# tzt101/MichiGAN

Hardware: AMD Instinct MI355X
Metric: training images/sec at 512x512 (G+D step) (higher is better)
Workload: dtype bf16; 1 GPU; SPADEB G + multiscale PatchGAN D + VGG19 + Gabor orientation losses, full G step + D step (Adam), bs=8/GPU, 512x512, BASELINE.json configs[2]; global_batch=8, batch_per_gpu=8, resolution=512, parallelism=dp1, init=reference default (xavier, 0.02), random VGG weights

## Files before the change

### michigan_amd/_cabi.py

```python
from __future__ import annotations

import contextlib
import ctypes
import os

MG_F32, MG_BF16 = 0, 1
MG_ACT_NONE, MG_ACT_RELU, MG_ACT_LRELU, MG_ACT_TANH = 0, 1, 2, 3
MG_EPI_PLAIN, MG_EPI_SPADE = 0, 1
MG_MAX_TAPS = 64
MG_ABI_VERSION = 10
MG_COMM_ID_BYTES = 128

OPT_CONV_BIGTILES, OPT_CONV_HALO, OPT_WGRAD3X3, OPT_CONV_HALO_BIG, OPT_CONV_SPLITK, OPT_CONV_THIN, OPT_CONV_WIDE, OPT_CONV_DOT = 1, 2, 3, 4, 5, 6, 7, 8
OPT_PROBE_HALO_VARIANT, OPT_PROBE_WGRAD3X3, OPT_PROBE_ADDR_LO, OPT_PROBE_ADDR_HI, OPT_PROBE_NOXPRE = 10, 12, 13, 14, 15
OPT_WGRAD_MIN_STAGES, OPT_NORM_BWD_VEC, OPT_PROBE_HALO_LDSPAD, OPT_CONV_HALO64, OPT_PROBE_HALO64_DBG, OPT_WGRAD3X3_STRIPE = 18, 19, 21, 22, 23, 24

_i32, _f32, _vp, _i64 = ctypes.c_int32, ctypes.c_float, ctypes.c_void_p, ctypes.c_int64


class ConvDesc(ctypes.Structure):
    _fields_ = [
        ("in_", _vp), ("wt", _vp), ("out", _vp), ("bias", _vp), ("resid", _vp), ("x", _vp),
        ("mean", _vp), ("rstd", _vp), ("gamma_out", _vp),
        ("dtype", _i32), ("N", _i32), ("Hin", _i32), ("Win", _i32), ("Cin", _i32),
# ... 102 lines not shown
    "mg_pixel_affine": ([_vp, _vp, _vp, _vp, _i32, _i64, _i32, _vp, _vp], _i32),
    "mg_bg_compose": ([_vp, _vp, _vp, _i64, _i32, _i32, _i32, _i32, _i32, _i32, _vp, _vp, _vp], _i32),
    "mg_masked_mean_fill": ([_vp, _vp, _vp, _vp, _i32, _i32, _i32, _i32, _vp, _vp], _i32),
    "mg_orient_loss_fwd": ([_vp, _vp, _vp, _i32, _i64, _vp, _i64, _i32, _i64, _vp, _vp, _vp], _i32),
    "mg_orient_loss_bwd": ([_vp, _vp, _vp, _i32, _i64, _vp, _i64, _vp, _vp, _vp, _i32, _i64, _vp, _vp], _i32),
    "mg_color_loss_fwd": ([_vp, _vp, _i64, _vp, _i64, _i32, _i32, _i32, _i32, _i32, _i32, _vp, _vp, _vp], _i32),
    "mg_color_loss_bwd": ([_vp, _vp, _i64, _vp, _i64, _vp, _vp, _vp, _i32, _i32, _i32, _i32, _i32, _i32, _vp, _vp], _i32),
    "mg_hair_lab_fwd": ([_vp, _vp, _i64, _vp, _i64, _vp, _i64, _vp, _i64, _vp, _i64, _i32, _i32, _i32, _i32, _i32, _i32, _vp, _vp, _vp, _vp], _i32),
    "mg_hair_lab_bwd": ([_vp, _vp, _i64, _vp, _i64, _vp, _i64, _vp, _vp, _vp, _i32, _i32, _i32, _i32, _i32, _i32, _vp, _vp], _i32),
    "mg_gabor_argmax_fwd": ([_vp, _vp, _vp, _vp, _i32, _i32, _i32, _i32, _i32, _vp], _i32),
    "mg_gabor_argmax_bwd": ([_vp, _vp, _vp, _vp, _i32, _i32, _i32, _i32, _i32, _vp], _i32),
    "mg_self_attention": ([_vp, _vp, _vp, _vp, _i32, _i32, _i32, _i32, _i32, _i64, _i64, _i64, _i64, _vp], _i32),
    "mg_sn_normalize": ([_vp, _i32, _f32, _vp, _vp, _vp, _vp], _i32),
    "mg_sn_scale": ([_vp, _vp, _vp, _i64, _vp], _i32),
    "mg_sn_bwd": ([_vp, _vp, _vp, _vp, _vp, _vp, _i32, _i32, _vp], _i32),
    "mg_adam_step": ([_vp, _vp, _vp, _vp, _i64, _f32, _f32, _f32, _f32, _i32, _f32, _vp], _i32),
    "mg_input_crop_u8": ([_vp, _vp, _vp, _vp, _vp, _vp, _i32, _i32, _i32, _i32, _i32, _i32, _i32, _i32, _vp], _i32),
    "mg_onehot_labels": ([_vp, _vp, _i32, _i64, _i32, _vp], _i32),
    "mg_orient_to_rgb_u8": ([_vp, _vp, _vp, _vp, _i64, _vp], _i32),
    "mg_generate_hole_u8": ([_vp, _vp, _vp, _vp, _vp, _vp, _i32, _i32, _i32, _vp], _i32),
    "mg_noise_octaves": ([_vp, _vp, _i32, _i32, _vp], _i32),
    "mg_resize_bicubic_u8": ([_vp, _vp, _vp, _vp, _vp, _i32, _vp, _vp, _i32, _i32, _i32, _i32, _i32, _i32, _i32, _vp], _i32),
    "mg_bicubic_ksize": ([_i32, _i32], _i32),
    "mg_inputs_set_option": ([_i32, _i32], _i32),
    "mg_bicubic_table": ([_i32, _i32, _vp, _vp], _i32),
    "mg_nearest_table": ([_i32, _i32, _vp], _i32),
    "mg_orient_rgb_table": ([_vp], _i32),
    "mg_noise_field_len": ([_i32], _i64),
    "mg_comm_unique_id": ([_vp], _i32),
    "mg_comm_init": ([_vp, _i32, _i32, ctypes.POINTER(_i64)], _i32),
    "mg_comm_destroy": ([_i64], _i32),
    "mg_comm_world": ([_i64, ctypes.POINTER(_i32), ctypes.POINTER(_i32)], _i32),
    "mg_allreduce_stats": ([_i64, _vp, _i64, _i32, _vp], _i32),
    "mg_allreduce_grads": ([_i64, _vp, _i64, _vp], _i32),
    "mg_probe_mfma_layout": ([_vp, _vp], _i32),
    "mg_probe_tr16": ([_vp, _vp, _vp], _i32),
    "mg_set_option": ([_i32, _i32], _i32),
    "mg_get_option": ([_i32, ctypes.POINTER(_i32)], _i32),
    "mg_sizeof_desc": ([_i32], _i32),
    "mg_abi_version": ([], _i32),
    "mg_last_error": ([], ctypes.c_char_p),
    "mg_feat_moment_workspace": ([_i32, _i64, _i32], _i64),
    "mg_feat_moment_loss_fwd": ([ctypes.POINTER(FeatMomentDesc), _vp], _i32),
    "mg_feat_moment_loss_bwd": ([ctypes.POINTER(FeatMomentDesc), _vp, _vp, _vp, _vp], _i32),
    "mg_orient_smooth": ([_vp, _vp, _vp, _vp, _vp, _vp, _vp, _i32, _i32, _i32, _vp], _i32),
    "mg_stroke_orient": ([_vp, _vp, _vp, _vp, _vp, _vp, _i32, _i32, _i32, _vp], _i32),
    "mg_stroke_compose": ([_vp, _vp, _vp, _vp, _vp, _vp, _vp, _i32, _i32, _i32, _i32, _i32, _i32, _vp, _vp], _i32),
    "mg_inpaint_finish": ([_vp, _vp, _vp, _vp, _vp, _vp, _i32, _i32, _i32, _i32, _i32, _vp, _vp, _vp], _i32),
}
_EDIT_PROTOS = {
    "mge_brush_u8": ([_vp, _vp, _i32, _i32, _i32, _i32, _vp], _i32),
    "mge_morph_u8": ([_vp, _vp, _i32, _i32, _i32, _i32, _i32, _vp, _i32, _i32, _i32, _vp], _i32),
}
EXPORTED_SYMBOLS = tuple(_PROTOS)
_NO_STATUS = {"mg_wgrad_det_workspace", "mg_norm_apply2_supported", "mg_grad_slot_blocks", "mg_pack_job_blocks", "mg_sn_layer_blocks", "mg_stats_workspace", "mg_sizeof_desc", "mg_abi_version", "mg_last_error", "mg_noise_field_len", "mg_bicubic_ksize",
              "mg_feat_moment_workspace"}
_BY_REF = {fn for fn, (argtypes, _) in _PROTOS.items()
           if argtypes and isinstance(getattr(argtypes[0], "_type_", None), type) and issubclass(argtypes[0]._type_, ctypes.Structure)}
DESC_MIRRORS = (ConvDesc, WgradDesc, GradSlot, PackJob, SnLayer, NormApply2Desc, PyramidDesc, FeatMomentDesc)

LIB_PATH = os.environ.get("MG_LIB") or os.path.join(os.path.dirname(os.path.abspath(__file__)), "lib", "libmichigan_hip.so")


class HipBackend:
    name = "hip"

    def __init__(self, path: str = LIB_PATH):
        if not os.path.exists(path) and path == LIB_PATH and os.environ.get("MG_AUTOBUILD", "1") != "0":
            import sys
            print("[michigan_amd] libmichigan_hip.so missing: building it with hipcc (gfx950), ~2 min", file=sys.stderr, flush=True)
            from . import build as _build
            _build.build_locked(verbose=False)
        if not os.path.exists(path):
            raise RuntimeError(
                f"libmichigan_hip.so not found at {path}: build it with "
                "`python -c 'import __graft_entry__ as g; g.build()'` (hipcc, gfx950). "
                "michigan_amd has no CPU / eager-PyTorch fallback.")
        import torch
        self._lib = ctypes.CDLL(path)
        for fn, (argtypes, restype) in list(_PROTOS.items()) + list(_EDIT_PROTOS.items()):
            f = getattr(self._lib, fn)
            f.argtypes, f.restype = argtypes, restype
        if self._lib.mg_abi_version() != MG_ABI_VERSION:
            raise RuntimeError("libmichigan_hip.so ABI version mismatch")
        if any(self._lib.mg_sizeof_desc(which) != ctypes.sizeof(mirror) for which, mirror in enumerate(DESC_MIRRORS)):
            raise RuntimeError("ctypes mirror of the descriptor structs is out of sync with include/michigan_hip.h")

    def __getattr__(self, fn):
        if fn not in _PROTOS and fn not in _EDIT_PROTOS:
            raise AttributeError(fn)
        raw = getattr(self._lib, fn)
        if fn in _NO_STATUS:
            return raw
        by_ref = fn in _BY_REF

        def call(*args):
            if by_ref:
                args = (ctypes.byref(args[0]),) + tuple(args[1:])
            rc = raw(*args)
            if rc != 0:
                msg = self._lib.mg_last_error()
                raise RuntimeError(f"{fn} failed (code {rc}): {msg.decode() if msg else '?'}")
            return rc
        self.__dict__[fn] = call
        return call


_backend = None


def backend():
    global _backend
    if _backend is None:
        _backend = HipBackend()
    return _backend


def set_backend(obj):
    global _backend
    prev, _backend = _backend, obj
    return prev


def get_option(key, be=None):
    v = _i32()
    (be or backend()).mg_get_option(key, ctypes.byref(v))
    return v.value


@contextlib.contextmanager
def options(values, be=None):
    be = be or backend()
    saved = {key: get_option(key, be) for key in values}
    try:
        for key, v in values.items():
            be.mg_set_option(key, v)
        yield
    finally:
        for key, v in saved.items():
            be.mg_set_option(key, v)
```

### michigan_amd/csrc/mg_conv.hip

```cpp

#include "mg_conv_common.h"
#include <map>
#include <mutex>

namespace {

template <typename T, int WM, int WN, int MT, int NT, int EPI, bool PACK>
__global__ __launch_bounds__(NTHR, 3) void conv_taps_kernel(const ConvK d)
{
    constexpr int TM = WM * MT * 32, TN = WN * NT * 32;
    constexpr int EPP = 16 / (int)sizeof(T);
    constexpr int CH  = ROWB / (int)sizeof(T);
    constexpr int A_PT = (TM * 4 + NTHR - 1) / NTHR;
    constexpr int B_PT = (TN * 4) / NTHR;
    constexpr int STAGE = (TM + TN) * ROWB;
    static_assert(WM * WN == 4, "4 waves per workgroup");
    static_assert(EPI == MG_EPI_PLAIN || MT == 2, "SPADE epilogue needs gamma/beta tile pair");

    extern __shared__ __attribute__((aligned(16))) unsigned char smem[];

    const int tid = threadIdx.x, lane = tid & 63, wave = tid >> 6;
    const int wm = wave / WN, wn = wave % WN;
    const int l31 = lane & 31, hi = lane >> 5;

// ... 339 lines not shown
    if constexpr (TM % (16 * WM * WN) == 0) {
        const size_t stage = (size_t)(TM + TN) * ROWB;
        const size_t ldsr = (stage >= 32768 ? 4 : 3) * stage + 2 * TM * sizeof(float);
        auto kern = conv_taps_glds_kernel<T, WM, WN, MT, NT, EPI, PACK>;
        k.ntiles = (int)nblk; k.ksplit = 1; k.ws = nullptr;
        if constexpr (EPI == MG_EPI_PLAIN && !PACK && WM == 2 && WN == 2 && MT == 2 && NT == 2) {
            const int nchunk = (k.Cin * (int)sizeof(T) + ROWB - 1) / ROWB, nkk = k.ntaps * nchunk;
            if (mg_opt(MG_OPT_CONV_SPLITK) && nblk <= 160 && nkk >= 64 && (k.Cout & 3) == 0 && (k.Cout_gemm & 3) == 0) {
                int S = (int)((384 + nblk - 1) / nblk);
                if (S > nkk / 16) S = nkk / 16;
                if (S > 16) S = 16;
                if (S >= 2) {
                    k.ws = splitk_workspace(st, (size_t)S * k.ngemm * k.Cout_gemm * sizeof(float));
                    if (k.ws == nullptr) return mg_fail(MG_ERR_LAUNCH, "mg_conv_taps: split-K scratch allocation failed");
                    k.ksplit = S;
                    hipLaunchKernelGGL(kern, dim3((unsigned)(nblk * S)), dim3(64 * WM * WN), ldsr, st, k);
                    const long nel = (long)k.ngemm * (k.Cout / 4);
                    const long fb = (nel + 255) / 256;
                    hipLaunchKernelGGL(conv_splitk_finish<T>, dim3((unsigned)(fb > 2048 ? 2048 : fb)), dim3(256), 0, st, k);
                    MG_CHECK_LAUNCH("mg_conv_taps(glds, split-K)");
                    return MG_OK;
                }
            }
        }
        if (ldsr > 65536) {
            mg_raise_lds_cap(reinterpret_cast<const void*>(kern), (int)ldsr);
        }
        hipLaunchKernelGGL(kern, dim3((unsigned)nblk), dim3(64 * WM * WN), ldsr, st, k);
        MG_CHECK_LAUNCH("mg_conv_taps(glds)");
        return MG_OK;
    } else {
        const size_t lds = 2 * (size_t)(TM + TN) * ROWB + 2 * TM * sizeof(float);
        hipLaunchKernelGGL((conv_taps_kernel<T, WM, WN, MT, NT, EPI, PACK>), dim3((unsigned)nblk), dim3(NTHR), lds, st, k);
        MG_CHECK_LAUNCH("mg_conv_taps");
        return MG_OK;
    }
}

template <typename T, int EPI>
int dispatch_tiles(ConvK& k, hipStream_t st)
{
    auto wgs = [&](int tm, int tn) { return (long)((k.Cout_gemm + tm - 1) / tm) * ((k.ngemm + tn - 1) / tn); };
    const bool big = mg_opt(MG_OPT_CONV_BIGTILES);
    const int kchunks = k.ntaps * ((k.Cin * (int)sizeof(T) + ROWB - 1) / ROWB);
    if (big && kchunks >= 64 && k.Cout_gemm >= 256 && (k.CoutP % 256) == 0 && wgs(256, 256) >= 384)
        return launch_conv<T, 4, 2, 2, 4, EPI>(k, st);
    if (k.Cout_gemm > 64) return launch_conv<T, 2, 2, 2, 2, EPI>(k, st);
    if (EPI == MG_EPI_SPADE || k.Cout_gemm > 32) return launch_conv<T, 1, 4, 2, 2, EPI>(k, st);
    if constexpr (EPI == MG_EPI_PLAIN) return launch_conv<T, 1, 4, 1, 2, EPI>(k, st);
    return MG_ERR_UNSUPPORTED;
}

template <typename T>
bool halo_applies(const ConvK& k)
{
    constexpr int CH = ROWB / (int)sizeof(T);
    if (!mg_opt(MG_OPT_CONV_HALO)) return false;
    if (k.ntaps != 9 || k.isy != 1 || k.isx != 1 || k.osy != 1 || k.osx != 1 || k.ooy != 0 || k.oox != 0) return false;
    if (k.Hj != k.Hin || k.Wj != k.Win || k.Hout != k.Hin || k.Wout != k.Win) return false;
    if (k.Cin % CH || k.Cout_gemm <= 32 || k.Hin < 8 || k.Win < 16) return false;
    if (k.Cout_gemm <= 64 && k.Hin < 16) return false;
    unsigned seen = 0;
    for (int t = 0; t < 9; ++t) {
        const int dy = (int)(short)(k.tap[t] & 0xffff), dx = k.tap[t] >> 16;
        if (dy < -1 || dy > 1 || dx < -1 || dx > 1) return false;
        seen |= 1u << ((dy + 1) * 3 + dx + 1);
    }
    if (seen != 0x1ffu) return false;
    const int th = k.Cout_gemm <= 64 ? 16 : 8, tmh = k.Cout_gemm <= 64 ? 64 : 128;
    const long wgs = (long)k.N * ((k.Hin + th - 1) / th) * ((k.Win + 15) / 16) * ((k.Cout_gemm + tmh - 1) / tmh);
    return wgs >= 384;
}

template <typename T>
int dispatch_conv(ConvK& k, int epilogue, hipStream_t st)
{
    if (conv_thin_applies(k, ET<T>::DT, epilogue)) return launch_conv_thin(k, st);
    if (conv_thin_taps_applies(k, ET<T>::DT, epilogue)) return launch_conv_thin_taps(k, st);
    if (conv_dot_applies(k, ET<T>::DT, epilogue)) return launch_conv_dot(k, ET<T>::DT, st);
    if (conv_fewout_applies(k, ET<T>::DT, epilogue)) return launch_conv_fewout(k, st);
    if (conv_halo64_applies(k, ET<T>::DT, epilogue)) return launch_conv_halo64(k, st);
    if (halo_applies<T>(k)) return launch_conv_halo(k, ET<T>::DT, epilogue, st);
    return epilogue == MG_EPI_SPADE ? dispatch_tiles<T, MG_EPI_SPADE>(k, st) : dispatch_tiles<T, MG_EPI_PLAIN>(k, st);
}

}

float* mg_stream_scratch(hipStream_t st, size_t bytes) { return splitk_workspace(st, bytes); }

extern "C" int mg_conv_taps(const mg_conv_desc* d, void* stream)
{
    MG_CHECK_ARG(d != nullptr, "mg_conv_taps: null descriptor");
    MG_CHECK_ARG(d->in && d->wt && d->out, "mg_conv_taps: null tensor pointer");
    MG_CHECK_ARG(d->dtype == MG_F32 || d->dtype == MG_BF16, "mg_conv_taps: bad dtype %d", d->dtype);
    MG_CHECK_ARG(d->ntaps >= 1 && d->ntaps <= MG_MAX_TAPS, "mg_conv_taps: ntaps=%d out of range", d->ntaps);
    MG_CHECK_ARG(d->Cin > 0 && (d->Cin % 8) == 0, "mg_conv_taps: Cin=%d must be a positive multiple of 8", d->Cin);
    MG_CHECK_ARG(d->N > 0 && d->Hj > 0 && d->Wj > 0 && d->Hin > 0 && d->Win > 0, "mg_conv_taps: empty geometry");
    MG_CHECK_ARG(d->Cout > 0 && d->Cout_gemm > 0 && d->CoutP >= d->Cout_gemm && (d->CoutP % 128) == 0,
                 "mg_conv_taps: bad channel counts Cout=%d Cout_gemm=%d CoutP=%d", d->Cout, d->Cout_gemm, d->CoutP);
    MG_CHECK_ARG((long)d->N * d->Hj * d->Wj < (1L << 30), "mg_conv_taps: too many output pixels");
    MG_CHECK_ARG((long)d->Cin * (d->dtype == MG_BF16 ? 2 : 4) <= 8192, "mg_conv_taps: Cin too large (%d)", d->Cin);
    MG_CHECK_ARG((d->Hj - 1) * d->osy + d->ooy < d->Hout && (d->Wj - 1) * d->osx + d->oox < d->Wout && d->ooy >= 0 && d->oox >= 0,
                 "mg_conv_taps: output grid exceeds output tensor");
    if (d->epilogue == MG_EPI_SPADE) {
        MG_CHECK_ARG(d->x && d->mean && d->rstd, "mg_conv_taps: SPADE epilogue needs x/mean/rstd");
        MG_CHECK_ARG(d->Cout_gemm == 2 * ((d->Cout + 31) / 32) * 32, "mg_conv_taps: SPADE needs Cout_gemm == 2*roundup(Cout,32)");
        MG_CHECK_ARG(d->x_up == 0 || (d->x_up == 1 && (d->Hout % 2) == 0 && (d->Wout % 2) == 0 &&
                                      (long)d->N * d->Hout * d->Wout * d->Cout < (1L << 32)),
                     "mg_conv_taps: x_up needs even output sizes (and fewer than 2^32 elements)");
    } else {
        MG_CHECK_ARG(d->epilogue == MG_EPI_PLAIN, "mg_conv_taps: bad epilogue %d", d->epilogue);
        MG_CHECK_ARG(d->Cout <= d->Cout_gemm, "mg_conv_taps: Cout > Cout_gemm");
        MG_CHECK_ARG(d->mask_slope >= 0.f && d->mask_slope <= 1.f, "mg_conv_taps: mask_slope %g outside [0, 1]", (double)d->mask_slope);
    }
    ConvK k;
    k.in = d->in; k.wt = d->wt; k.out = d->out; k.bias = d->bias; k.resid = d->resid; k.x = d->x;
    k.mean = d->mean; k.rstd = d->rstd; k.gamma_out = d->gamma_out;
    k.N = d->N; k.Hin = d->Hin; k.Win = d->Win; k.Cin = d->Cin;
    k.Hout = d->Hout; k.Wout = d->Wout; k.Cout = d->Cout; k.Cout_gemm = d->Cout_gemm; k.CoutP = d->CoutP;
    k.Hj = d->Hj; k.Wj = d->Wj; k.isy = d->isy; k.isx = d->isx;
    k.osy = d->osy; k.osx = d->osx; k.ooy = d->ooy; k.oox = d->oox;
    k.ntaps = d->ntaps; k.act = d->act; k.slope = d->slope;
    k.x_up = d->epilogue == MG_EPI_SPADE ? d->x_up : 0;
    k.mslope = d->mask_slope;
    k.ngemm = d->N * d->Hj * d->Wj; k.tiles_m = 0; k.tpc = 1; k.tiles_y = k.tiles_x = 0;
    k.ksplit = 1; k.ntiles = 1; k.ws = nullptr;
    const int probe = mg_opt(MG_OPT_PROBE_HALO_VARIANT);
    k.wide = ((mg_opt(MG_OPT_CONV_WIDE) && d->dtype == MG_BF16 && (d->Cout % 8) == 0) ? 1 : 0) | (probe ? 2 : 0) | (probe == 6 ? 4 : 0) | (mg_opt(MG_OPT_PROBE_NOXPRE) ? 8 : 0);
    for (int t = 0; t < MG_MAX_TAPS; ++t)
        k.tap[t] = t < d->ntaps ? (int)((((uint32_t)(int)d->tap_dy[t]) & 0xffffu) | (((uint32_t)(int)d->tap_dx[t]) << 16)) : 0;
    hipStream_t st = reinterpret_cast<hipStream_t>(stream);
    return d->dtype == MG_BF16 ? dispatch_conv<uint16_t>(k, d->epilogue, st) : dispatch_conv<float>(k, d->epilogue, st);
}
```

### michigan_amd/csrc/mg_conv_common.h

```cpp
#pragma once
#include "mg_common.h"
#include "mg_options.h"
#include <type_traits>


namespace {

constexpr int ROWB = 64;
constexpr int NTHR = 256;

}
struct ConvK {
    const void* in; const void* wt; void* out;
    const float* bias; const void* resid; const void* x;
    const float* mean; const float* rstd; void* gamma_out;
    int N, Hin, Win, Cin;
    int Hout, Wout, Cout, Cout_gemm, CoutP;
    int Hj, Wj, isy, isx, osy, osx, ooy, oox;
    int ntaps, act; float slope;
    int ngemm;
    int tiles_m;
    int tpc;
    int tap[MG_MAX_TAPS];
    int tiles_y, tiles_x;
    int ksplit, ntiles;
    float* ws;
    int wide;
    int x_up;
    float mslope;
};
namespace {

__device__ __forceinline__ int lds_off(int row, int piece) { return row * ROWB + ((piece ^ ((row >> 2) & 3)) << 4); }


template <int MT, int NT>
__device__ __forceinline__ void mma_f32_chunk(const f32x4_t (&a)[MT][2], const f32x4_t (&b)[NT][2], f32x16_t (&acc)[MT][NT])
{
#if MG_F32_ONE_CHAIN
#pragma unroll
    for (int j = 0; j < 8; ++j)
#pragma unroll
        for (int mt = 0; mt < MT; ++mt)
#pragma unroll
            for (int nt = 0; nt < NT; ++nt)
                acc[mt][nt] = __builtin_amdgcn_mfma_f32_32x32x2f32(a[mt][j >> 2][j & 3], b[nt][j >> 2][j & 3], acc[mt][nt], 0, 0, 0);
    return;
#endif
    constexpr int TILES = MT * NT, GT = TILES >= 2 ? 2 : TILES;
    static_assert(TILES % GT == 0, "tile groups");
#pragma unroll
    for (int g0 = 0; g0 < TILES; g0 += GT) {
        f32x16_t t[GT];
#pragma unroll
        for (int j = 0; j < 8; ++j)
#pragma unroll
            for (int g = 0; g < GT; ++g) {
                const int mt = (g0 + g) / NT, nt = (g0 + g) % NT;
                f32x16_t c;
                if (j == 0) {
#pragma unroll
                    for (int e = 0; e < 16; ++e) c[e] = 0.f;
                } else {
                    c = t[g];
                }
                t[g] = __builtin_amdgcn_mfma_f32_32x32x2f32(a[mt][j >> 2][j & 3], b[nt][j >> 2][j & 3], c, 0, 0, 0);
            }
#pragma unroll
        for (int g = 0; g < GT; ++g) {
            const int mt = (g0 + g) / NT, nt = (g0 + g) % NT;
            acc[mt][nt] += t[g];
            asm volatile("" : "+v"(acc[mt][nt]));
        }
    }
}

template <typename T, int MT, int NT>
__device__ __forceinline__ void conv_compute(const unsigned char* As, const unsigned char* Bs, int l31, int hi,
                                             f32x16_t (&acc)[MT][NT])
{
    const int sw = (l31 >> 2) & 3;
    if constexpr (sizeof(T) == 2) {
// ... 557 lines not shown
```

### michigan_amd/csrc/mg_conv_halo.hip

```cpp
#include "mg_conv_common.h"
#ifndef MG_HALO_SCHED
#define MG_HALO_SCHED 0
#endif


namespace {

constexpr int TW = 16, PW = TW + 2;

constexpr int RING = 3;
template <int WM, int NT> struct HaloGeom {
    static constexpr int WN = 4 / WM;
    static constexpr int TM = WM * 64;
    static constexpr int TH = WN * NT * 32 / TW;
    static constexpr int PROWS = (TH + 2) * PW;
    static constexpr int PBLK_REAL = (PROWS + 15) / 16;
    static constexpr int PBLK = (PBLK_REAL + 3) / 4 * 4;
    static constexpr int PSTAGE = PBLK * 1024;
    static constexpr int ASTAGE = TM * ROWB;
    static constexpr int A_IPS = TM / 64, P_IPS = PBLK / 4;
    static constexpr int PATCH0 = RING * ASTAGE;
    static constexpr int PAR = PATCH0 + 2 * PSTAGE;
    static constexpr int LDS = PAR + 2 * TM * 4;
    static constexpr int OCC = NT == 4 ? 2 : 3;
};

__device__ unsigned long long* g_mg_probe_out = nullptr;

__device__ __forceinline__ unsigned long long stamp()
{
    unsigned long long v;
    asm volatile("s_memrealtime %0\n\ts_waitcnt lgkmcnt(0)" : "=s"(v) :: "memory");
    return v;
}

template <typename T, int EPI, int WM, int NT, int PROBE = 0>
__global__ __launch_bounds__(NTHR, (NT == 4 || sizeof(T) == 4 ? 2 : 3)) void conv3x3_halo_kernel(const ConvK d)
{
    using G = HaloGeom<WM, NT>;
    constexpr int PF = RING - 1;
    constexpr int MT = 2, WN = G::WN;
    constexpr int TH = G::TH, PROWS = G::PROWS, PSTAGE = G::PSTAGE, ASTAGE = G::ASTAGE, TM_H = G::TM;
    constexpr int A_IPS = G::A_IPS, P_IPS = G::P_IPS;
    constexpr bool BF = sizeof(T) == 2;
    constexpr int EPP = 16 / (int)sizeof(T);
    constexpr int CH  = ROWB / (int)sizeof(T);
    constexpr int KX  = BF ? 32 : 16;

    extern __shared__ __attribute__((aligned(16))) unsigned char smem[];
    unsigned long long e_entry = 0;
    if constexpr (PROBE == 4) e_entry = stamp();

    const int tid = threadIdx.x, lane = tid & 63;
    const int wave = __builtin_amdgcn_readfirstlane(tid >> 6);
    const int wm = wave / WN, wn = wave % WN;
    const int l31 = lane & 31, hi = lane >> 5;

    int tile;
    {
        const int nblk = gridDim.x, b = blockIdx.x;
        const int q8 = nblk >> 3, r8 = nblk & 7, xcd = b & 7, idx = b >> 3;
        tile = (xcd < r8 ? xcd * (q8 + 1) : r8 * (q8 + 1) + (xcd - r8) * q8) + idx;
    }
    const int tm = tile % d.tiles_m;  tile /= d.tiles_m;
    const int tx = tile % d.tiles_x;  tile /= d.tiles_x;
    const int ty = tile % d.tiles_y;
    const int img = tile / d.tiles_y;
    const int m0 = tm * TM_H, y0 = ty * TH, x0 = tx * TW;

    const T* __restrict__ In = reinterpret_cast<const T*>(d.in);
    const unsigned lds0 = (unsigned)(size_t)(__attribute__((address_space(3))) unsigned char*)smem;

    const int lrow = lane >> 2;
    const int piece = (lane & 3) ^ ((lane >> 4) & 3);
    const unsigned char* const zsrc = g_mg_zeros + (lane & 3) * 16;

    const unsigned char* pp[P_IPS];
#pragma unroll
    for (int j = 0; j < P_IPS; ++j) {
        const int r = (wave + 4 * j) * 16 + lrow;
        const int pr = r / PW, pc = r - pr * PW;
        const int iy = y0 + pr - 1, ix = x0 + pc - 1;
        const bool ok = r < PROWS && (unsigned)iy < (unsigned)d.Hin && (unsigned)ix < (unsigned)d.Win;
        pp[j] = ok ? reinterpret_cast<const unsigned char*>(In + ((size_t)((img * d.Hin + iy) * d.Win + ix) * d.Cin + piece * EPP)) : zsrc;
    }
    const unsigned char* wbase = reinterpret_cast<const unsigned char*>(d.wt) + (size_t)m0 * d.Cin * sizeof(T);
    unsigned woff[A_IPS];
#pragma unroll
    for (int j = 0; j < A_IPS; ++j)
        woff[j] = (unsigned)(((wave + 4 * j) * 16 + lrow) * d.Cin + piece * EPP) * (unsigned)sizeof(T);
    const long tapstride = (long)d.CoutP * d.Cin * (long)sizeof(T);
    const long chunkwrap = (long)ROWB - 8 * tapstride;

    const int nchunk = d.Cin / CH;

    auto issue_patch = [&](int buf) {
        const unsigned base = lds0 + G::PATCH0 + buf * PSTAGE;
#pragma unroll
        for (int j = 0; j < P_IPS; ++j) {
            const int blk = wave + 4 * j;
            glds16(pp[j], __builtin_amdgcn_readfirstlane(base + blk * 1024));
            pp[j] += ROWB;
        }
    };
    auto issue_a = [&](int slot, bool last_tap) {
        const unsigned base = lds0 + slot * ASTAGE;
#pragma unroll
        for (int j = 0; j < A_IPS; ++j)
            glds16_s(wbase, woff[j], __builtin_amdgcn_readfirstlane(base + (wave + 4 * j) * 1024));
        wbase += last_tap ? chunkwrap : tapstride;
    };

    constexpr bool ZERO_C = BF && (PROBE == 0 || PROBE == 4);
    f32x16_t acc[MT][NT];
    if constexpr (!ZERO_C) {
#pragma unroll
        for (int mt = 0; mt < MT; ++mt)
#pragma unroll
            for (int nt = 0; nt < NT; ++nt)
#pragma unroll
                for (int r = 0; r < 16; ++r) acc[mt][nt][r] = 0.f;
    }

    const int ksp = BF ? hi : hi * 2;
    const int aoff = (wm * 64 + l31) * ROWB + ((ksp ^ ((l31 >> 2) & 3)) << 4);
    int boff[9][NT];
    {
        const int py = l31 >> 4, px = (l31 - 2 * py) & 15;
#pragma unroll
        for (int t = 0; t < 9; ++t) {
            const int tp = d.tap[t];
            const int dy = (int)(short)(tp & 0xffff), dx = tp >> 16;
#pragma unroll
            for (int nt = 0; nt < NT; ++nt) {
                const int brow = ((wn * NT + nt) * 2 + py + 1 + dy) * PW + px + 1 + dx;
                boff[t][nt] = G::PATCH0 + brow * ROWB + ((ksp ^ ((brow >> 2) & 3)) << 4);
            }
        }
    }

    auto compute = [&](auto t_, int slot, auto first_) {
        constexpr int t = decltype(t_)::value;
        constexpr bool FIRST = decltype(first_)::value;
        const unsigned char* As = smem + slot * ASTAGE;
        if constexpr (BF) {
#pragma unroll
            for (int ks = 0; ks < 2; ++ks) {
                bf16x8_t a[MT], b[NT];
#pragma unroll
                for (int mt = 0; mt < MT; ++mt)
                    a[mt] = *reinterpret_cast<const bf16x8_t*>(As + mt * 32 * ROWB + (ks ? aoff ^ KX : aoff));
#pragma unroll
                for (int nt = 0; nt < NT; ++nt)
                    b[nt] = *reinterpret_cast<const bf16x8_t*>(smem + (ks ? boff[t][nt] ^ KX : boff[t][nt]));
#pragma unroll
// ... 25 lines not shown
#elif MG_HALO_SCHED == 2
            if constexpr (MT == 2 && NT == 4) __builtin_amdgcn_iglp_opt(0);
#elif MG_HALO_SCHED == 3
            if constexpr (MT == 2 && NT == 4) __builtin_amdgcn_iglp_opt(1);
#endif
        } else {
            f32x4_t a[MT][2], b[NT][2];
#pragma unroll
            for (int mt = 0; mt < MT; ++mt) {
                a[mt][0] = *reinterpret_cast<const f32x4_t*>(As + mt * 32 * ROWB + aoff);
                a[mt][1] = *reinterpret_cast<const f32x4_t*>(As + mt * 32 * ROWB + (aoff ^ KX));
            }
#pragma unroll
            for (int nt = 0; nt < NT; ++nt) {
                b[nt][0] = *reinterpret_cast<const f32x4_t*>(smem + boff[t][nt]);
                b[nt][1] = *reinterpret_cast<const f32x4_t*>(smem + (boff[t][nt] ^ KX));
            }
            mma_f32_chunk<MT, NT>(a, b, acc);
        }
    };

    auto pixmap = [&](int p, size_t& opix, size_t& upix) -> bool {
        const int py = p >> 4;
        const int y = y0 + py, x = x0 + (((p & 15) - 2 * (py & 1)) & 15);
        if (y >= d.Hout || x >= d.Wout) return false;
        opix = (size_t)((img * d.Hout + y) * d.Wout + x);
        upix = (size_t)((img * (d.Hout >> 1) + (y >> 1)) * (d.Wout >> 1) + (x >> 1));
        return true;
    };
    constexpr bool XPRE = EPI == MG_EPI_SPADE && BF;
    uint2 xpre[2 * NT * 2] = {};
    bool xpre_ok = false;
    if constexpr (XPRE) {
        xpre_ok = ((d.Cout | d.Cout_gemm) & 3) == 0 && d.act != MG_ACT_TANH && !(d.wide & 8);
        if (xpre_ok) {
            const uint16_t* __restrict__ X = reinterpret_cast<const uint16_t*>(d.x);
#pragma unroll
            for (int nt = 0; nt < NT; ++nt) {
                size_t opix, upix = 0;
                const bool ok = pixmap(wn * NT * 32 + nt * 32 + l31, opix, upix);
                const unsigned xo = ok ? (unsigned)((d.x_up ? upix : opix) * d.Cout) : 0u;
#pragma unroll
                for (int hh = 0; hh < 2; ++hh)
#pragma unroll
                    for (int q = 0; q < 2; ++q) {
                        const int occ = ((m0 + wm * 64) >> 1) + (hh * 2 + q) * 8 + hi * 4;
                        xpre[(hh * NT + nt) * 2 + q] = *reinterpret_cast<const uint2*>(X + xo + (occ < d.Cout ? occ : 0));
                    }
            }
        }
    }
    float* const par = reinterpret_cast<float*>(smem + G::PAR);
    conv_stage_params_dma<TM_H, EPI, 4>(d, m0, lds0 + G::PAR, wave, lane);
    issue_patch(0);
#pragma unroll
    for (int i = 0; i < PF; ++i) issue_a(i, false);

    unsigned long long e_begin = 0;
    if constexpr (PROBE == 4) e_begin = stamp();
    if constexpr (PROBE != 0 && PROBE != 4) {
        unsigned long long t_wait = 0, t_bar = 0, t_tap = 0, t_all = stamp();
        for (int c = 0; c < nchunk; ++c) {
            const bool next_chunk = (c + 1 < nchunk);
            const int pdelta = (c & 1) ? -PSTAGE : PSTAGE;
            static_for<0, 9>([&](auto t_) {
                constexpr int t = decltype(t_)::value;
                unsigned long long s0 = 0, s1 = 0, s2 = 0;
                if constexpr (PROBE == 3) s0 = stamp();
                if constexpr (PROBE == 1) { if constexpr (t == 0) wait_vmcnt<0>(); }
                else {
                    if constexpr (t == 1 || t == 2) { if (next_chunk) wait_vmcnt<A_IPS + P_IPS>(); else wait_vmcnt<A_IPS>(); }
                    else if constexpr (t == 8)      { if (next_chunk) wait_vmcnt<A_IPS>(); else wait_vmcnt<0>(); }
                    else                            wait_vmcnt<A_IPS>();
                }
                if constexpr (PROBE == 3) s1 = stamp();
                if constexpr (PROBE != 2) __builtin_amdgcn_s_barrier();
                if constexpr (PROBE == 3) s2 = stamp();
                if constexpr (PROBE != 1) {
                    if constexpr (t < 7) issue_a((t + 2) % 3, t == 6);
                    else { if (next_chunk) issue_a((t + 2) % 3, false); }
                }
                if constexpr (t == 0) { if (next_chunk) issue_patch((c + 1) & 1); }
                compute(t_, t % 3, std::false_type{});
#pragma unroll
                for (int nt = 0; nt < NT; ++nt) boff[t][nt] += pdelta;
                if constexpr (PROBE == 3) {
                    const unsigned long long s3 = stamp();
                    t_wait += s1 - s0; t_bar += s2 - s1; t_tap += s3 - s2;
                }
            });
        }
        if constexpr (PROBE == 3) {
            t_all = stamp() - t_all;
            if (lane == 0) {
                unsigned long long* o = reinterpret_cast<unsigned long long*>(d.out) + ((size_t)blockIdx.x * 4 + wave) * 4;
                o[0] = t_wait; o[1] = t_bar; o[2] = t_tap; o[3] = t_all;
            }
            float keep = 0.f;
#pragma unroll
            for (int mt = 0; mt < MT; ++mt)
#pragma unroll
                for (int nt = 0; nt < NT; ++nt)
#pragma unroll
                    for (int r = 0; r < 16; ++r) keep += acc[mt][nt][r];
            if (keep == 12345.678f) reinterpret_cast<T*>(d.out)[1 << 20] = (T)1;
            return;
        }
    } else {
        auto chunk = [&](int c, auto first_) {
            const bool next_chunk = (c + 1 < nchunk);
            const int pdelta = (c & 1) ? -PSTAGE : PSTAGE;
            static_for<0, 9>([&](auto t_) {
                constexpr int t = decltype(t_)::value;
                if constexpr (t == 1 || t == 2) { if (next_chunk) wait_vmcnt<A_IPS + P_IPS>(); else wait_vmcnt<A_IPS>(); }
                else if constexpr (t == 8)      { if (next_chunk) wait_vmcnt<A_IPS>(); else wait_vmcnt<0>(); }
                else                            wait_vmcnt<A_IPS>();
                __builtin_amdgcn_s_barrier();
                if constexpr (t < 7) issue_a((t + 2) % 3, t == 6);
                else { if (next_chunk) issue_a((t + 2) % 3, false); }
                if constexpr (t == 0) { if (next_chunk) issue_patch((c + 1) & 1); }
                compute(t_, t % 3, std::bool_constant<ZERO_C && decltype(first_)::value && t == 0>{});
#pragma unroll
                for (int nt = 0; nt < NT; ++nt) boff[t][nt] += pdelta;
            });
        };
        chunk(0, std::true_type{});
        for (int c = 1; c < nchunk; ++c) chunk(c, std::false_type{});
    }

#if MG_PROBES
    if (PROBE != 4 && (d.wide & 2)) {
        if (acc[0][0][0] == 12345.678f) reinterpret_cast<T*>(d.out)[0] = (T)1;
        return;
    }
#endif
    if constexpr (PROBE == 4) {
        const unsigned long long e0 = stamp();
        unsigned long long ts[12] = {};
        conv_epilogue<T, MT, NT, EPI, TM_H>(d, acc, m0, pixmap, wm, wn, l31, hi, par, [&](int i) { ts[i] = stamp(); }, xpre, xpre_ok);
        const unsigned long long e1 = stamp();
        wait_vmcnt<0>();
        const unsigned long long e2 = stamp();
        if (lane == 0 && g_mg_probe_out) {
            unsigned hw, xcc;
            asm volatile("s_getreg_b32 %0, hwreg(HW_REG_HW_ID)\n\ts_getreg_b32 %1, hwreg(HW_REG_XCC_ID)" : "=s"(hw), "=s"(xcc));
            unsigned long long* o = g_mg_probe_out + ((size_t)blockIdx.x * 4 + wave) * 20;
#pragma unroll
            for (int i = 0; i < 12; ++i) o[8 + i] = ts[i];
            o[0] = e_entry; o[1] = e_begin; o[2] = e0; o[3] = e1; o[4] = e2; o[5] = ((unsigned long long)xcc << 32) | hw;
        }
        return;
    }
    conv_epilogue<T, MT, NT, EPI, TM_H>(d, acc, m0, pixmap, wm, wn, l31, hi, par, EpiNoMark(), xpre, xpre_ok);
}

template <typename T, int EPI, int WM, int NT, int PROBE = 0>
int launch_halo_g(ConvK& k, hipStream_t st)
{
    using G = HaloGeom<WM, NT>;
    k.tiles_m = (k.Cout_gemm + G::TM - 1) / G::TM;
    k.tiles_y = (k.Hin + G::TH - 1) / G::TH;
    k.tiles_x = (k.Win + TW - 1) / TW;
    const long nblk = (long)k.N * k.tiles_y * k.tiles_x * k.tiles_m;
    if (nblk <= 0 || nblk > 0x7fffffffL) return mg_fail(MG_ERR_ARG, "mg_conv_taps(halo): bad grid %ld", nblk);
    auto kern = conv3x3_halo_kernel<T, EPI, WM, NT, PROBE>;
    int lds = G::LDS;
#if MG_PROBES
    lds += mg_opt(MG_OPT_PROBE_HALO_LDSPAD);
#endif
    if (lds > 65536) {
        mg_raise_lds_cap(reinterpret_cast<const void*>(kern), lds);
    }
    hipLaunchKernelGGL(kern, dim3((unsigned)nblk), dim3(NTHR), lds, st, k);
    MG_CHECK_LAUNCH("mg_conv_taps(halo)");
    return MG_OK;
}

template <typename T, int EPI>
int launch_halo(ConvK& k, hipStream_t st)
{
    if (k.Cout_gemm <= 64) return launch_halo_g<T, EPI, 1, 2>(k, st);
    if constexpr (sizeof(T) == 4) return launch_halo_g<T, EPI, 2, 2>(k, st);
    else {
    const long big = (long)k.N * ((k.Hin + 15) / 16) * ((k.Win + 15) / 16) * ((k.Cout_gemm + 127) / 128);
    if (mg_opt(MG_OPT_CONV_HALO_BIG) && k.Hin >= 16 && big >= 1024) {
#if MG_PROBES
        if constexpr (sizeof(T) == 2) {
            const int probe = mg_opt(MG_OPT_PROBE_HALO_VARIANT);
            if constexpr (EPI == MG_EPI_PLAIN) {
                if (probe == 2) return launch_halo_g<T, EPI, 2, 4, 1>(k, st);
                if (probe == 3) return launch_halo_g<T, EPI, 2, 4, 2>(k, st);
                if (probe == 4) return launch_halo_g<T, EPI, 2, 4, 3>(k, st);
            }
            if (probe >= 5) return launch_halo_g<T, EPI, 2, 4, 4>(k, st);
        }
#endif
        return launch_halo_g<T, EPI, 2, 4>(k, st);
    }
    return launch_halo_g<T, EPI, 2, 2>(k, st);
    }
}

}

int conv_halo_set_probe(unsigned long long addr)
{
    unsigned long long* p = reinterpret_cast<unsigned long long*>(addr);
    return hipMemcpyToSymbol(HIP_SYMBOL(g_mg_probe_out), &p, sizeof(p)) == hipSuccess ? MG_OK : MG_ERR_ARG;
}

int launch_conv_halo(ConvK& k, int dtype, int epilogue, hipStream_t st)
{
    if (dtype == MG_BF16)
        return epilogue == MG_EPI_SPADE ? launch_halo<uint16_t, MG_EPI_SPADE>(k, st) : launch_halo<uint16_t, MG_EPI_PLAIN>(k, st);
    return epilogue == MG_EPI_SPADE ? launch_halo<float, MG_EPI_SPADE>(k, st) : launch_halo<float, MG_EPI_PLAIN>(k, st);
}
```

### michigan_amd/csrc/mg_norm.hip

```cpp
#include "mg_common.h"
#include "mg_launch.h"
#include "mg_options.h"
#include "mg_reduce.h"


namespace {

struct StatGeom { int tpr; int rpb; int nchunks; int64_t chunk; };

static inline StatGeom stat_geom(int G, int64_t P, int C)
{
    StatGeom g;
    const int c4 = C / 4;
    g.tpr = c4 < MG_NTHR ? c4 : MG_NTHR;
    g.rpb = MG_NTHR / g.tpr;
    int64_t want = (1536 + G - 1) / G;
    const int64_t cap = (P + (int64_t)g.rpb * 16 - 1) / ((int64_t)g.rpb * 16);
    if (want > cap) want = cap;
    if (want > 512) want = 512;
    if (want < 1) want = 1;
    g.chunk = (P + want - 1) / want;
    g.nchunks = (int)((P + g.chunk - 1) / g.chunk);
    return g;
}
// ... 42 lines not shown
    return {dpre, has_g1 ? dpre * gv : dpre};
}

template <int W>
__device__ __forceinline__ void join_to_partial(float (&s)[W], float (&ss)[W], float* red, int cv, int rows, bool row0, float* __restrict__ partial, int C, int c)
{
    float* const terms[2] = {s, ss};
    mg_row_join<2, W>(terms, red, cv, rows, row0);
    if (row0) {
        float* dst = partial + ((size_t)blockIdx.y * gridDim.x + blockIdx.x) * 2 * C + c;
#pragma unroll
        for (int j = 0; j < W; ++j) { dst[j] = s[j]; dst[C + j] = ss[j]; }
    }
}

struct QuadChunk { int tq, tr; bool active; int64_t p0, p1; };
__device__ __forceinline__ QuadChunk quad_chunk(int64_t P, int tpr, int rpb, int64_t chunk)
{
    const int tid = threadIdx.x;
    const int64_t p0 = (int64_t)blockIdx.x * chunk;
    return {tid % tpr, tid / tpr, tid < tpr * rpb, p0, (p0 + chunk < P) ? p0 + chunk : P};
}

template <typename T>
__global__ __launch_bounds__(MG_NTHR) void stats_stage1_quad(const T* __restrict__ x, float* __restrict__ partial, int64_t P, int C,
                                                             int tpr, int rpb, int64_t chunk, int shift)
{
    __shared__ float red[MG_NTHR * 8];
    const int g = blockIdx.y, c4 = C / 4;
    const auto [tq, tr, active, p0, p1] = quad_chunk(P, tpr, rpb, chunk);
    for (int qd0 = 0; qd0 < c4; qd0 += tpr) {
        const int qd = qd0 + tq;
        const bool qv = active && qd < c4;
        const int c = (qd < c4 ? qd : 0) * 4;
        float s[4] = {0.f, 0.f, 0.f, 0.f}, ss[4] = {0.f, 0.f, 0.f, 0.f};
        f32x4_t kv = {0.f, 0.f, 0.f, 0.f};
        if (shift) kv = ET<T>::load4(x + (size_t)g * P * C + c);
        if (qv) {
            for (int64_t p = p0 + tr; p < p1; p += rpb) {
                const f32x4_t xv = ET<T>::load4(x + ((size_t)g * P + p) * C + c);
#pragma unroll
                for (int j = 0; j < 4; ++j) { const float t = xv[j] - kv[j]; s[j] += t; ss[j] += t * t; }
            }
        }
        join_to_partial(s, ss, red, tpr, rpb, qv && tr == 0, partial, C, c);
        __syncthreads();
    }
}

template <typename T, bool HAS_H>
__global__ __launch_bounds__(MG_NTHR) void bwd_stage1_quad(
    const T* __restrict__ x, const T* __restrict__ dh, const T* __restrict__ h, const T* __restrict__ g1,
    const float* __restrict__ mean, const float* __restrict__ rstd, T* __restrict__ dgb,
    float* __restrict__ partial, int64_t P, int C, int tpr, int rpb, int64_t chunk, int act, float slope, int up, int H, int W)
{
    __shared__ float red[MG_NTHR * 8];
    const int g = blockIdx.y, c4 = C / 4;
    const auto [tq, tr, active, p0, p1] = quad_chunk(P, tpr, rpb, chunk);
    const int Cr2 = 2 * ((C + 31) / 32) * 32;
    for (int qd0 = 0; qd0 < c4; qd0 += tpr) {
        const int qd = qd0 + tq;
        const bool qv = active && qd < c4;
        const int c = (qd < c4 ? qd : 0) * 4;
        float s[4] = {0.f, 0.f, 0.f, 0.f}, ss[4] = {0.f, 0.f, 0.f, 0.f};
        f32x4_t mu, rs;
#pragma unroll
        for (int j = 0; j < 4; ++j) { mu[j] = mean[(size_t)g * C + c + j]; rs[j] = rstd[(size_t)g * C + c + j]; }
        if (qv) {
            for (int64_t p = p0 + tr; p < p1; p += rpb) {
                const size_t o = ((size_t)g * P + p) * C + c;
                size_t ox = o;
                if (up) ox = up_src_offset((int)p, H, W, C, c);
                const f32x4_t xv = ET<T>::load4(x + ox);
                const f32x4_t dv = ET<T>::load4(dh + o);
                f32x4_t hv = {1.f, 1.f, 1.f, 1.f};
                if constexpr (HAS_H) hv = ET<T>::load4(h + o);
                f32x4_t gv = {1.f, 1.f, 1.f, 1.f};
                if (g1) gv = ET<T>::load4(g1 + o);
                f32x4_t dgam, dbet;
#pragma unroll
                for (int j = 0; j < 4; ++j) {
                    const DxHat d = dxhat_quad(dv[j], hv[j], gv[j], act, slope);
                    const float xh = (xv[j] - mu[j]) * rs[j];
                    s[j] += d.dxh; ss[j] += d.dxh * xh;
                    dgam[j] = d.dpre * xh; dbet[j] = d.dpre;
                }
                if (dgb) {
                    const size_t ob = ((size_t)g * P + p) * Cr2 + (size_t)(c >> 5) * 64 + (c & 31);
                    ET<T>::store4(dgb + ob, dgam);
                    ET<T>::store4(dgb + ob + 32, dbet);
                }
            }
        }
        join_to_partial(s, ss, red, tpr, rpb, qv && tr == 0, partial, C, c);
        __syncthreads();
    }
}

__global__ __launch_bounds__(256) void reduce_stage2(const float* __restrict__ partial, float* __restrict__ sums, int nchunks, int C2)
{
    __shared__ double red[256];
    const int cl = threadIdx.x & 31, kk = threadIdx.x >> 5;
    const int i = blockIdx.x * 32 + cl;
    const int g = blockIdx.y;
    double a = 0.0;
    if (i < C2) a = mg_chunk_sum_f64(a, partial + (size_t)g * nchunks * C2 + i, kk, nchunks, C2);
    a = mg_chunk_rows_join(a, red);
    if (kk == 0 && i < C2) sums[(size_t)g * C2 + i] = (float)a;
}

template <typename T>
__global__ void norm_act_fwd_kernel(const T* __restrict__ x, T* __restrict__ y, int64_t nquads, int64_t P, int C,
                                    const float* __restrict__ mean, const float* __restrict__ rstd, int act, float slope,
                                    const T* __restrict__ resid)
{
    const int c4 = C / 4;
    for (int64_t i = (int64_t)blockIdx.x * blockDim.x + threadIdx.x; i < nquads; i += (int64_t)gridDim.x * blockDim.x) {
        const int qd = (int)(i % c4);
        const int64_t pix = i / c4;
        const int g = (int)(pix / P);
        const int c = qd * 4;
        const f32x4_t xv = ET<T>::load4(x + i * 4);
        f32x4_t o;
#pragma unroll
        for (int j = 0; j < 4; ++j)
            o[j] = mg_act((xv[j] - mean[(size_t)g * C + c + j]) * rstd[(size_t)g * C + c + j], act, slope);
        if (resid) {
            const f32x4_t rv = ET<T>::load4(resid + i * 4);
#pragma unroll
            for (int j = 0; j < 4; ++j) o[j] += rv[j];
        }
        ET<T>::store4(y + i * 4, o);
    }
}

template <typename T>
__global__ void norm_bwd_apply_kernel(const T* __restrict__ dh, const T* __restrict__ h, const T* __restrict__ x,
                                      const T* __restrict__ g1, T* __restrict__ dx, int64_t nquads, int64_t P, int C,
                                      const float* __restrict__ mean, const float* __restrict__ rstd,
                                      const float* __restrict__ s1, const float* __restrict__ s2, int sgs, float sscale, int act, float slope)
// ... 116 lines not shown
            const int64_t p = p0 + k * step;
            if (p < P) {
                float o4[VEC];
#pragma unroll
                for (int j = 0; j < VEC; ++j) {
                    const float v = (xv[k][j] - m[j]) * r[j];
                    const float t = v > 0.f ? v : v * neg;
                    o4[j] = relu ? fmaxf(v, 0.f) : t;
                    if (resid) o4[j] += rv[k][j];
                }
                EV<T>::store(y + base + (size_t)p * C, o4);
            }
        }
    }
}

template <typename T, int PIX>
__global__ __launch_bounds__(MG_NTHR) void stats_stage1_vec(const T* __restrict__ x, float* __restrict__ partial, int64_t P, int C, int64_t chunk, int shift)
{
    constexpr int VEC = EV<T>::VEC;
    __shared__ float red[MG_NTHR * 2 * VEC];
    const auto [cv, rows, tq, tr, c] = chan_thread<VEC>(C);
    const int g = blockIdx.y;
    const int64_t p0 = (int64_t)blockIdx.x * chunk;
    const int64_t p1 = (p0 + chunk < P) ? p0 + chunk : P;
    float s[VEC], ss[VEC], kv[VEC];
#pragma unroll
    for (int j = 0; j < VEC; ++j) { s[j] = 0.f; ss[j] = 0.f; }
    const size_t base = (size_t)g * P * C + c;
    if (shift) EV<T>::load(x + base, kv);
    else {
#pragma unroll
        for (int j = 0; j < VEC; ++j) kv[j] = 0.f;
    }
    for (int64_t pp = p0 + tr; pp < p1; pp += (int64_t)rows * PIX) {
        float xv[PIX][VEC];
#pragma unroll
        for (int k = 0; k < PIX; ++k) {
            const int64_t p = pp + (int64_t)k * rows;
            if (p < p1) EV<T>::load(x + base + (size_t)p * C, xv[k]);
            else {
#pragma unroll
                for (int j = 0; j < VEC; ++j) xv[k][j] = kv[j];
            }
        }
#pragma unroll
        for (int k = 0; k < PIX; ++k)
#pragma unroll
            for (int j = 0; j < VEC; ++j) { const float t = xv[k][j] - kv[j]; s[j] += t; ss[j] += t * t; }
    }
    join_to_partial(s, ss, red, cv, rows, tr == 0, partial, C, c);
}

template <typename T, int PIX, bool HAS_H, bool UP>
__global__ __launch_bounds__(MG_NTHR) void bwd_stage1_vec(const T* __restrict__ x, const T* __restrict__ dh, const T* __restrict__ h, const T* __restrict__ g1,
                                                     const float* __restrict__ mean, const float* __restrict__ rstd, T* __restrict__ dgb,
                                                     float* __restrict__ partial, int64_t P, int C, int64_t chunk, float neg, int H, int W)
{
    constexpr int VEC = EV<T>::VEC;
    __shared__ float red[MG_NTHR * 2 * VEC];
    const auto [cv, rows, tq, tr, c] = chan_thread<VEC>(C);
    const int g = blockIdx.y;
    const int Cr2 = 2 * ((C + 31) / 32) * 32;
    const int64_t p0 = (int64_t)blockIdx.x * chunk;
    const int64_t p1 = (p0 + chunk < P) ? p0 + chunk : P;
    float mu[VEC], rs[VEC], s[VEC], ss[VEC];
    chan_stats(mean + (size_t)g * C + c, rstd + (size_t)g * C + c, mu, rs);
#pragma unroll
    for (int j = 0; j < VEC; ++j) { s[j] = 0.f; ss[j] = 0.f; }
    const size_t base = (size_t)g * P * C + c;
    const size_t gbase = (size_t)g * P * Cr2 + (size_t)(c >> 5) * 64 + (c & 31);
    for (int64_t pp = p0 + tr; pp < p1; pp += (int64_t)rows * PIX) {
        float xv[PIX][VEC], dv[PIX][VEC], hv[PIX][VEC], gv[PIX][VEC];
#pragma unroll
        for (int k = 0; k < PIX; ++k) {
            const int64_t p = pp + (int64_t)k * rows;
            if (p < p1) {
                size_t ox = base + (size_t)p * C;
                if (UP) ox = up_src_offset((int)p, H, W, C, c);
                EV<T>::load(x + ox, xv[k]);
                EV<T>::load(dh + base + (size_t)p * C, dv[k]);
                if (HAS_H) EV<T>::load(h + base + (size_t)p * C, hv[k]);
                if (g1) EV<T>::load(g1 + base + (size_t)p * C, gv[k]);
            }
        }
#pragma unroll
        for (int k = 0; k < PIX; ++k) {
            const int64_t p = pp + (int64_t)k * rows;
            if (p < p1) {
                float dgam[VEC], dbet[VEC];
#pragma unroll
                for (int j = 0; j < VEC; ++j) {
                    const DxHat d = dxhat_vec(dv[k][j], hv[k][j], gv[k][j], neg, HAS_H, g1 != nullptr);
                    const float xh = (xv[k][j] - mu[j]) * rs[j];
                    s[j] += d.dxh; ss[j] += d.dxh * xh;
                    dgam[j] = d.dpre * xh; dbet[j] = d.dpre;
                }
                if (dgb) {
                    EV<T>::store(dgb + gbase + (size_t)p * Cr2, dgam);
                    EV<T>::store(dgb + gbase + (size_t)p * Cr2 + 32, dbet);
                }
            }
        }
    }
    join_to_partial(s, ss, red, cv, rows, tr == 0, partial, C, c);
}

__global__ void norm_finalize_kernel(const double* __restrict__ sums, int G, int C, double count, float eps, float momentum,
                                     float* __restrict__ running_mean, float* __restrict__ running_var,
                                     float* __restrict__ mean, float* __restrict__ rstd)
{
    const int i = blockIdx.x * blockDim.x + threadIdx.x;
    if (i >= G * C) return;
    const int g = i / C, c = i - g * C;
    const double s = sums[((size_t)g * 2) * C + c], ss = sums[((size_t)g * 2 + 1) * C + c];
    finalize_channel(s, ss, count, eps, momentum, running_mean, running_var, c, mean, rstd, [&] { return i; });
}

template <typename T, int NB, bool UP>
__global__ __launch_bounds__(MG_NTHR) void norm_bwd_apply2_vec(const mg_norm_apply2_desc d, float neg0, float neg1)
{
    constexpr int VEC = EV<T>::VEC;
    const int C = d.C;
    const auto [cv, rows, tq, tr, c] = chan_thread<VEC>(C);
    const T* dh0 = (const T*)d.dh[0]; const T* h0 = (const T*)d.h[0]; const T* g0 = (const T*)d.g1[0];
    const T* dh1 = (const T*)d.dh[1]; const T* h1 = (const T*)d.h[1]; const T* g1 = (const T*)d.g1[1];
    const T* x = (const T*)d.x; T* dx = (T*)d.dx;
    constexpr int Q = UP ? 4 : 1;
    float m[VEC], r[VEC], k1[VEC], k2[VEC];
    chan_stats(d.mean + c, d.rstd + c, m, r);
#pragma unroll
    for (int j = 0; j < VEC; ++j) {
        float s1 = d.sums[0][c + j], s2 = d.sums[0][C + c + j];
        if (NB == 2) { s1 += d.sums[1][c + j]; s2 += d.sums[1][C + c + j]; }
        k1[j] = (float)Q * r[j] * s1 * d.inv_count;
        k2[j] = (float)Q * r[j] * r[j] * s2 * d.inv_count;
    }
    const int W = d.W, H = d.H, W2 = W >> 1, H2 = H >> 1;
    const int64_t Pout = UP ? d.P / 4 : d.P;
    const int64_t step = (int64_t)gridDim.x * rows;
    for (int64_t po = (int64_t)blockIdx.x * rows + tr; po < Pout; po += step) {
        int64_t pf[Q];
        if (UP) {
            const int pp = (int)po, n = pp / (H2 * W2), rem = pp - n * (H2 * W2);
            const int y2 = rem / W2, x2 = rem - y2 * W2;
            const int64_t base = ((int64_t)n * H + 2 * y2) * W + 2 * x2;
            pf[0] = base; if (Q > 1) { pf[1 % Q] = base + 1; pf[2 % Q] = base + W; pf[3 % Q] = base + W + 1; }
        } else pf[0] = po;
        float xv[VEC], acc[VEC];
        EV<T>::load(x + (size_t)po * C + c, xv);
#pragma unroll
// ... 33 lines not shown
    const int cl = threadIdx.x & 31, kk = threadIdx.x >> 5;
    const int c = blockIdx.x * 16 + (cl & 15);
    const int g = blockIdx.y;
    const int C2 = 2 * C;
    const int i = (cl >> 4) * C + c;
    double a = 0.0;
    if (c < C) a = mg_chunk_sum_f64(a, partial + (size_t)g * nchunks * C2 + i, kk, nchunks, C2);
    a = mg_chunk_rows_join(a, red);
    if (kk == 0) fin[cl] = a;
    __syncthreads();
    if (threadIdx.x < 16 && c < C) {
        const double kv = shift ? (double)ET<T>::load1(x + (size_t)g * P * C + c) : 0.0;
        const double sh = fin[threadIdx.x], ssh = fin[16 + threadIdx.x], n = (double)P;
        const double s = (sh + n * kv) * sum_scale;
        const double ss = (ssh + 2.0 * kv * sh + n * kv * kv) * sum_scale;
        sums[(size_t)g * C2 + c] = s;
        sums[(size_t)g * C2 + C + c] = ss;
        if (FIN) finalize_channel(s, ss, count, eps, momentum, running_mean, running_var, c, mean, rstd, [&] { return (size_t)g * C + c; });
    }
}

template <typename T, bool FIN>
int run_stats(const void* x, int G, int64_t P, int C, int shift, double* sums, void* partial, double sum_scale, double count, float eps, float momentum,
              float* running_mean, float* running_var, float* mean, float* rstd, hipStream_t st)
{
    const StatGeom sg = stat_geom(G, P, C);
    dim3 grid(sg.nchunks, G);
    if (vec_geom_ok<T>(C))
        hipLaunchKernelGGL((stats_stage1_vec<T, 4>), grid, dim3(MG_NTHR), 0, st, (const T*)x, (float*)partial, P, C, sg.chunk, shift);
    else
        hipLaunchKernelGGL(stats_stage1_quad<T>, grid, dim3(MG_NTHR), 0, st, (const T*)x, (float*)partial, P, C, sg.tpr, sg.rpb, sg.chunk, shift);
    MG_CHECK_LAUNCH("channel statistics (stage 1)");
    hipLaunchKernelGGL((stats_stage2<T, FIN>), dim3((C + 15) / 16, G), dim3(256), 0, st, (const float*)partial, (const T*)x, P, sums, sg.nchunks, C, shift,
                       sum_scale, count, eps, momentum, running_mean, running_var, mean, rstd);
    MG_CHECK_LAUNCH("channel statistics (stage 2)");
    return MG_OK;
}

template <typename T>
int run_reduce(const void* x, const void* dh, const void* h, const void* g1, const float* mean, const float* rstd,
               void* dgb, int G, int64_t P, int C, float* sums, void* partial, int act, float slope, hipStream_t st,
               int up, int H, int W)
{
    const StatGeom sg = stat_geom(G, P, C);
    dim3 grid(sg.nchunks, G);
    if (mg_opt(MG_OPT_NORM_BWD_VEC) && takes_vec<T>(C, act)) {
        const float neg = mg_neg_slope(act, slope);
        mg_by_bool(h != nullptr && act != MG_ACT_NONE, [&](auto hh) { mg_by_bool(up != 0, [&](auto upf) {
            hipLaunchKernelGGL((bwd_stage1_vec<T, 2, hh.value, upf.value>), grid, dim3(MG_NTHR), 0, st, (const T*)x, (const T*)dh, (const T*)h,
                               (const T*)g1, mean, rstd, (T*)dgb, (float*)partial, P, C, sg.chunk, neg, H, W); }); });
    } else
        mg_by_bool(h != nullptr, [&](auto hh) {
            hipLaunchKernelGGL((bwd_stage1_quad<T, hh.value>), grid, dim3(MG_NTHR), 0, st, (const T*)x, (const T*)dh, (const T*)h, (const T*)g1,
                               mean, rstd, (T*)dgb, (float*)partial, P, C, sg.tpr, sg.rpb, sg.chunk, act, slope, up, H, W); });
    MG_CHECK_LAUNCH("reduce_stage1");
    dim3 grid2((2 * C + 31) / 32, G);
    hipLaunchKernelGGL(reduce_stage2, grid2, dim3(256), 0, st, (const float*)partial, sums, sg.nchunks, 2 * C);
    MG_CHECK_LAUNCH("reduce_stage2");
    return MG_OK;
}

}

#define MG_CHECK_NORM_GEOM(name) \
    MG_CHECK_ARG(dtype == MG_F32 || dtype == MG_BF16, "%s: bad dtype %d", name, dtype); \
    MG_CHECK_ARG(G > 0 && P > 0 && C > 0 && (C % 4) == 0 && C <= 4096, "%s: bad geometry G=%d P=%ld C=%d (C must be a multiple of 4, <= 4096)", name, G, (long)P, C)

extern "C" int64_t mg_stats_workspace(int32_t G, int64_t P, int32_t C)
{
    if (G <= 0 || P <= 0 || C <= 0) return 0;
    const StatGeom sg = stat_geom(G, P, C);
    return (int64_t)G * sg.nchunks * 2 * C * (int64_t)sizeof(float);
}

extern "C" int mg_channel_stats(const void* x, int32_t dtype, int32_t G, int64_t P, int32_t C, int32_t shift,
                                double* sums, void* partial, void* stream)
{
    MG_CHECK_NORM_GEOM("mg_channel_stats");
    MG_CHECK_ARG(x && sums && partial, "mg_channel_stats: null pointer");
    hipStream_t st = reinterpret_cast<hipStream_t>(stream);
    return mg_by_dtype(dtype, [&](auto t) { using T = typename decltype(t)::type;
        return run_stats<T, false>(x, G, P, C, shift != 0, sums, partial, 1.0, 1.0, 0.f, 0.f, nullptr, nullptr, nullptr, nullptr, st); });
}

extern "C" int mg_channel_stats_finalize(const void* x, int32_t dtype, int32_t G, int64_t P, int32_t C, float sum_scale, double count,
                                         float eps, float momentum, float* running_mean, float* running_var,
                                         double* sums, float* mean, float* rstd, void* partial, void* stream)
{
    MG_CHECK_NORM_GEOM("mg_channel_stats_finalize");
    MG_CHECK_ARG(x && sums && mean && rstd && partial, "mg_channel_stats_finalize: null pointer");
    MG_CHECK_ARG(count > 0 && sum_scale > 0.f, "mg_channel_stats_finalize: bad count / scale");
    MG_CHECK_ARG((running_mean == nullptr) == (running_var == nullptr) && (running_mean == nullptr || G == 1),
                 "mg_channel_stats_finalize: running statistics need both buffers and G == 1");
    hipStream_t st = reinterpret_cast<hipStream_t>(stream);
    return mg_by_dtype(dtype, [&](auto t) { using T = typename decltype(t)::type;
        return run_stats<T, true>(x, G, P, C, 1, sums, partial, (double)sum_scale, count, eps, momentum, running_mean, running_var, mean, rstd, st); });
}

extern "C" int mg_norm_act_fwd(const void* x, void* y, int32_t dtype, int32_t G, int64_t P, int32_t C,
                               const float* mean, const float* rstd, int32_t act, float slope, const void* resid, void* stream)
{
    MG_CHECK_NORM_GEOM("mg_norm_act_fwd");
    MG_CHECK_ARG(x && y && mean && rstd, "mg_norm_act_fwd: null pointer");
    hipStream_t st = reinterpret_cast<hipStream_t>(stream);
    const int64_t nq = (int64_t)G * P * (C / 4);
    mg_by_dtype(dtype, [&](auto t) { using T = typename decltype(t)::type;
        if (takes_vec<T>(C, act)) {
            hipLaunchKernelGGL((norm_act_fwd_vec<T, 4>), dim3(pix_grid(P, vec_rows<T>(C), 4, G), G), dim3(MG_NTHR), 0, st,
                               (const T*)x, (T*)y, P, C, mean, rstd, mg_neg_slope(act, slope), act == MG_ACT_RELU, (const T*)resid);
        } else
            hipLaunchKernelGGL(norm_act_fwd_kernel<T>, dim3(mg_ew_grid(nq, 8192)), dim3(MG_NTHR), 0, st,
                               (const T*)x, (T*)y, nq, P, C, mean, rstd, act, slope, (const T*)resid);
    });
    MG_CHECK_LAUNCH("mg_norm_act_fwd");
    return MG_OK;
}

static int norm_bwd_reduce(const char* name, const void* dh, const void* h, const void* x, const void* g1,
                           int32_t dtype, int32_t G, int64_t P, int32_t C, const float* mean, const float* rstd, int32_t act, float slope,
                           void* dgb, float* sums, void* partial, void* stream, int up, int32_t N, int32_t H, int32_t W)
{
    MG_CHECK_NORM_GEOM(name);
    MG_CHECK_ARG(dh && (h || act == MG_ACT_NONE) && x && mean && rstd && sums && partial, "%s: null pointer", name);
    MG_CHECK_ARG(dgb == nullptr || G == 1, "%s: dgb output requires G == 1", name);
    if (up) MG_CHECK_ARG(N > 0 && H > 0 && W > 0 && (H % 2) == 0 && (W % 2) == 0 && P < (1L << 31), "%s: H, W must be even", name);
    hipStream_t st = reinterpret_cast<hipStream_t>(stream);
    return mg_by_dtype(dtype, [&](auto t) { using T = typename decltype(t)::type;
        return run_reduce<T>(x, dh, h, g1, mean, rstd, dgb, G, P, C, sums, partial, act, slope, st, up, H, W); });
}

extern "C" int mg_norm_bwd_reduce(const void* dh, const void* h, const void* x, const void* g1,
                                  int32_t dtype, int32_t G, int64_t P, int32_t C,
                                  const float* mean, const float* rstd, int32_t act, float slope,
                                  void* dgb, float* sums, void* partial, void* stream)
{
    return norm_bwd_reduce("mg_norm_bwd_reduce", dh, h, x, g1, dtype, G, P, C, mean, rstd, act, slope, dgb, sums, partial, stream, 0, 0, 0, 0);
}

extern "C" int mg_norm_bwd_reduce_up(const void* dh, const void* h, const void* x, const void* g1,
                                     int32_t dtype, int32_t N, int32_t H, int32_t W, int32_t C,
                                     const float* mean, const float* rstd, int32_t act, float slope,
                                     void* dgb, float* sums, void* partial, void* stream)
{
    return norm_bwd_reduce("mg_norm_bwd_reduce_up", dh, h, x, g1, dtype, 1, (int64_t)N * H * W, C, mean, rstd, act, slope, dgb, sums, partial, stream, 1, N, H, W);
}

template <typename T>
static int launch_apply2(const mg_norm_apply2_desc& d, hipStream_t st)
{
    const int rows = vec_rows<T>(d.C);
    const bool two = d.dh[1] != nullptr;
    const int64_t pout = d.up ? d.P / 4 : d.P;
    const float n0 = mg_neg_slope(d.act[0], d.slope[0]), n1 = mg_neg_slope(d.act[1], d.slope[1]);
    const dim3 grid(pix_grid(pout, rows, 1, 1)), blk(MG_NTHR);
    mg_by_bool(d.up != 0, [&](auto up) { mg_by_bool(two, [&](auto nb2) {
        hipLaunchKernelGGL((norm_bwd_apply2_vec<T, nb2.value ? 2 : 1, up.value>), grid, blk, 0, st, d, n0, n1); }); });
    return 0;
}

extern "C" int mg_norm_apply2_supported(int32_t dtype, int32_t C)
{
    return dtype == MG_BF16 ? vec_geom_ok<uint16_t>(C) : (dtype == MG_F32 ? vec_geom_ok<float>(C) : 0);
}

extern "C" int mg_norm_bwd_apply2(const mg_norm_apply2_desc* d, void* stream)
{
    MG_CHECK_ARG(d != nullptr, "mg_norm_bwd_apply2: null descriptor");
    MG_CHECK_ARG(d->dtype == MG_F32 || d->dtype == MG_BF16, "mg_norm_bwd_apply2: bad dtype");
    MG_CHECK_ARG(d->dh[0] && d->sums[0] && d->x && d->mean && d->rstd && d->dx, "mg_norm_bwd_apply2: null pointer");
    MG_CHECK_ARG((d->dh[1] == nullptr) == (d->sums[1] == nullptr), "mg_norm_bwd_apply2: the second branch needs dh and sums");
    for (int b = 0; b < 2; ++b)
        MG_CHECK_ARG(d->act[b] != MG_ACT_TANH && (d->h[b] || d->act[b] == MG_ACT_NONE || !d->dh[b]), "mg_norm_bwd_apply2: activation needs its output h");
    MG_CHECK_ARG(d->C > 0 && d->P > 0 && d->P < (1L << 31) && mg_norm_apply2_supported(d->dtype, d->C), "mg_norm_bwd_apply2: unsupported geometry C=%d", d->C);
    MG_CHECK_ARG(!d->up || (d->H > 0 && d->W > 0 && (d->H % 2) == 0 && (d->W % 2) == 0 && d->P % ((int64_t)d->H * d->W) == 0),
                 "mg_norm_bwd_apply2: up needs even H, W and P = N*H*W");
    hipStream_t st = reinterpret_cast<hipStream_t>(stream);
    mg_by_dtype(d->dtype, [&](auto t) { launch_apply2<typename decltype(t)::type>(*d, st); });
    MG_CHECK_LAUNCH("mg_norm_bwd_apply2");
    return MG_OK;
}

extern "C" int mg_norm_bwd_apply(const void* dh, const void* h, const void* x, const void* g1,
                                 int32_t dtype, int32_t G, int64_t P, int32_t C,
                                 const float* mean, const float* rstd, const float* s1, const float* s2,
                                 int32_t sum_gstride, float sum_scale, int32_t act, float slope, void* dx, void* stream)
{
    MG_CHECK_NORM_GEOM("mg_norm_bwd_apply");
    MG_CHECK_ARG(sum_gstride >= C, "mg_norm_bwd_apply: sum_gstride < C");
    const int sgs = sum_gstride; const float sscale = sum_scale;
    MG_CHECK_ARG(dh && (h || act == MG_ACT_NONE) && x && mean && rstd && s1 && s2 && dx, "mg_norm_bwd_apply: null pointer");
    hipStream_t st = reinterpret_cast<hipStream_t>(stream);
    const int64_t nq = (int64_t)G * P * (C / 4);
    mg_by_dtype(dtype, [&](auto t) { using T = typename decltype(t)::type;
        if (takes_vec<T>(C, act)) {
            hipLaunchKernelGGL((norm_bwd_apply_vec<T, 2>), dim3(pix_grid(P, vec_rows<T>(C), 2, G), G), dim3(MG_NTHR), 0, st,
                               (const T*)dh, (const T*)h, (const T*)x, (const T*)g1, (T*)dx,
                               P, C, mean, rstd, s1, s2, sgs, sscale, mg_neg_slope(act, slope));
// ... 23 lines not shown
```

### michigan_amd/csrc/mg_wgrad.hip

```cpp
#include "mg_common.h"
#include "mg_wgrad_common.h"
#include "mg_options.h"



namespace {

constexpr int NTHR = 256;

struct WgK {
    const void* x; const void* dy; float* dw; float* dbias;
    int N, Hin, Win, Cin, Hj, Wj, Cg, isy, isx, ntaps;
    int K;
    int kper;
    int tiles_m, tiles_n, splitk;
    int tpt;
    long det_stride;
    int tap[MG_MAX_TAPS];
};

template <typename T, bool TR>
__global__ __launch_bounds__(NTHR) void wgrad_kernel(const WgK d)
{
    constexpr bool BF = (sizeof(T) == 2);
// ... 256 lines not shown
        }
    }
}

template <typename T, bool TR>
int launch_wgrad(WgK& k, hipStream_t st, int* nsplit = nullptr, bool dry = false)
{
    constexpr bool BF = (sizeof(T) == 2);
    constexpr int KP = BF ? 32 : 16;
    constexpr int RS = BF ? 320 : 528;
    k.tiles_m = (k.Cg + 127) / 128;
    k.tpt = (k.Cin < 128 && 128 % k.Cin == 0) ? 128 / k.Cin : 1;
    k.tiles_n = k.tpt > 1 ? 1 : (k.Cin + 127) / 128;
    const long base = (long)k.tiles_m * k.tiles_n * ((k.ntaps + k.tpt - 1) / k.tpt);
    int S = k.splitk;
    if (S <= 0) {
        S = (int)((1536 + base - 1) / base);
        const int min_stages = mg_opt(MG_OPT_WGRAD_MIN_STAGES);
        int maxS = (k.K + KP * min_stages - 1) / (KP * min_stages);
        if (base * maxS < 256) {
            const int fill = (int)((256 + base - 1) / base), floor4 = (k.K + KP * 4 - 1) / (KP * 4);
            maxS = fill < floor4 ? fill : floor4;
        }
        if (S > maxS) S = maxS;
        if (S < 1) S = 1;
    }
    k.kper = ((k.K + S - 1) / S + KP - 1) / KP * KP;
    S = (k.K + k.kper - 1) / k.kper;
    k.splitk = S;
    const long nblk = base * S;
    if (nsplit) *nsplit = S;
    if (dry) return MG_OK;
    if (nblk <= 0 || nblk > 0x7fffffffL) return mg_fail(MG_ERR_ARG, "mg_conv_wgrad: bad grid %ld", nblk);
    const size_t lds = 2 * 2 * (size_t)KP * RS;
    hipLaunchKernelGGL((wgrad_kernel<T, TR>), dim3((unsigned)nblk), dim3(NTHR), lds, st, k);
    MG_CHECK_LAUNCH("mg_conv_wgrad");
    return MG_OK;
}

}

int launch_wgrad_det_finish(const float* ws, int nsplit, long stride, float* dw, long ndw, float* dbias, int nbias, hipStream_t st)
{
    const long total = ndw + nbias;
    long grid = (total + 31) / 32;
    if (grid > 8192) grid = 8192;
    hipLaunchKernelGGL(wgrad_det_finish_kernel, dim3((unsigned)grid), dim3(256), 0, st, ws, nsplit, stride, dw, ndw, dbias, nbias);
    MG_CHECK_LAUNCH("mg_conv_wgrad(deterministic finish)");
    return MG_OK;
}

namespace {

int route_wgrad(const mg_wgrad_desc* d, hipStream_t st, float* dw, float* dbias, long det_stride, int* nsplit, bool dry)
{
    WgK k;
    k.x = d->x; k.dy = d->dy; k.dw = dw; k.dbias = dbias;
    k.N = d->N; k.Hin = d->Hin; k.Win = d->Win; k.Cin = d->Cin;
    k.Hj = d->Hj; k.Wj = d->Wj; k.Cg = d->Cg; k.isy = d->isy; k.isx = d->isx; k.ntaps = d->ntaps;
    k.K = d->N * d->Hj * d->Wj; k.splitk = d->splitk; k.kper = 0; k.tiles_m = k.tiles_n = 0; k.tpt = 1; k.det_stride = det_stride;
    for (int t = 0; t < MG_MAX_TAPS; ++t)
        k.tap[t] = t < d->ntaps ? (int)((((uint32_t)(int)d->tap_dy[t]) & 0xffffu) | (((uint32_t)(int)d->tap_dx[t]) << 16)) : 0;
    if (d->dtype == MG_BF16 && d->ntaps == 9 && d->isy == 1 && d->isx == 1 && d->Hin == d->Hj && d->Win == d->Wj && d->Cin == 8) {
        bool std3x3 = true;
        for (int t = 0; t < 9; ++t) std3x3 = std3x3 && d->tap_dy[t] == t / 3 - 1 && d->tap_dx[t] == t % 3 - 1;
        Wg3K k3;
        k3.x = d->x; k3.dy = d->dy; k3.dw = dw; k3.dbias = dbias;
        k3.N = d->N; k3.H = d->Hin; k3.W = d->Win; k3.Cin = d->Cin; k3.Cg = d->Cg;
        k3.nstg = 0; k3.sps = 0; k3.tiles_m = k3.tiles_n = 0; k3.splitk = 0; k3.det_stride = det_stride; k3.half_cu = 0; k3.stripe_w = 0;
        if (std3x3 && wgrad_thin_applies(k3)) return launch_wgrad_thin(k3, st, nsplit, dry);
    }
    if (wgrad_thin_taps_applies(d)) return launch_wgrad_thin_taps(d, st, dw, dbias, det_stride, nsplit, dry);
    if (mg_opt(MG_OPT_WGRAD3X3) && d->dtype == MG_BF16 && (d->flags & 1) && d->ntaps == 9 && d->isy == 1 && d->isx == 1 &&
        d->Hin == d->Hj && d->Win == d->Wj && (d->Win == 16 || d->Win % 32 == 0) && (d->Hin * d->Win) % 32 == 0 &&
        d->Cin >= 64 && d->Cg >= 64) {
        bool std3x3 = true;
        for (int t = 0; t < 9; ++t) std3x3 = std3x3 && d->tap_dy[t] == t / 3 - 1 && d->tap_dx[t] == t % 3 - 1;
        if (std3x3) {
            Wg3K k3;
            k3.x = d->x; k3.dy = d->dy; k3.dw = dw; k3.dbias = dbias;
            k3.N = d->N; k3.H = d->Hin; k3.W = d->Win; k3.Cin = d->Cin; k3.Cg = d->Cg;
            k3.nstg = k.K / 32; k3.sps = 0; k3.tiles_m = k3.tiles_n = 0; k3.splitk = d->splitk; k3.det_stride = det_stride;
            k3.half_cu = (d->flags & 2) ? 1 : 0; k3.stripe_w = 0;
            return launch_wgrad3x3(k3, st, nsplit, dry);
        }
    }
    if (d->dtype == MG_BF16)
        return (d->flags & 1) ? launch_wgrad<uint16_t, true>(k, st, nsplit, dry) : launch_wgrad<uint16_t, false>(k, st, nsplit, dry);
    return launch_wgrad<float, false>(k, st, nsplit, dry);
}

int check_wgrad_desc(const mg_wgrad_desc* d, const char* who)
{
    MG_CHECK_ARG(d != nullptr, "%s: null descriptor", who);
    MG_CHECK_ARG(d->x && d->dy && d->dw, "%s: null tensor pointer", who);
    MG_CHECK_ARG(d->dtype == MG_F32 || d->dtype == MG_BF16, "%s: bad dtype %d", who, d->dtype);
    MG_CHECK_ARG(d->ntaps >= 1 && d->ntaps <= MG_MAX_TAPS, "%s: ntaps=%d out of range", who, d->ntaps);
    MG_CHECK_ARG(d->Cin > 0 && (d->Cin % 8) == 0 && d->Cg > 0 && (d->Cg % 8) == 0,
                 "%s: Cin=%d / Cg=%d must be positive multiples of 8", who, d->Cin, d->Cg);
    MG_CHECK_ARG(d->N > 0 && d->Hj > 0 && d->Wj > 0 && d->Hin > 0 && d->Win > 0, "%s: empty geometry", who);
    MG_CHECK_ARG((long)d->N * d->Hj * d->Wj < (1L << 30), "%s: too many pixels", who);
    return MG_OK;
}

}

extern "C" int64_t mg_wgrad_det_workspace(const mg_wgrad_desc* d)
{
    if (check_wgrad_desc(d, "mg_wgrad_det_workspace") != MG_OK) return -1;
    int S = 0;
    if (route_wgrad(d, nullptr, d->dw, d->dbias, 0, &S, true) != MG_OK || S <= 0) return -1;
    const long slab = (long)d->ntaps * d->Cg * d->Cin + (d->dbias ? d->Cg : 0);
    return (int64_t)S * slab * (int64_t)sizeof(float);
}

extern "C" int mg_conv_wgrad(const mg_wgrad_desc* d, void* stream)
{
    const int rc = check_wgrad_desc(d, "mg_conv_wgrad");
    if (rc != MG_OK) return rc;
    hipStream_t st = reinterpret_cast<hipStream_t>(stream);
    if (d->det_ws == nullptr) return route_wgrad(d, st, d->dw, d->dbias, 0, nullptr, false);
    int S = 0;
    if (route_wgrad(d, st, d->dw, d->dbias, 0, &S, true) != MG_OK || S <= 0) return mg_fail(MG_ERR_ARG, "mg_conv_wgrad: cannot size the deterministic workspace");
    const long ndw = (long)d->ntaps * d->Cg * d->Cin, nbias = d->dbias ? d->Cg : 0, slab = ndw + nbias;
    MG_CHECK_ARG(d->det_ws_bytes >= (int64_t)S * slab * (int64_t)sizeof(float), "mg_conv_wgrad: deterministic workspace too small (%ld splits)", (long)S);
    float* ws = reinterpret_cast<float*>(d->det_ws);
    int S2 = 0;
    const int r2 = route_wgrad(d, st, ws, d->dbias ? ws + ndw : nullptr, slab, &S2, false);
    if (r2 != MG_OK) return r2;
    if (S2 != S) return mg_fail(MG_ERR_LAUNCH, "mg_conv_wgrad: split count changed between sizing and launch (%d vs %d)", S, S2);
    return launch_wgrad_det_finish(ws, S, slab, d->dw, ndw, d->dbias, (int)nbias, st);
}
```

### michigan_amd/csrc/mg_wgrad3x3.hip

```cpp
#include "mg_conv_common.h"
#include "mg_wgrad_common.h"


namespace {

typedef __attribute__((ext_vector_type(4))) short s16x4_t;
typedef __attribute__((ext_vector_type(8))) short s16x8_t;
typedef __attribute__((address_space(3))) s16x4_t* lds_s16x4_p;

__device__ unsigned long long* g_mg_wg3_probe_out = nullptr;
__device__ __forceinline__ unsigned long long wg3_stamp()
{
    unsigned long long v;
    asm volatile("s_memrealtime %0\n\ts_waitcnt lgkmcnt(0)" : "=s"(v) :: "memory");
    return v;
}

template <int MT, int NT, bool W16, bool PROBE = false>
__global__ __launch_bounds__(256, 2) void wgrad3x3_kernel(const Wg3K d)
{
    constexpr int TM = 64 * MT, TN = 64 * NT;
    constexpr int RBA = TM * 2, RBB = TN * 2;
    constexpr int PPA = RBA / 16, PPB = RBB / 16;
    constexpr int A_ROWS = 32, B_ROWS = (NT == 2) ? 36 : 40;
    constexpr int A_BYTES = A_ROWS * RBA, B_BYTES = B_ROWS * RBB;
    constexpr int A_IPS = A_BYTES / 4096;
    constexpr int B_IPS = (B_BYTES + 4095) / 4096;
    constexpr int IPS = A_IPS + B_IPS;
    constexpr int STAGE = A_BYTES + B_BYTES;
    constexpr int NS = 4;
    static_assert(A_BYTES % 4096 == 0 && B_BYTES % 1024 == 0, "stage must be whole wave blocks");

    extern __shared__ __attribute__((aligned(16))) unsigned char smem[];

    const int tid = threadIdx.x, lane = tid & 63;
    const int wave = __builtin_amdgcn_readfirstlane(tid >> 6);
    const int wm = wave >> 1, wn = wave & 1;
    const int l31 = lane & 31, hi = lane >> 5;

    int tile;
    {
        const int nblk = gridDim.x, b = blockIdx.x;
        const int q8 = nblk >> 3, r8 = nblk & 7, xcd = b & 7, idx = b >> 3;
        tile = (xcd < r8 ? xcd * (q8 + 1) : r8 * (q8 + 1) + (xcd - r8) * q8) + idx;
    }
    const int tm = tile % d.tiles_m;  tile /= d.tiles_m;
    const int tn = tile % d.tiles_n;  tile /= d.tiles_n;
    const int ky = tile % 3;
    const int split = tile / 3;
    const int m0 = tm * TM, n0 = tn * TN;
    const int sbeg = split * d.sps;
    const int send = min(d.nstg, sbeg + d.sps);
    const int nk = send - sbeg;
    if (nk <= 0) return;

    const int H = d.H, W = d.W;
    constexpr int SEG = W16 ? 16 : 32, SEGP = SEG + 2;
    constexpr int PR = (32 / SEG) * SEGP;
    const unsigned lds0 = (unsigned)(size_t)(__attribute__((address_space(3))) unsigned char*)smem;
    const unsigned dump = lds0 + NS * STAGE + wave * 1024;
    const unsigned char* zsrc = g_mg_zeros + (lane & 3) * 16;

    auto swz_a = [](int row) { return RBA == 256 ? (row & 3) : ((row >> 1) & 1); };
    auto swz_b = [](int row) { return RBB == 256 ? (row & 3) : ((row >> 1) & 1); };

    int aoff[A_IPS];
#pragma unroll
    for (int j = 0; j < A_IPS; ++j) {
        const int g = j * 256 + tid, row = g / PPA, slot = g % PPA;
        int ch = m0 + ((slot ^ (swz_a(row) << 2)) << 3);
        if (ch >= d.Cg) ch = m0;
        aoff[j] = (row * d.Cg + ch) * 2;
    }
    int boff[B_IPS], brc[B_IPS];
#pragma unroll
    for (int j = 0; j < B_IPS; ++j) {
        const int g = j * 256 + tid, row = g / PPB, slot = g % PPB;
        int ch = n0 + ((slot ^ (swz_b(row) << 2)) << 3);
        if (ch >= d.Cin) ch = n0;
        const int r = (W16 && row >= SEGP) ? 1 : 0, c = row - r * SEGP - 1;
        boff[j] = (((r + ky - 1) * W + c) * d.Cin + ch) * 2;
        brc[j] = row < PR ? (r | (c + 1) << 4) : -1;
    }
    const unsigned char* const dy0 = reinterpret_cast<const unsigned char*>(d.dy);
    const unsigned char* const x0p = reinterpret_cast<const unsigned char*>(d.x);
    const unsigned char* abase; const unsigned char* xbase;
    int sy, sx, sg_next = sbeg;
    int simg = 0, sstripe = 0;
    const int SWp = W16 ? W : d.stripe_w, nsegs = SWp / 32, nstripes = W / SWp;
    if (W16) {
        abase = dy0 + (size_t)sbeg * 32 * d.Cg * 2;
        xbase = x0p + (size_t)sbeg * 32 * d.Cin * 2;
        const int rem = (sbeg * 32) % (H * W); sy = rem / W; sx = rem - sy * W;
    } else {
        const int spi = H * (W / 32);
        simg = sbeg / spi;
        int r = sbeg - simg * spi;
        sstripe = r / (H * nsegs);  r -= sstripe * (H * nsegs);
        sy = r / nsegs;
        sx = sstripe * SWp + (r - sy * nsegs) * 32;
        const size_t p = ((size_t)simg * H + sy) * W + sx;
        abase = dy0 + p * d.Cg * 2;
        xbase = x0p + p * d.Cin * 2;
    }
    sy = __builtin_amdgcn_readfirstlane(sy); sx = __builtin_amdgcn_readfirstlane(sx);
    simg = __builtin_amdgcn_readfirstlane(simg); sstripe = __builtin_amdgcn_readfirstlane(sstripe);
    const int a_step = 32 * d.Cg * 2, x_step = 32 * d.Cin * 2;

    unsigned long long m_live[B_IPS], m_left[B_IPS], m_right[B_IPS], m_r1[B_IPS];
#pragma unroll
    for (int j = 0; j < B_IPS; ++j) {
        const bool lv = brc[j] >= 0;
        const int c = (brc[j] >> 4) - 1, r = brc[j] & 15;
        m_live[j]  = __builtin_amdgcn_ballot_w64(lv);
        m_left[j]  = __builtin_amdgcn_ballot_w64(lv && c == -1);
        m_right[j] = __builtin_amdgcn_ballot_w64(lv && c == SEG);
        m_r1[j]    = __builtin_amdgcn_ballot_w64(lv && r == 1);
    }
    const unsigned long long zaddr = (unsigned long long)(size_t)zsrc;
    const unsigned zlo = (unsigned)zaddr, zhi = (unsigned)(zaddr >> 32);

    auto issue = [&](int stage) {
        const bool real = sg_next < send;
        const unsigned sbase = lds0 + stage * STAGE;
        if (real) {
#pragma unroll
            for (int j = 0; j < A_IPS; ++j)
                glds16_s(abase, (unsigned)aoff[j], __builtin_amdgcn_readfirstlane(sbase + j * 4096 + wave * 1024));
        } else {
#pragma unroll
            for (int j = 0; j < A_IPS; ++j)
                glds16(zsrc, __builtin_amdgcn_readfirstlane(sbase + j * 4096 + wave * 1024));
        }
        const int sxs = __builtin_amdgcn_readfirstlane(sx), sys = __builtin_amdgcn_readfirstlane(sy), kys = __builtin_amdgcn_readfirstlane(ky);
        const bool lok = sxs > 0, rok = sxs + SEG < W;
        const bool y0 = (unsigned)(sys + kys - 1) < (unsigned)H, y1 = (unsigned)(sys + kys) < (unsigned)H;
#pragma unroll
        for (int j = 0; j < B_IPS; ++j) {
            unsigned long long v = real ? m_live[j] : 0ull;
            if (!lok) v &= ~m_left[j];
            if (!rok) v &= ~m_right[j];
            if (W16) { if (!y0) v &= m_r1[j]; if (!y1) v &= ~m_r1[j]; }
            else if (!y0) v = 0ull;
            v = ((unsigned long long)(unsigned)__builtin_amdgcn_readfirstlane((int)(v >> 32)) << 32) | (unsigned)__builtin_amdgcn_readfirstlane((int)v);
            asm("" : "+s"(v));
            const unsigned long long pa = (unsigned long long)(size_t)(xbase + boff[j]);
            unsigned plo, phi;
            asm("v_cndmask_b32_e64 %0, %1, %2, %3" : "=v"(plo) : "v"(zlo), "v"((unsigned)pa), "s"(v));
            asm("v_cndmask_b32_e64 %0, %1, %2, %3" : "=v"(phi) : "v"(zhi), "v"((unsigned)(pa >> 32)), "s"(v));
            const bool live = (j * 4096 + wave * 1024) < B_BYTES;
            glds16(reinterpret_cast<const void*>((size_t)(((unsigned long long)phi << 32) | plo)),
                   __builtin_amdgcn_readfirstlane(live ? sbase + A_BYTES + j * 4096 + wave * 1024 : dump));
        }
        ++sg_next;
        if (W16) {
            abase += a_step; xbase += x_step;
            sy += 2; if (sy >= H) sy = 0;
        } else {
            sx += 32;
            if (sx < (sstripe + 1) * SWp) { abase += a_step; xbase += x_step; }
            else {
                sx = sstripe * SWp; ++sy;
                if (sy >= H) { sy = 0; ++sstripe; if (sstripe >= nstripes) { sstripe = 0; ++simg; } sx = sstripe * SWp; }
                const size_t p = ((size_t)simg * H + sy) * W + sx;
                abase = dy0 + p * d.Cg * 2;
                xbase = x0p + p * d.Cin * 2;
            }
        }
    };

    f32x16_t acc[3][MT][NT];
#pragma unroll
    for (int kx = 0; kx < 3; ++kx)
#pragma unroll
        for (int mt = 0; mt < MT; ++mt)
#pragma unroll
            for (int nt = 0; nt < NT; ++nt)
#pragma unroll
                for (int r = 0; r < 16; ++r) acc[kx][mt][nt][r] = 0.f;

    const bool do_bias = d.dbias != nullptr && ky == 1 && tn == 0 && wn == 0;
    float bsum[MT];
#pragma unroll
    for (int mt = 0; mt < MT; ++mt) bsum[mt] = 0.f;

    const int i16 = lane & 15, g2 = lane >> 4;
    const int rsub = (g2 >> 1) * 8 + (i16 >> 2);
    const int csub = ((g2 & 1) * 16 + (i16 & 3) * 4) * 2;
    constexpr int ksb = W16 ? SEGP : 16;

    auto compute = [&](int slot) {
        const unsigned char* As = smem + slot * STAGE;
        const unsigned char* Bs = As + A_BYTES;
#pragma unroll
        for (int ks = 0; ks < 2; ++ks) {
            bf16x8_t a[MT];
            const int ra = ks * 16 + rsub;
#pragma unroll
            for (int mt = 0; mt < MT; ++mt) {
                const int col = ((wm * MT + mt) * 64 + csub) ^ (swz_a(ra) << 6);
                const unsigned char* p = As + ra * RBA + col;
                s16x4_t v0 = __builtin_amdgcn_ds_read_tr16_b64_v4i16((lds_s16x4_p)(p));
                s16x4_t v1 = __builtin_amdgcn_ds_read_tr16_b64_v4i16((lds_s16x4_p)(p + 4 * RBA));
                a[mt] = __builtin_bit_cast(bf16x8_t, __builtin_shufflevector(v0, v1, 0, 1, 2, 3, 4, 5, 6, 7));
                if (do_bias) {
                    typedef __attribute__((ext_vector_type(4))) unsigned u32x4_t;
                    const u32x4_t w = __builtin_bit_cast(u32x4_t, a[mt]);
#pragma unroll
                    for (int j = 0; j < 4; ++j) bsum[mt] += __uint_as_float(w[j] << 16) + __uint_as_float(w[j] & 0xffff0000u);
                }
            }
            static_for<0, 3>([&](auto kx_) {
                constexpr int kx = decltype(kx_)::value;
                bf16x8_t b[NT];
                const int rb = ks * ksb + kx + rsub;
#pragma unroll
                for (int nt = 0; nt < NT; ++nt) {
                    const int col = ((wn * NT + nt) * 64 + csub) ^ (swz_b(rb) << 6);
// ... 15 lines not shown
    for (int s = 0; s < NS - 1; ++s) issue(s);
    int slot = 0, islot = NS - 1;
    unsigned long long t_wait = 0, t_bar = 0, t_issue = 0, t_mfma = 0, t_begin = 0;
    if constexpr (PROBE) t_begin = wg3_stamp();
    for (int it = 0; it < nk; ++it) {
        unsigned long long s0 = 0, s1 = 0, s2 = 0, s3 = 0;
        if constexpr (PROBE) s0 = wg3_stamp();
        wait_vmcnt<(NS - 2) * IPS>();
        if constexpr (PROBE) s1 = wg3_stamp();
        __builtin_amdgcn_s_barrier();
        if constexpr (PROBE) s2 = wg3_stamp();
        issue(islot);
        if constexpr (PROBE) s3 = wg3_stamp();
        compute(slot);
        if constexpr (PROBE) { const unsigned long long s4 = wg3_stamp(); t_wait += s1 - s0; t_bar += s2 - s1; t_issue += s3 - s2; t_mfma += s4 - s3; }
        slot = (slot == NS - 1) ? 0 : slot + 1;
        islot = (islot == NS - 1) ? 0 : islot + 1;
    }
    wait_vmcnt<0>();
    unsigned long long t_loop_end = 0;
    if constexpr (PROBE) t_loop_end = wg3_stamp();

    if (do_bias) {
#pragma unroll
        for (int mt = 0; mt < MT; ++mt) {
            const float t = bsum[mt] + __shfl_xor(bsum[mt], 32);
            const int co = m0 + (wm * MT + mt) * 32 + l31;
            if (hi == 0 && co < d.Cg) wg_accum(d.dbias, d.det_stride, split, (size_t)co, t);
        }
    }

    static_for<0, 3 * MT * NT>([&](auto i_) {
        constexpr int kx = decltype(i_)::value / (MT * NT), mt = (decltype(i_)::value / NT) % MT, nt = decltype(i_)::value % NT;
        const int ci = n0 + (wn * NT + nt) * 32 + l31;
        if (ci >= d.Cin) return;
        const int tap = ky * 3 + kx;
#pragma unroll
        for (int r = 0; r < 16; ++r) {
            const int co = m0 + (wm * MT + mt) * 32 + (r & 3) + 8 * (r >> 2) + 4 * hi;
            if (co < d.Cg)
                wg_accum(d.dw, d.det_stride, split, (size_t)(tap * d.Cg + co) * d.Cin + ci, acc[kx][mt][nt][r]);
        }
    });
    if constexpr (PROBE) {
        const unsigned long long t_end = wg3_stamp();
        if (lane == 0 && g_mg_wg3_probe_out) {
            unsigned long long* o = g_mg_wg3_probe_out + ((size_t)blockIdx.x * 4 + wave) * 8;
            o[0] = t_wait; o[1] = t_bar; o[2] = t_issue; o[3] = t_mfma; o[4] = t_loop_end - t_begin; o[5] = t_end - t_loop_end; o[6] = (unsigned long long)nk; o[7] = t_begin;
        }
    }
}


template <int MT, int NT, bool W16>
int launch3(Wg3K& k, hipStream_t st, int* nsplit, bool dry)
{
    constexpr int TM = 64 * MT, TN = 64 * NT;
    constexpr int STAGE = 32 * TM * 2 + ((NT == 2) ? 36 : 40) * TN * 2;
    constexpr size_t LDS = 4 * (size_t)STAGE + 4096;
    k.tiles_m = (k.Cg + TM - 1) / TM;
    k.tiles_n = (k.Cin + TN - 1) / TN;
    const int stripe = mg_opt(MG_OPT_WGRAD3X3_STRIPE);
    k.stripe_w = (!W16 && stripe >= 32 && (stripe % 32) == 0 && k.W > stripe && (k.W % stripe) == 0) ? stripe : k.W;
    const long base = 3L * k.tiles_m * k.tiles_n;
    int S = k.splitk;
    if (S <= 0) {
        const int lo = (int)((384 + base - 1) / base), hi = (int)((1536 + base - 1) / base);
        S = k.nstg / 192 < hi ? k.nstg / 192 : hi;
        if (S < lo) S = lo;
        if (S > k.nstg / 16) S = k.nstg / 16;
        if (S < 1) S = 1;
    }
    if (S > k.nstg) S = k.nstg;
    k.sps = (k.nstg + S - 1) / S;
    S = (k.nstg + k.sps - 1) / k.sps;
    const long nblk = base * S;
    if (nsplit) *nsplit = S;
    if (dry) return MG_OK;
    if (nblk <= 0 || nblk > 0x7fffffffL) return mg_fail(MG_ERR_ARG, "mg_conv_wgrad: bad grid %ld", nblk);
    auto kern = wgrad3x3_kernel<MT, NT, W16>;
    constexpr size_t LDS_HALF_CU = LDS > 84 * 1024 ? LDS : 84 * 1024;
    const size_t lds_req = k.half_cu ? LDS_HALF_CU : LDS;
    mg_raise_lds_cap(reinterpret_cast<const void*>(kern), (int)LDS_HALF_CU);
#if MG_PROBES
    if constexpr (MT == 2 && NT == 2 && !W16) {
        if (mg_opt(MG_OPT_PROBE_WGRAD3X3)) {
            auto pk = wgrad3x3_kernel<MT, NT, W16, true>;
            mg_raise_lds_cap(reinterpret_cast<const void*>(pk), (int)LDS);
            hipLaunchKernelGGL(pk, dim3((unsigned)nblk), dim3(256), LDS, st, k);
            MG_CHECK_LAUNCH("mg_conv_wgrad(3x3 probe)");
            return MG_OK;
        }
    }
#endif
    hipLaunchKernelGGL(kern, dim3((unsigned)nblk), dim3(256), lds_req, st, k);
    MG_CHECK_LAUNCH("mg_conv_wgrad(3x3)");
    return MG_OK;
}

}

int wgrad3x3_set_probe(unsigned long long addr)
{
    unsigned long long* p = reinterpret_cast<unsigned long long*>(addr);
    return hipMemcpyToSymbol(HIP_SYMBOL(g_mg_wg3_probe_out), &p, sizeof(p)) == hipSuccess ? MG_OK : MG_ERR_ARG;
}

int launch_wgrad3x3(Wg3K& k, hipStream_t st, int* nsplit, bool dry)
{
    const bool m2 = k.Cg > 64, n2 = k.Cin > 64;
    if (k.W == 16) {
        if (m2 && n2) return launch3<2, 2, true>(k, st, nsplit, dry);
        if (m2)       return launch3<2, 1, true>(k, st, nsplit, dry);
        if (n2)       return launch3<1, 2, true>(k, st, nsplit, dry);
        return launch3<1, 1, true>(k, st, nsplit, dry);
    }
    if (m2 && n2) return launch3<2, 2, false>(k, st, nsplit, dry);
    if (m2)       return launch3<2, 1, false>(k, st, nsplit, dry);
    if (n2)       return launch3<1, 2, false>(k, st, nsplit, dry);
    return launch3<1, 1, false>(k, st, nsplit, dry);
}
```

### michigan_amd/csrc/mg_wgrad_common.h

```cpp
#pragma once
#include "mg_common.h"

struct Wg3K {
    const void* x; const void* dy; float* dw; float* dbias;
    int N, H, W, Cin, Cg;
    int nstg;
    int sps;
    int tiles_m, tiles_n;
    int splitk;
    long det_stride;
    int half_cu;
    int stripe_w;
};

__device__ __forceinline__ void wg_accum(float* base, long det_stride, int split, size_t idx, float v)
{
    if (det_stride) base[(size_t)split * det_stride + idx] = v;
    else atomicAdd(base + idx, v);
}
int launch_wgrad_det_finish(const float* ws, int nsplit, long stride, float* dw, long ndw, float* dbias, int nbias, hipStream_t st);

int launch_wgrad3x3(Wg3K& k, hipStream_t st, int* nsplit = nullptr, bool dry = false);
bool wgrad_thin_applies(const Wg3K& k);
int launch_wgrad_thin(Wg3K& k, hipStream_t st, int* nsplit = nullptr, bool dry = false);

struct WgT {
    const void* x; const void* dy; float* ws;
    int N, Hin, Win, Hj, Wj, ntaps;
    int HH, HW, dy0, dx0;
    long slab;
    int has_bias;
    int tap[MG_MAX_TAPS];
};
bool wgrad_thin_taps_applies(const mg_wgrad_desc* d);
int launch_wgrad_thin_taps(const mg_wgrad_desc* d, hipStream_t st, float* dw, float* dbias, long det_stride, int* nsplit, bool dry);
float* mg_stream_scratch(hipStream_t st, size_t bytes);
```

### michigan_amd/ops.py

```python
from __future__ import annotations

import ctypes
import os
import weakref
from typing import List, Optional, Sequence, Tuple

import torch
import torch.nn.functional as F

from . import _cabi as C

ACT_NONE, ACT_RELU, ACT_LRELU, ACT_TANH = C.MG_ACT_NONE, C.MG_ACT_RELU, C.MG_ACT_LRELU, C.MG_ACT_TANH

WGRAD_USE_TR = True
SYNC_BN_GROUP = None
SYNC_BN_ASYNC = os.environ.get("MG_SYNCBN_ASYNC", "0") == "1"
GRAD_SINK = True
WGRAD_DETERMINISTIC = os.environ.get("MG_DETERMINISTIC") == "1"


def set_deterministic(flag: bool = True) -> bool:
    global WGRAD_DETERMINISTIC
    prev, WGRAD_DETERMINISTIC = WGRAD_DETERMINISTIC, bool(flag)
    return prev
# ... 42 lines not shown
    return None if t is None else ctypes.c_void_p(t.data_ptr())


_RAW_STREAM = getattr(torch._C, "_cuda_getCurrentRawStream", None)


def _stream(t: torch.Tensor):
    if t.is_cuda:
        if _RAW_STREAM is not None:
            return ctypes.c_void_p(_RAW_STREAM(t.device.index))
        return ctypes.c_void_p(torch.cuda.current_stream(t.device).cuda_stream)
    return None


def _roundup(v: int, m: int) -> int:
    return (v + m - 1) // m * m


def _nhwc(t: torch.Tensor) -> torch.Tensor:
    if t.dim() != 4:
        raise ValueError(f"expected an NHWC 4-d tensor, got shape {tuple(t.shape)}")
    return t.contiguous()


def _set_taps(desc, taps: Sequence[Tuple[int, int]]):
    if not 1 <= len(taps) <= C.MG_MAX_TAPS:
        raise ValueError(f"{len(taps)} taps (max {C.MG_MAX_TAPS})")
    desc.ntaps = len(taps)
    for i, (dy, dx) in enumerate(taps):
        desc.tap_dy[i] = dy
        desc.tap_dx[i] = dx


def fwd_taps(kh: int, kw: int, pad: int, dilation: int = 1) -> List[Tuple[int, int]]:
    return [(ky * dilation - pad, kx * dilation - pad) for ky in range(kh) for kx in range(kw)]


def gemm_weight(weight: torch.Tensor, cin_pad: int) -> torch.Tensor:
    cout, cin, kh, kw = weight.shape
    w = weight.permute(2, 3, 0, 1).reshape(kh * kw, cout, cin)
    if cin_pad > cin:
        w = F.pad(w, (0, cin_pad - cin))
    return w


def pad_channels(x: torch.Tensor, mult: int = 8) -> torch.Tensor:
    c = x.shape[-1]
    cp = _roundup(c, mult)
    return x if cp == c else F.pad(x, (0, cp - c))


def _launch_conv(inp, wt, out, bias, taps, *, Hj, Wj, isy, isx, osy=1, osx=1, ooy=0, oox=0,
                 cout, cout_gemm, act=ACT_NONE, slope=0.2, resid=None,
                 spade_x=None, mean=None, rstd=None, gamma_out=None, algo_cin=None, relu_mask=None, x_up=False, mask_slope=0.0):
    d = C.ConvDesc()
    d.in_, d.wt, d.out = inp.data_ptr(), wt.data_ptr(), out.data_ptr()
    d.bias = bias.data_ptr() if bias is not None else None
    d.resid = resid.data_ptr() if resid is not None else None
    d.x = spade_x.data_ptr() if spade_x is not None else (relu_mask.data_ptr() if relu_mask is not None else None)
    d.mean = mean.data_ptr() if mean is not None else None
    d.rstd = rstd.data_ptr() if rstd is not None else None
    d.gamma_out = gamma_out.data_ptr() if gamma_out is not None else None
    d.dtype = _dt(inp)
    d.N, d.Hin, d.Win, d.Cin = inp.shape
    _, d.Hout, d.Wout, _ = out.shape
    d.Cout, d.Cout_gemm, d.CoutP = cout, cout_gemm, wt.shape[1]
    d.Hj, d.Wj, d.isy, d.isx = Hj, Wj, isy, isx
    d.osy, d.osx, d.ooy, d.oox = osy, osx, ooy, oox
    d.epilogue = C.MG_EPI_SPADE if spade_x is not None else C.MG_EPI_PLAIN
    d.act, d.slope = act, slope
    d.x_up = 1 if (x_up and spade_x is not None) else 0
    d.mask_slope = float(mask_slope) if relu_mask is not None else 0.0
    _set_taps(d, taps)
    assert wt.shape[0] == len(taps) and wt.shape[2] == inp.shape[3] and wt.dtype == inp.dtype
    C.backend().mg_conv_taps(d, _stream(inp))


def _arena_epoch(p) -> int:
    arena = getattr(p, "_mg_arena", None)
    return 0 if arena is None else arena.weight_epoch


def _param_state(params):
    return [(p._version, _arena_epoch(p)) for p in params]


class _ParamCache:
    PRUNE_ABOVE = 4096

    def __init__(self):
        self._entries = {}

    def get(self, key, params):
        ent = self._entries.get(key)
        if ent is None:
            return None
        for ref, (version, epoch), p in zip(ent[1], ent[0], params):
            if ref() is not p or p._version != version or _arena_epoch(p) != epoch:
                return None
        return ent[2]

    def only_epoch_moved(self, key, params) -> bool:
        ent = self._entries.get(key)
        return ent is not None and all(ref() is p and p._version == version for ref, (version, _), p in zip(ent[1], ent[0], params))

    def put(self, key, params, value):
        if len(self._entries) > self.PRUNE_ABOVE:
            self.prune()
        self._entries[key] = [_param_state(params), tuple(weakref.ref(p) for p in params), value]

    def restamp(self, key):
        ent = self._entries[key]
        ent[0] = _param_state([ref() for ref in ent[1]])

    def live(self, arena):
        for key, (_, refs, value) in list(self._entries.items()):
            params = [ref() for ref in refs]
            if all(p is not None for p in params) and getattr(params[0], "_mg_arena", None) is arena:
                yield key, params, value

    def prune(self):
        for key in [k for k, ent in self._entries.items() if any(ref() is None for ref in ent[1])]:
            del self._entries[key]


_PACK_CACHE = _ParamCache()
_BIAS_PAIR_CACHE = _ParamCache()
# ... 145 lines not shown

def expire_fold_expectations():
    for addr in [a for a, ref in _FOLD_EXPECTED.items() if ref is None or ref() is None]:
        del _FOLD_EXPECTED[addr]


def _weak_node(t):
    try:
        return weakref.ref(t.grad_fn) if t.grad_fn is not None else None
    except TypeError:
        return None


def reset_mask_protocol():
    _RELU_MASKED.clear()
    _FOLD_EXPECTED.clear()


_RELU_MASKED = {}
_FOLD_EXPECTED = {}
_DGRAD_CLASSES = {}
_DGRAD_PERM = {}


def _leave_mask_record(g: torch.Tensor, y: torch.Tensor):
    _RELU_MASKED[g.data_ptr()] = (y.data_ptr(), g._version)


def _take_mask_record(g: torch.Tensor, y: torch.Tensor) -> bool:
    return _RELU_MASKED.pop(g.data_ptr(), None) == (y.data_ptr(), g._version)


def _dgrad_classes(kh: int, kw: int, stride: int, pad: int):
    key = (kh, kw, stride, pad)
    if key not in _DGRAD_CLASSES:
        classes, order = [], []
        for py in range(stride):
            for px in range(stride):
                taps, lo = [], len(order)
                for ky in range(kh):
                    if (py + pad - ky) % stride:
                        continue
                    for kx in range(kw):
                        if (px + pad - kx) % stride:
                            continue
                        taps.append(((py + pad - ky) // stride, (px + pad - kx) // stride))
                        order.append(ky * kw + kx)
                classes.append((py, px, taps, (lo, len(order))))
        _DGRAD_CLASSES[key] = (classes, order)
    return _DGRAD_CLASSES[key]


def conv_dgrad(dy: torch.Tensor, wt: torch.Tensor, kh: int, kw: int, stride: int, pad: int,
               in_hw: Tuple[int, int], cin: int, relu_mask: Optional[torch.Tensor] = None, mask_slope: float = 0.0) -> torch.Tensor:
    n, ho, wo, cg8 = dy.shape
    t = kh * kw
    h, w = in_hw
    assert wt.shape[0] == t and wt.shape[2] == cg8
    classes, order = _dgrad_classes(kh, kw, stride, pad)
    full = all(taps for _, _, taps, _ in classes)
    dx = (torch.empty if full else torch.zeros)((n, h, w, cin), dtype=dy.dtype, device=dy.device)
    if stride > 1:
        pkey = (kh, kw, stride, pad, wt.device)
        if pkey not in _DGRAD_PERM:
            _DGRAD_PERM[pkey] = torch.tensor(order, dtype=torch.long, device=wt.device)
        wt = wt.index_select(0, _DGRAD_PERM[pkey])
    for py, px, taps, (lo, hi) in classes:
        hj, wj = len(range(py, h, stride)), len(range(px, w, stride))
        if hj == 0 or wj == 0 or not taps:
            continue
        _launch_conv(dy, wt[lo:hi], dx, None, taps, Hj=hj, Wj=wj, isy=1, isx=1,
                     osy=stride, osx=stride, ooy=py, oox=px, cout=cin, cout_gemm=cin, relu_mask=relu_mask, mask_slope=mask_slope)
    if relu_mask is not None:
        assert relu_mask.shape == dx.shape and relu_mask.dtype == dx.dtype
        _leave_mask_record(dx, relu_mask)
    return dx


def conv_wgrad(x: torch.Tensor, dy: torch.Tensor, kh: int, kw: int, stride: int, pad: int, want_bias: bool = False, out=None, beside: bool = False):
    n, h, w, cin = x.shape
    _, hj, wj, cg8 = dy.shape
    if out is not None:
        return _wgrad_launch(x, dy, fwd_taps(kh, kw, pad), stride, want_bias, out, beside)
    if _wgrad_swapped(stride, cg8, cin):
        swapped = _wgrad_launch(dy, x, [(pad - ky, pad - kx) for ky in range(kh) for kx in range(kw)], 1, False)
        dw = swapped.transpose(1, 2).contiguous()
        return (dw, channel_sums(dy)[0, 0].float()) if want_bias else dw
    return _wgrad_launch(x, dy, fwd_taps(kh, kw, pad), stride, want_bias)


WGRAD_SIDE_STREAM = os.environ.get("MG_WGRAD_STREAM", "1") != "0"
WGRAD_HALF_CU = os.environ.get("MG_WGRAD_HALF_CU", "1") != "0"
_WGRAD_STREAMS = {}
WGRAD_HELD_BUDGET = int(os.environ.get("MG_WGRAD_HELD_MB", "6144")) << 20


def streams_overlap(main, cand) -> bool:
    dev = main.device
    big = torch.empty(64 << 20, dtype=torch.float32, device=dev)
    small = torch.zeros(64, dtype=torch.float32, device=dev)
    torch.cuda.synchronize(dev)
    votes = 0
    for _ in range(3):
        e0, e1, e2 = (torch.cuda.Event(enable_timing=True) for _ in range(3))
        with torch.cuda.stream(main):
            e0.record(main)
            for _ in range(4):
                big.add_(1.0)
            e1.record(main)
        with torch.cuda.stream(cand):
            small.add_(1.0)
            e2.record(cand)
        torch.cuda.synchronize(dev)
        votes += int(e0.elapsed_time(e2) < 0.6 * e0.elapsed_time(e1))
    return votes >= 2


STREAM_PROBE = os.environ.get("MG_STREAM_PROBE", "1") != "0"
_STREAM_PROBE_LOG = []


def _new_side_stream(device):
    main = torch.cuda.current_stream(device)
    if not STREAM_PROBE:
        return torch.cuda.Stream(device=device)
    rejected = []
    for attempt in range(1, 9):
        cand = torch.cuda.Stream(device=device)
        if streams_overlap(main, cand):
            _STREAM_PROBE_LOG.append((device.index, attempt, True))
            _REJECTED_STREAMS.extend(rejected)
            return cand
        rejected.append(cand)
    _STREAM_PROBE_LOG.append((device.index, 8, False))
    _REJECTED_STREAMS.extend(rejected[1:])
    return rejected[0]


_REJECTED_STREAMS = []


class _SideStream:

    def __init__(self, device):
        self.stream = _new_side_stream(device)
        self.dirty = False
        self.held = []

    def hold(self, event, x, dy):
        held = self.held
        while held and held[0][0].query():
            held.pop(0)
        held.append((event, x, dy, x.numel() * x.element_size() + dy.numel() * dy.element_size()))
        over = sum(h[3] for h in held) - WGRAD_HELD_BUDGET
        while over > 0 and len(held) > 1:
            old = held.pop(0)
            torch.cuda.current_stream(x.device).wait_event(old[0])
            over -= old[3]

    def join(self):
        torch.cuda.current_stream(self.stream.device).wait_stream(self.stream)
        self.dirty = False
        self.held.clear()


def _wgrad_side(device) -> _SideStream:
    ent = _WGRAD_STREAMS.get(device.index)
    if ent is None:
        ent = _WGRAD_STREAMS[device.index] = _SideStream(device)
    return ent


def wgrad_join(device=None):
    for idx, ent in _WGRAD_STREAMS.items():
        if ent.dirty and (device is None or device.index == idx):
            ent.join()


def sink_wgrad(arena, slot, x, dy, kh, kw, stride, pad, need_b):
    if WGRAD_SIDE_STREAM and x.is_cuda:
        ent = _wgrad_side(x.device)
        side = ent.stream
        side.wait_stream(torch.cuda.current_stream(x.device))
        with torch.cuda.stream(side):
            conv_wgrad(x, dy, kh, kw, stride, pad, want_bias=need_b, out=(slot[1], slot[2]), beside=WGRAD_HALF_CU)
            arena.slot_written(slot[0])
            ev = torch.cuda.Event()
            ev.record(side)
        ent.dirty = True
        ent.hold(ev, x, dy)
        return
    conv_wgrad(x, dy, kh, kw, stride, pad, want_bias=need_b, out=(slot[1], slot[2]))
    arena.slot_written(slot[0])


BRANCH_STREAMS = int(os.environ.get("MG_BRANCH_STREAMS", "2"))


def side_stream(device):
    return _wgrad_side(device).stream


def _wgrad_swapped(stride: int, cg8: int, cin: int) -> bool:
    return stride == 1 and cg8 <= 8 and cin >= 32


def _wgrad_launch(x, dy, taps, stride, want_bias, out=None, beside=False):
    n, h, w, cin = x.shape
    _, hj, wj, cg8 = dy.shape
    ndw = len(taps) * cg8 * cin
    if out is not None:
        dw, dbias = out
        assert dw.shape == (len(taps), cg8, cin) and (dbias is not None or not want_bias)
        dbias = dbias if want_bias else None
    else:
        buf = torch.zeros(ndw + (cg8 if want_bias else 0), dtype=torch.float32, device=x.device)
        dw = buf[:ndw].view(len(taps), cg8, cin)
        dbias = buf[ndw:] if want_bias else None
    d = C.WgradDesc()
    d.x, d.dy, d.dw = x.data_ptr(), dy.data_ptr(), dw.data_ptr()
    d.dbias = dbias.data_ptr() if want_bias else None
    d.dtype = _dt(x)
    d.N, d.Hin, d.Win, d.Cin = n, h, w, cin
    d.Hj, d.Wj, d.Cg = hj, wj, cg8
    d.isy = d.isx = stride
    d.splitk = 0
    d.flags = (1 if (WGRAD_USE_TR and x.dtype == torch.bfloat16) else 0) | (2 if beside else 0)
    _set_taps(d, taps)
    assert dy.dtype == x.dtype
    if WGRAD_DETERMINISTIC:
        nbytes = int(C.backend().mg_wgrad_det_workspace(ctypes.byref(d)))
        if nbytes < 0:
            raise RuntimeError("mg_wgrad_det_workspace failed")
        ws = torch.empty(max(nbytes, 16), dtype=torch.uint8, device=x.device)
        d.det_ws, d.det_ws_bytes = ws.data_ptr(), nbytes
    C.backend().mg_conv_wgrad(d, _stream(x))
    return (dw, dbias) if want_bias else dw


def _stats_workspace(groups: int, p: int, c: int, device) -> torch.Tensor:
    return torch.empty(max(int(C.backend().mg_stats_workspace(groups, p, c)), 4), dtype=torch.uint8, device=device)


def channel_sums(x: torch.Tensor, groups: int = 1, shift: bool = False) -> torch.Tensor:
    c = x.shape[-1]
    p = x.numel() // (groups * c)
    be = C.backend()
    ws = _stats_workspace(groups, p, c, x.device)
    sums = torch.empty((groups, 2, c), dtype=torch.float64, device=x.device)
    be.mg_channel_stats(_p(x), _dt(x), groups, p, c, int(shift), _p(sums), _p(ws), _stream(x))
    return sums


def act_backward(dy: torch.Tensor, y: torch.Tensor, act: int, slope: float) -> torch.Tensor:
    if act == ACT_NONE:
        return dy
    dpre = torch.empty_like(dy)
    numel = dy.numel()
    if numel % 4:
        raise ValueError("act_backward needs numel % 4 == 0")
    C.backend().mg_act_bwd(_p(dy), _p(y), _p(dpre), _dt(dy), numel, act, slope, _stream(dy))
    return dpre


class _Conv2dFn(torch.autograd.Function):
    @staticmethod
    def forward(ctx, x, weight, bias, resid, stride, pad, act, slope, x_relu=False, sink=None, x_mask_slope=0.0):
        ctx.sink = sink
        ctx.x_mask_slope = float(x_mask_slope)
        x = _nhwc(x)
        n, h, w, cx = x.shape
        cout, cin, kh, kw = weight.shape
        if cx < cin or cx % 8:
            raise ValueError(f"conv2d: input has {cx} channels, weight expects {cin} (input must be >= and a multiple of 8)")
        ho = (h + 2 * pad - kh) // stride + 1
        wo = (w + 2 * pad - kw) // stride + 1
        wp = pack_weight(weight, None, x.dtype, _roundup(cout, 128), cx, 0)
        bp = bias.detach().float().contiguous() if bias is not None else None
        out = torch.empty((n, ho, wo, cout), dtype=x.dtype, device=x.device)
        if resid is not None:
            resid = _nhwc(resid)
            if resid.shape != out.shape or resid.dtype != out.dtype:
                raise ValueError("conv2d: residual must match the output")
        _launch_conv(x, wp, out, bp, fwd_taps(kh, kw, pad), Hj=ho, Wj=wo, isy=stride, isx=stride,
                     cout=cout, cout_gemm=cout, act=act, slope=slope, resid=resid, algo_cin=cin)
        ctx.save_for_backward(x, weight, out if act != ACT_NONE else None)
        ctx.cfg = (stride, pad, act, slope, bias is not None, resid is not None)
        ctx.x_relu = bool(x_relu)
        return out
# ... 198 lines not shown
            self.index = None

    def refresh(self):
        arena = self.arena()
        live = [(r0(), r1()) for r0, r1 in self.pairs]
        if arena is None or any(a is None or b is None for a, b in live):
            return False
        if self.index is None or self.flat_ptr != arena.flat.data_ptr():
            idx, msk, self.offsets, off, padded = [], [], [], 0, False
            for bg, bb in live:
                c = bg.numel()
                cr = _roundup(c, 32)
                o0, o1 = arena._span_of[id(bg)][0], arena._span_of[id(bb)][0]
                ch = torch.arange(cr).reshape(cr // 32, 1, 32)
                src = torch.cat([o0 + ch, o1 + ch], dim=1)
                ok = (ch < c).expand(cr // 32, 2, 32)
                padded = padded or cr != c
                idx.append(torch.where(ok, src, torch.zeros_like(src)).reshape(-1))
                msk.append(ok.reshape(-1))
                self.offsets.append((off, off + 2 * cr))
                off += 2 * cr
            dev = arena.flat.device
            self.index = torch.cat(idx).to(dev)
            self.mask = torch.cat(msk).to(dev).float() if padded else None
            self.flat_ptr = arena.flat.data_ptr()
        rows = torch.index_select(arena.flat.detach(), 0, self.index)
        if self.mask is not None:
            rows = rows * self.mask
        for (bg, bb), (a, b) in zip(live, self.offsets):
            _BIAS_PAIR_CACHE.put((bg.data_ptr(), bb.data_ptr()), (bg, bb), rows[a:b])
        return True


def spade_bias_rows(bg: torch.Tensor, bb: torch.Tensor) -> torch.Tensor:
    if not (isinstance(bg, torch.nn.Parameter) and isinstance(bb, torch.nn.Parameter)):
        return _interleave32(bg.detach().float(), bb.detach().float()).contiguous()
    key, params = (bg.data_ptr(), bb.data_ptr()), (bg, bb)
    hit = _BIAS_PAIR_CACHE.get(key, params)
    if hit is not None:
        return hit
    arena = getattr(bg, "_mg_arena", None)
    if arena is not None and getattr(bb, "_mg_arena", None) is arena and hasattr(arena, "_span_of") and BATCHED_PACK:
        plan = _BIAS_PLANS.get(arena)
        if plan is None:
            plan = _BIAS_PLANS[arena] = _BiasPlan(arena)
        plan.register(bg, bb)
        if plan.refresh():
            return _BIAS_PAIR_CACHE.get(key, params)
    rows = _interleave32(bg.detach().float(), bb.detach().float()).contiguous()
    _BIAS_PAIR_CACHE.put(key, params, rows)
    return rows


def _interleave32(a: torch.Tensor, b: torch.Tensor) -> torch.Tensor:
    c = a.numel()
    cr = _roundup(c, 32)
    if cr != c:
        a, b = F.pad(a, (0, cr - c)), F.pad(b, (0, cr - c))
    return torch.stack([a.reshape(cr // 32, 32), b.reshape(cr // 32, 32)], dim=1).reshape(2 * cr)


def _spade_branch_fwd(who, x, actv, wg, bg, wb, bb, mean, rstd, act, slope, need_g1, up=False):
    n, h, w = actv.shape[:3]
    c = x.shape[3]
    if wg.shape != wb.shape or wg.shape[0] != c or wg.shape[1] != actv.shape[3]:
        raise ValueError(f"{who}: mlp_gamma / mlp_beta weights have the wrong shape")
    kh = wg.shape[2]
    rows = 2 * _roundup(c, 32)
    wp = pack_weight(wg, wb, x.dtype, _roundup(rows, 128), actv.shape[3], 0)
    bias = spade_bias_rows(bg, bb)
    out = torch.empty((n, h, w, c), dtype=x.dtype, device=x.device)
    g1 = torch.empty_like(out) if need_g1 else None
    _launch_conv(actv, wp, out, bias, fwd_taps(kh, kh, kh // 2), Hj=h, Wj=w, isy=1, isx=1, cout=c, cout_gemm=rows,
                 act=act, slope=slope, spade_x=x, mean=mean, rstd=rstd, gamma_out=g1, x_up=up)
    return out, g1


def _spade_branch_reduce(dh, h, g1, x, mean, rstd, act, slope, sums, up=False):
    n, hh, ww, c = dh.shape
    p = n * hh * ww
    rows = 2 * _roundup(c, 32)
    be = C.backend()
    alloc = torch.zeros if rows != 2 * c else torch.empty
    dgb = alloc((n, hh, ww, rows), dtype=x.dtype, device=x.device)
    ws = _stats_workspace(1, p, c, x.device)
    if _grad_premasked(dh, h, act):
        act = ACT_NONE
    hp = _p(h) if act != ACT_NONE else None
    if up:
        be.mg_norm_bwd_reduce_up(_p(dh), hp, _p(x), _p(g1), _dt(x), n, hh, ww, c, _p(mean), _p(rstd), act, slope,
                                 _p(dgb), _p(sums), _p(ws), _stream(x))
    else:
        be.mg_norm_bwd_reduce(_p(dh), hp, _p(x), _p(g1), _dt(x), 1, p, c, _p(mean), _p(rstd), act, slope,
                              _p(dgb), _p(sums), _p(ws), _stream(x))
    return dgb, act, hp


def _spade_branch_grads(needs, sink, actv, dgb, wg, wb, actv_relu):
    hh, ww, rows = dgb.shape[1:]
    c, kh = wg.shape[0], wg.shape[2]
    pad = kh // 2
    dactv = dwg = dbg = dwb = dbb = None
    if needs[0]:
        wt = pack_weight(wg, wb, dgb.dtype, _roundup(actv.shape[3], 128), rows, 1)
        dactv = conv_dgrad(dgb, wt, kh, kh, 1, pad, (hh, ww), actv.shape[3],
                           relu_mask=actv if (actv_relu and FUSE_RELU_MASK) else None)
    need_w = needs[1] or needs[3]
    need_b = needs[2] or needs[4]
    slot = db = None
    if sink is not None and needs[1] and needs[3]:
        slot = sink[0].grad_slot(wg, wb, sink[2] if need_b else None, sink[3] if need_b else None, kh * kh, rows, actv.shape[3], None)
    if slot is not None:
        sink_wgrad(sink[0], slot, actv, dgb, kh, kh, 1, pad, need_b)
    elif need_w:
        res = conv_wgrad(actv, dgb, kh, kh, 1, pad, want_bias=need_b)
        dwg, dwb = unpack_wgrad(res[0] if need_b else res, wg.shape, two=True)
        db = res[1] if need_b else None
    elif need_b:
        db = channel_sums(dgb)[0, 0].float()
    if db is not None:
        db = db.reshape(rows // 64, 2, 32)
        dbg, dbb = db[:, 0].reshape(-1)[:c], db[:, 1].reshape(-1)[:c]
    return dactv, dwg, dbg, dwb, dbb


class _SpadeFn(torch.autograd.Function):
    @staticmethod
    def forward(ctx, x, actv, w_gamma, b_gamma, w_beta, b_beta, mean, rstd, count, act, slope, actv_relu=False, sink=None):
        ctx.actv_relu = bool(actv_relu)
        ctx.sink = sink
        x, actv = _nhwc(x), _nhwc(actv)
        if actv.shape[:3] != x.shape[:3] or actv.dtype != x.dtype:
            raise ValueError("spade_modulate: activation map and x disagree in shape/dtype")
        out, g1 = _spade_branch_fwd("spade_modulate", x, actv, w_gamma, b_gamma, w_beta, b_beta, mean, rstd, act, slope,
                                    any(ctx.needs_input_grad))
        if g1 is not None:
            ctx.save_for_backward(x, actv, w_gamma, w_beta, out, g1, mean, rstd)
        ctx.cfg = (count, act, slope)
        return out

    @staticmethod
    def backward(ctx, dh):
        x, actv, w_gamma, w_beta, h, g1, mean, rstd = ctx.saved_tensors
        count, act, slope = ctx.cfg
        dh = dh.contiguous()
        n, hh, ww, c = x.shape
        sums = torch.empty((1, 2, c), dtype=torch.float32, device=x.device)
        dgb, act, hp = _spade_branch_reduce(dh, h, g1, x, mean, rstd, act, slope, sums)
        dx = work = None
        if ctx.needs_input_grad[0] and SYNC_BN_GROUP is not None:
            work = _sync_bn_all_reduce(sums, "syncbn_bwd")
        dactv, dwg, dbg, dwb, dbb = _spade_branch_grads(ctx.needs_input_grad[1:6], ctx.sink, actv, dgb, w_gamma, w_beta, ctx.actv_relu)
        if ctx.needs_input_grad[0]:
            if work is not None:
                work.wait()
            dx = torch.empty_like(x)
            C.backend().mg_norm_bwd_apply(_p(dh), hp, _p(x), _p(g1), _dt(x), 1, n * hh * ww, c, _p(mean), _p(rstd),
                                          _p(sums[0, 0]), _p(sums[0, 1]), 2 * c, 1.0 / float(count), act, slope, _p(dx), _stream(x))
        return dx, dactv, dwg, dbg, dwb, dbb, None, None, None, None, None, None, None


class _SpadePairFn(torch.autograd.Function):

    @staticmethod
    def forward(ctx, x, actv0, wg0, bg0, wb0, bb0, actv1, wg1, bg1, wb1, bb1, mean, rstd, count, act0, act1, slope, up, relu0, relu1, sinks):
        x, actv0, actv1 = _nhwc(x), _nhwc(actv0), _nhwc(actv1)
        n, hs, ws, c = x.shape
        h, w = (2 * hs, 2 * ws) if up else (hs, ws)
        if actv0.shape[:3] != (n, h, w) or actv1.shape[:3] != (n, h, w) or actv0.dtype != x.dtype or actv1.dtype != x.dtype:
            raise ValueError("spade_modulate_pair: activation maps and x disagree in shape / dtype")
        need = any(ctx.needs_input_grad)
        (out0, g10), (out1, g11) = (_spade_branch_fwd("spade_modulate_pair", x, actv, wg, bg, wb, bb, mean, rstd, act, slope, need, up)
                                    for actv, wg, bg, wb, bb, act in ((actv0, wg0, bg0, wb0, bb0, act0), (actv1, wg1, bg1, wb1, bb1, act1)))
        if need:
            ctx.save_for_backward(x, actv0, wg0, wb0, out0, g10, actv1, wg1, wb1, out1, g11, mean, rstd)
        ctx.cfg = (count, (act0, act1), slope, bool(up), (bool(relu0), bool(relu1)), sinks, (h, w))
        return out0, out1

    @staticmethod
    def backward(ctx, dh0, dh1):
        x, actv0, wg0, wb0, h0, g10, actv1, wg1, wb1, h1, g11, mean, rstd = ctx.saved_tensors
        count, acts, slope, up, relus, sinks, (hh, ww) = ctx.cfg
        n, _, _, c = x.shape
        need_x = ctx.needs_input_grad[0]
        sums = torch.empty((2, 2, c), dtype=torch.float32, device=x.device)
        branches = ((dh0.contiguous(), h0, g10, actv0, wg0, wb0, 1), (dh1.contiguous(), h1, g11, actv1, wg1, wb1, 6))
        reduced = [_spade_branch_reduce(dh, h, g1, x, mean, rstd, acts[b], slope, sums[b], up)
                   for b, (dh, h, g1, *_r) in enumerate(branches)]
        work = None
        if need_x and SYNC_BN_GROUP is not None:
            work = _sync_bn_all_reduce(sums, "syncbn_bwd")
        grads = [None] * 11
        for b, (dh, h, g1, actv, wg, wb, base) in enumerate(branches):
            grads[base:base + 5] = _spade_branch_grads(ctx.needs_input_grad[base:base + 5], sinks[b], actv, reduced[b][0], wg, wb, relus[b])
        if need_x:
            if work is not None:
                work.wait()
            d = C.NormApply2Desc()
            for b, (dh, h, g1, *_r) in enumerate(branches):
                act = reduced[b][1]
                d.dh[b], d.g1[b], d.sums[b] = dh.data_ptr(), g1.data_ptr(), sums[b].data_ptr()
                d.h[b] = h.data_ptr() if act != ACT_NONE else None
                d.act[b], d.slope[b] = act, slope
            d.x, d.mean, d.rstd = x.data_ptr(), mean.data_ptr(), rstd.data_ptr()
            dx = torch.empty_like(x)
            d.dx, d.P, d.dtype, d.C = dx.data_ptr(), n * hh * ww, _dt(x), c
            d.up, d.H, d.W, d.inv_count = (1 if up else 0), hh, ww, 1.0 / float(count)
            C.backend().mg_norm_bwd_apply2(d, _stream(x))
            grads[0] = dx
        return tuple(grads) + (None,) * 10


def spade_pair_supported(x: torch.Tensor) -> bool:
    return bool(C.backend().mg_norm_apply2_supported(_dt(x), x.shape[-1])) and x.numel() * 4 < (1 << 32)


def spade_modulate_pair(x, mods, mean, rstd, count, *, acts, slope=0.2, up=False):
    (a0, wg0, bg0, wb0, bb0), (a1, wg1, bg1, wb1, bb1) = mods
    sk0, sk1 = _sink_for(wg0, bg0, wb0, bb0), _sink_for(wg1, bg1, wb1, bb1)
    sinks = (None if sk0 is None else (sk0[0], sk0[1], bg0, bb0), None if sk1 is None else (sk1[0], sk1[1], bg1, bb1))
    return _SpadePairFn.apply(x, a0, wg0, bg0, wb0, bb0, a1, wg1, bg1, wb1, bb1, mean, rstd, count, acts[0], acts[1], slope, bool(up),
                              getattr(a0, "_mg_relu_out", False), getattr(a1, "_mg_relu_out", False), sinks)


def spade_modulate(x, actv, w_gamma, b_gamma, w_beta, b_beta, mean, rstd, count, *, act=ACT_NONE, slope=0.2):
    sk = _sink_for(w_gamma, b_gamma, w_beta, b_beta)
    return _SpadeFn.apply(x, actv, w_gamma, b_gamma, w_beta, b_beta, mean, rstd, count, act, slope,
                          getattr(actv, "_mg_relu_out", False), None if sk is None else (sk[0], sk[1], b_gamma, b_beta))


class _InstanceNormActFn(torch.autograd.Function):
    @staticmethod
    def forward(ctx, x, eps, act, slope):
        x = _nhwc(x)
        n, h, w, c = x.shape
        p = h * w
        if FUSED_STATS_FINALIZE:
            mean, rstd, _ = stats_finalize(x, n, float(p), eps)
        else:
            sums = channel_sums(x, groups=n, shift=True)
            mean = torch.empty((n, c), dtype=torch.float32, device=x.device)
# ... 1134 lines not shown
```

Before: 131.7 images/s.

## Read SPADE dbeta directly from dh instead of materializing interleaved dgamma/dbeta tensor

In the SPADE backward pass, when dh is already the pre-activation gradient, the norm reduce now writes only dgamma. The dgrad halo conv and the wgrad kernels then read a two-source input, alternating 32-channel blocks between dgamma and dh (dbeta equals dh). This removes writing and rereading the interleaved 2C-channel dgb tensor, cutting memory traffic and allocation at each SPADE layer. It adds new kernel variants, a routing check that falls back to the old path, and more code paths that must stay consistent.

```diff
diff --git a/include/michigan_hip/spade_dbeta.h b/include/michigan_hip/spade_dbeta.h
--- /dev/null
+++ b/include/michigan_hip/spade_dbeta.h
@@ -0,0 +1,28 @@
+#ifndef MICHIGAN_HIP_SPADE_DBETA_H
+#define MICHIGAN_HIP_SPADE_DBETA_H
+
+#include "../michigan_hip.h"
+
+#ifdef __cplusplus
+extern "C" {
+#endif
+
+int mgs_norm_bwd_reduce(const void* dh, const void* h, const void* x, const void* g1,
+                        int32_t dtype, int32_t G, int64_t P, int32_t C,
+                        const float* mean, const float* rstd, int32_t act, float slope,
+                        void* dgamma, float* sums, void* partial, void* stream);
+int mgs_norm_bwd_reduce_up(const void* dh, const void* h, const void* x, const void* g1,
+                           int32_t dtype, int32_t N, int32_t H, int32_t W, int32_t C,
+                           const float* mean, const float* rstd, int32_t act, float slope,
+                           void* dgamma, float* sums, void* partial, void* stream);
+
+int mgs_conv_taps2(const mg_conv_desc* d, const void* in_odd, void* stream);
+
+int mgs_conv_wgrad2(const mg_wgrad_desc* d, const void* dy_odd, void* stream);
+
+int mgs_spade_dbeta_route(int32_t dtype, int32_t N, int32_t H, int32_t W, int32_t C, int32_t Cact, int32_t wgrad_flags);
+
+#ifdef __cplusplus
+}
+#endif
+#endif
diff --git a/michigan_amd/_cabi.py b/michigan_amd/_cabi.py
--- a/michigan_amd/_cabi.py
+++ b/michigan_amd/_cabi.py
@@ -178,6 +178,16 @@
     "mge_brush_u8": ([_vp, _vp, _i32, _i32, _i32, _i32, _vp], _i32),
     "mge_morph_u8": ([_vp, _vp, _i32, _i32, _i32, _i32, _i32, _vp, _i32, _i32, _i32, _vp], _i32),
 }
+_SPADE_PROTOS = {
+    "mgs_norm_bwd_reduce": ([_vp, _vp, _vp, _vp, _i32, _i32, _i64, _i32, _vp, _vp, _i32, _f32, _vp, _vp, _vp, _vp], _i32),
+    "mgs_norm_bwd_reduce_up": ([_vp, _vp, _vp, _vp, _i32, _i32, _i32, _i32, _i32, _vp, _vp, _i32, _f32, _vp, _vp, _vp, _vp], _i32),
+    "mgs_conv_taps2": ([ctypes.POINTER(ConvDesc), _vp, _vp], _i32),
+    "mgs_conv_wgrad2": ([ctypes.POINTER(WgradDesc), _vp, _vp], _i32),
+    "mgs_spade_dbeta_route": ([_i32, _i32, _i32, _i32, _i32, _i32, _i32], _i32),
+}
+_EXT_PROTOS = {**_EDIT_PROTOS, **_SPADE_PROTOS}
+_EXT_NO_STATUS = {"mgs_spade_dbeta_route"}
+_EXT_BY_REF = {"mgs_conv_taps2", "mgs_conv_wgrad2"}
 EXPORTED_SYMBOLS = tuple(_PROTOS)
 _NO_STATUS = {"mg_wgrad_det_workspace", "mg_norm_apply2_supported", "mg_grad_slot_blocks", "mg_pack_job_blocks", "mg_sn_layer_blocks", "mg_stats_workspace", "mg_sizeof_desc", "mg_abi_version", "mg_last_error", "mg_noise_field_len", "mg_bicubic_ksize",
               "mg_feat_moment_workspace"}
@@ -204,7 +214,7 @@
                 "michigan_amd has no CPU / eager-PyTorch fallback.")
         import torch
         self._lib = ctypes.CDLL(path)
-        for fn, (argtypes, restype) in list(_PROTOS.items()) + list(_EDIT_PROTOS.items()):
+        for fn, (argtypes, restype) in list(_PROTOS.items()) + list(_EXT_PROTOS.items()):
             f = getattr(self._lib, fn)
             f.argtypes, f.restype = argtypes, restype
         if self._lib.mg_abi_version() != MG_ABI_VERSION:
@@ -213,12 +223,12 @@
             raise RuntimeError("ctypes mirror of the descriptor structs is out of sync with include/michigan_hip.h")
 
     def __getattr__(self, fn):
-        if fn not in _PROTOS and fn not in _EDIT_PROTOS:
+        if fn not in _PROTOS and fn not in _EXT_PROTOS:
             raise AttributeError(fn)
         raw = getattr(self._lib, fn)
-        if fn in _NO_STATUS:
+        if fn in _NO_STATUS or fn in _EXT_NO_STATUS:
             return raw
-        by_ref = fn in _BY_REF
+        by_ref = fn in _BY_REF or fn in _EXT_BY_REF
 
         def call(*args):
             if by_ref:
diff --git a/michigan_amd/csrc/mg_conv.hip b/michigan_amd/csrc/mg_conv.hip
--- a/michigan_amd/csrc/mg_conv.hip
+++ b/michigan_amd/csrc/mg_conv.hip
@@ -415,10 +415,9 @@
 }
 
 template <typename T>
-bool halo_applies(const ConvK& k)
+bool halo_shape_ok(const ConvK& k)
 {
     constexpr int CH = ROWB / (int)sizeof(T);
-    if (!mg_opt(MG_OPT_CONV_HALO)) return false;
     if (k.ntaps != 9 || k.isy != 1 || k.isx != 1 || k.osy != 1 || k.osx != 1 || k.ooy != 0 || k.oox != 0) return false;
     if (k.Hj != k.Hin || k.Wj != k.Win || k.Hout != k.Hin || k.Wout != k.Win) return false;
     if (k.Cin % CH || k.Cout_gemm <= 32 || k.Hin < 8 || k.Win < 16) return false;
@@ -429,10 +428,23 @@
         if (dy < -1 || dy > 1 || dx < -1 || dx > 1) return false;
         seen |= 1u << ((dy + 1) * 3 + dx + 1);
     }
-    if (seen != 0x1ffu) return false;
+    return seen == 0x1ffu;
+}
+
+template <typename T>
+bool halo_applies(const ConvK& k)
+{
+    if (!mg_opt(MG_OPT_CONV_HALO) || !halo_shape_ok<T>(k)) return false;
     const int th = k.Cout_gemm <= 64 ? 16 : 8, tmh = k.Cout_gemm <= 64 ? 64 : 128;
     const long wgs = (long)k.N * ((k.Hin + th - 1) / th) * ((k.Win + 15) / 16) * ((k.Cout_gemm + tmh - 1) / tmh);
     return wgs >= 384;
+}
+
+template <typename T>
+bool routes_to_halo(const ConvK& k, int epilogue)
+{
+    return !conv_thin_applies(k, ET<T>::DT, epilogue) && !conv_thin_taps_applies(k, ET<T>::DT, epilogue) && !conv_dot_applies(k, ET<T>::DT, epilogue) &&
+           !conv_fewout_applies(k, ET<T>::DT, epilogue) && !conv_halo64_applies(k, ET<T>::DT, epilogue) && halo_applies<T>(k);
 }
 
 template <typename T>
@@ -451,7 +463,7 @@
 
 float* mg_stream_scratch(hipStream_t st, size_t bytes) { return splitk_workspace(st, bytes); }
 
-extern "C" int mg_conv_taps(const mg_conv_desc* d, void* stream)
+static int check_conv_desc(const mg_conv_desc* d)
 {
     MG_CHECK_ARG(d != nullptr, "mg_conv_taps: null descriptor");
     MG_CHECK_ARG(d->in && d->wt && d->out, "mg_conv_taps: null tensor pointer");
@@ -476,8 +488,12 @@
         MG_CHECK_ARG(d->Cout <= d->Cout_gemm, "mg_conv_taps: Cout > Cout_gemm");
         MG_CHECK_ARG(d->mask_slope >= 0.f && d->mask_slope <= 1.f, "mg_conv_taps: mask_slope %g outside [0, 1]", (double)d->mask_slope);
     }
-    ConvK k;
-    k.in = d->in; k.wt = d->wt; k.out = d->out; k.bias = d->bias; k.resid = d->resid; k.x = d->x;
+    return MG_OK;
+}
+
+static void fill_convk(ConvK& k, const mg_conv_desc* d)
+{
+    k.in = d->in; k.in2 = nullptr; k.wt = d->wt; k.out = d->out; k.bias = d->bias; k.resid = d->resid; k.x = d->x;
     k.mean = d->mean; k.rstd = d->rstd; k.gamma_out = d->gamma_out;
     k.N = d->N; k.Hin = d->Hin; k.Win = d->Win; k.Cin = d->Cin;
     k.Hout = d->Hout; k.Wout = d->Wout; k.Cout = d->Cout; k.Cout_gemm = d->Cout_gemm; k.CoutP = d->CoutP;
@@ -492,6 +508,70 @@
     k.wide = ((mg_opt(MG_OPT_CONV_WIDE) && d->dtype == MG_BF16 && (d->Cout % 8) == 0) ? 1 : 0) | (probe ? 2 : 0) | (probe == 6 ? 4 : 0) | (mg_opt(MG_OPT_PROBE_NOXPRE) ? 8 : 0);
     for (int t = 0; t < MG_MAX_TAPS; ++t)
         k.tap[t] = t < d->ntaps ? (int)((((uint32_t)(int)d->tap_dy[t]) & 0xffffu) | (((uint32_t)(int)d->tap_dx[t]) << 16)) : 0;
+}
+
+extern "C" int mg_conv_taps(const mg_conv_desc* d, void* stream)
+{
+    const int rc = check_conv_desc(d);
+    if (rc != MG_OK) return rc;
+    ConvK k;
+    fill_convk(k, d);
     hipStream_t st = reinterpret_cast<hipStream_t>(stream);
     return d->dtype == MG_BF16 ? dispatch_conv<uint16_t>(k, d->epilogue, st) : dispatch_conv<float>(k, d->epilogue, st);
 }
+
+static int check_conv_taps2(const mg_conv_desc* d, const void* in_odd, const char* who)
+{
+    const int rc = check_conv_desc(d);
+    if (rc != MG_OK) return rc;
+    MG_CHECK_ARG(in_odd != nullptr, "%s: null second source", who);
+    MG_CHECK_ARG(d->dtype == MG_BF16 && d->epilogue == MG_EPI_PLAIN, "%s: bf16 and the plain epilogue only", who);
+    MG_CHECK_ARG((d->Cin % 64) == 0, "%s: Cin=%d must be a multiple of 64 (whole [32 | 32] blocks)", who, d->Cin);
+    MG_CHECK_ARG(d->Cout_gemm > 64, "%s: Cout_gemm=%d must be above 64", who, d->Cout_gemm);
+    MG_CHECK_ARG((long)d->N * d->Hin * d->Win * d->Cin < (1L << 31), "%s: input too large", who);
+    return MG_OK;
+}
+
+extern "C" int mgs_conv_taps2(const mg_conv_desc* d, const void* in_odd, void* stream)
+{
+    const int rc = check_conv_taps2(d, in_odd, "mgs_conv_taps2");
+    if (rc != MG_OK) return rc;
+    ConvK k;
+    fill_convk(k, d);
+    MG_CHECK_ARG(halo_shape_ok<uint16_t>(k), "mgs_conv_taps2: not a 3x3 / stride 1 / same-size convolution the halo-tile kernel takes");
+    k.in2 = in_odd;
+    return launch_conv_halo(k, MG_BF16, MG_EPI_PLAIN, reinterpret_cast<hipStream_t>(stream));
+}
+
+bool conv_taps2_routed(const mg_conv_desc* d)
+{
+    if (d == nullptr || d->dtype != MG_BF16 || d->epilogue != MG_EPI_PLAIN || d->Cin <= 0 || (d->Cin % 64) || d->Cout_gemm <= 64) return false;
+    if (d->ntaps < 1 || d->ntaps > MG_MAX_TAPS) return false;
+    ConvK k;
+    fill_convk(k, d);
+    return routes_to_halo<uint16_t>(k, MG_EPI_PLAIN);
+}
+
+bool wgrad2_routed(const mg_wgrad_desc* d);
+bool norm_reduce_dgamma_ok(int dtype, int C);
+
+extern "C" int mgs_spade_dbeta_route(int32_t dtype, int32_t N, int32_t H, int32_t W, int32_t C, int32_t Cact, int32_t wgrad_flags)
+{
+    if (dtype != MG_BF16 || N <= 0 || H <= 0 || W <= 0 || C <= 0 || (C % 32) || Cact <= 0 || (Cact % 8)) return 0;
+    if ((long)N * H * W >= (1L << 30) || (long)N * H * W * 2 * C >= (1L << 31) || 4L * C > 8192) return 0;
+    if (!norm_reduce_dgamma_ok(dtype, C)) return 0;
+    mg_conv_desc cd = {};
+    cd.dtype = dtype; cd.epilogue = MG_EPI_PLAIN;
+    cd.N = N; cd.Hin = cd.Hout = cd.Hj = H; cd.Win = cd.Wout = cd.Wj = W; cd.Cin = 2 * C;
+    cd.Cout = cd.Cout_gemm = Cact; cd.CoutP = (Cact + 127) / 128 * 128;
+    cd.isy = cd.isx = cd.osy = cd.osx = 1;
+    mg_wgrad_desc wd = {};
+    wd.dtype = dtype; wd.N = N; wd.Hin = wd.Hj = H; wd.Win = wd.Wj = W; wd.Cin = Cact; wd.Cg = 2 * C;
+    wd.isy = wd.isx = 1; wd.flags = wgrad_flags;
+    cd.ntaps = wd.ntaps = 9;
+    for (int t = 0; t < 9; ++t) {
+        cd.tap_dy[t] = (int8_t)(1 - t / 3); cd.tap_dx[t] = (int8_t)(1 - t % 3);
+        wd.tap_dy[t] = (int8_t)(t / 3 - 1); wd.tap_dx[t] = (int8_t)(t % 3 - 1);
+    }
+    return (conv_taps2_routed(&cd) && wgrad2_routed(&wd)) ? 1 : 0;
+}
diff --git a/michigan_amd/csrc/mg_conv_common.h b/michigan_amd/csrc/mg_conv_common.h
--- a/michigan_amd/csrc/mg_conv_common.h
+++ b/michigan_amd/csrc/mg_conv_common.h
@@ -28,6 +28,7 @@
     int wide;
     int x_up;
     float mslope;
+    const void* in2;
 };
 namespace {
 
diff --git a/michigan_amd/csrc/mg_conv_halo.hip b/michigan_amd/csrc/mg_conv_halo.hip
--- a/michigan_amd/csrc/mg_conv_halo.hip
+++ b/michigan_amd/csrc/mg_conv_halo.hip
@@ -34,9 +34,10 @@
     return v;
 }
 
-template <typename T, int EPI, int WM, int NT, int PROBE = 0>
+template <typename T, int EPI, int WM, int NT, int PROBE = 0, bool SRC2 = false>
 __global__ __launch_bounds__(NTHR, (NT == 4 || sizeof(T) == 4 ? 2 : 3)) void conv3x3_halo_kernel(const ConvK d)
 {
+    static_assert(!SRC2 || (sizeof(T) == 2 && EPI == MG_EPI_PLAIN && PROBE == 0), "two-source input: the bf16 data-gradient kernel only");
     using G = HaloGeom<WM, NT>;
     constexpr int PF = RING - 1;
     constexpr int MT = 2, WN = G::WN;
@@ -76,14 +77,18 @@
     const unsigned char* const zsrc = g_mg_zeros + (lane & 3) * 16;
 
     const unsigned char* pp[P_IPS];
+    const int pitch = SRC2 ? d.Cin >> 1 : d.Cin;
+    unsigned inside = 0;
 #pragma unroll
     for (int j = 0; j < P_IPS; ++j) {
         const int r = (wave + 4 * j) * 16 + lrow;
         const int pr = r / PW, pc = r - pr * PW;
         const int iy = y0 + pr - 1, ix = x0 + pc - 1;
         const bool ok = r < PROWS && (unsigned)iy < (unsigned)d.Hin && (unsigned)ix < (unsigned)d.Win;
-        pp[j] = ok ? reinterpret_cast<const unsigned char*>(In + ((size_t)((img * d.Hin + iy) * d.Win + ix) * d.Cin + piece * EPP)) : zsrc;
-    }
+        pp[j] = ok ? reinterpret_cast<const unsigned char*>(In + ((size_t)((img * d.Hin + iy) * d.Win + ix) * pitch + piece * EPP)) : zsrc;
+        if (SRC2 && ok) inside |= 1u << j;
+    }
+    const long src_delta = SRC2 ? reinterpret_cast<const unsigned char*>(d.in2) - reinterpret_cast<const unsigned char*>(d.in) : 0L;
     const unsigned char* wbase = reinterpret_cast<const unsigned char*>(d.wt) + (size_t)m0 * d.Cin * sizeof(T);
     unsigned woff[A_IPS];
 #pragma unroll
@@ -94,13 +99,22 @@
 
     const int nchunk = d.Cin / CH;
 
-    auto issue_patch = [&](int buf) {
+    auto issue_patch = [&](int buf, bool odd) {
         const unsigned base = lds0 + G::PATCH0 + buf * PSTAGE;
 #pragma unroll
         for (int j = 0; j < P_IPS; ++j) {
             const int blk = wave + 4 * j;
-            glds16(pp[j], __builtin_amdgcn_readfirstlane(base + blk * 1024));
-            pp[j] += ROWB;
+            if constexpr (SRC2) {
+                const unsigned char* src = pp[j];
+                if (odd) {
+                    if ((inside >> j) & 1u) src += src_delta;
+                    pp[j] += ROWB;
+                }
+                glds16(src, __builtin_amdgcn_readfirstlane(base + blk * 1024));
+            } else {
+                glds16(pp[j], __builtin_amdgcn_readfirstlane(base + blk * 1024));
+                pp[j] += ROWB;
+            }
         }
     };
     auto issue_a = [&](int slot, bool last_tap) {
@@ -232,7 +246,7 @@
     }
     float* const par = reinterpret_cast<float*>(smem + G::PAR);
     conv_stage_params_dma<TM_H, EPI, 4>(d, m0, lds0 + G::PAR, wave, lane);
-    issue_patch(0);
+    issue_patch(0, false);
 #pragma unroll
     for (int i = 0; i < PF; ++i) issue_a(i, false);
 
@@ -260,7 +274,7 @@
                     if constexpr (t < 7) issue_a((t + 2) % 3, t == 6);
                     else { if (next_chunk) issue_a((t + 2) % 3, false); }
                 }
-                if constexpr (t == 0) { if (next_chunk) issue_patch((c + 1) & 1); }
+                if constexpr (t == 0) { if (next_chunk) issue_patch((c + 1) & 1, ((c + 1) & 1) != 0); }
                 compute(t_, t % 3, std::false_type{});
 #pragma unroll
                 for (int nt = 0; nt < NT; ++nt) boff[t][nt] += pdelta;
@@ -298,7 +312,7 @@
                 __builtin_amdgcn_s_barrier();
                 if constexpr (t < 7) issue_a((t + 2) % 3, t == 6);
                 else { if (next_chunk) issue_a((t + 2) % 3, false); }
-                if constexpr (t == 0) { if (next_chunk) issue_patch((c + 1) & 1); }
+                if constexpr (t == 0) { if (next_chunk) issue_patch((c + 1) & 1, ((c + 1) & 1) != 0); }
                 compute(t_, t % 3, std::bool_constant<ZERO_C && decltype(first_)::value && t == 0>{});
 #pragma unroll
                 for (int nt = 0; nt < NT; ++nt) boff[t][nt] += pdelta;
@@ -334,7 +348,7 @@
     conv_epilogue<T, MT, NT, EPI, TM_H>(d, acc, m0, pixmap, wm, wn, l31, hi, par, EpiNoMark(), xpre, xpre_ok);
 }
 
-template <typename T, int EPI, int WM, int NT, int PROBE = 0>
+template <typename T, int EPI, int WM, int NT, int PROBE = 0, bool SRC2 = false>
 int launch_halo_g(ConvK& k, hipStream_t st)
 {
     using G = HaloGeom<WM, NT>;
@@ -343,7 +357,7 @@
     k.tiles_x = (k.Win + TW - 1) / TW;
     const long nblk = (long)k.N * k.tiles_y * k.tiles_x * k.tiles_m;
     if (nblk <= 0 || nblk > 0x7fffffffL) return mg_fail(MG_ERR_ARG, "mg_conv_taps(halo): bad grid %ld", nblk);
-    auto kern = conv3x3_halo_kernel<T, EPI, WM, NT, PROBE>;
+    auto kern = conv3x3_halo_kernel<T, EPI, WM, NT, PROBE, SRC2>;
     int lds = G::LDS;
 #if MG_PROBES
     lds += mg_opt(MG_OPT_PROBE_HALO_LDSPAD);
@@ -389,8 +403,21 @@
     return hipMemcpyToSymbol(HIP_SYMBOL(g_mg_probe_out), &p, sizeof(p)) == hipSuccess ? MG_OK : MG_ERR_ARG;
 }
 
+static int launch_halo_src2(ConvK& k, hipStream_t st)
+{
+    const long big = (long)k.N * ((k.Hin + 15) / 16) * ((k.Win + 15) / 16) * ((k.Cout_gemm + 127) / 128);
+    const long small = (long)k.N * ((k.Hin + 7) / 8) * ((k.Win + 15) / 16) * ((k.Cout_gemm + 127) / 128);
+    if (mg_opt(MG_OPT_CONV_HALO_BIG) && k.Hin >= 16 && (big >= 1024 || small < 384))
+        return launch_halo_g<uint16_t, MG_EPI_PLAIN, 2, 4, 0, true>(k, st);
+    return launch_halo_g<uint16_t, MG_EPI_PLAIN, 2, 2, 0, true>(k, st);
+}
+
 int launch_conv_halo(ConvK& k, int dtype, int epilogue, hipStream_t st)
 {
+    if (k.in2 != nullptr) {
+        if (dtype != MG_BF16 || epilogue != MG_EPI_PLAIN || k.Cout_gemm <= 64) return mg_fail(MG_ERR_UNSUPPORTED, "halo kernel: two-source input is bf16 / plain / Cout_gemm > 64 only");
+        return launch_halo_src2(k, st);
+    }
     if (dtype == MG_BF16)
         return epilogue == MG_EPI_SPADE ? launch_halo<uint16_t, MG_EPI_SPADE>(k, st) : launch_halo<uint16_t, MG_EPI_PLAIN>(k, st);
     return epilogue == MG_EPI_SPADE ? launch_halo<float, MG_EPI_SPADE>(k, st) : launch_halo<float, MG_EPI_PLAIN>(k, st);
diff --git a/michigan_amd/csrc/mg_norm.hip b/michigan_amd/csrc/mg_norm.hip
--- a/michigan_amd/csrc/mg_norm.hip
+++ b/michigan_amd/csrc/mg_norm.hip
@@ -118,7 +118,7 @@
 __global__ __launch_bounds__(MG_NTHR) void bwd_stage1_quad(
     const T* __restrict__ x, const T* __restrict__ dh, const T* __restrict__ h, const T* __restrict__ g1,
     const float* __restrict__ mean, const float* __restrict__ rstd, T* __restrict__ dgb,
-    float* __restrict__ partial, int64_t P, int C, int tpr, int rpb, int64_t chunk, int act, float slope, int up, int H, int W)
+    float* __restrict__ partial, int64_t P, int C, int tpr, int rpb, int64_t chunk, int act, float slope, int up, int H, int W, int gonly)
 {
     __shared__ float red[MG_NTHR * 8];
     const int g = blockIdx.y, c4 = C / 4;
@@ -151,7 +151,8 @@
                     s[j] += d.dxh; ss[j] += d.dxh * xh;
                     dgam[j] = d.dpre * xh; dbet[j] = d.dpre;
                 }
-                if (dgb) {
+                if (dgb && gonly) ET<T>::store4(dgb + o, dgam);
+                else if (dgb) {
                     const size_t ob = ((size_t)g * P + p) * Cr2 + (size_t)(c >> 5) * 64 + (c & 31);
                     ET<T>::store4(dgb + ob, dgam);
                     ET<T>::store4(dgb + ob + 32, dbet);
@@ -374,7 +375,7 @@
     join_to_partial(s, ss, red, cv, rows, tr == 0, partial, C, c);
 }
 
-template <typename T, int PIX, bool HAS_H, bool UP>
+template <typename T, int PIX, bool HAS_H, bool UP, bool GONLY = false>
 __global__ __launch_bounds__(MG_NTHR) void bwd_stage1_vec(const T* __restrict__ x, const T* __restrict__ dh, const T* __restrict__ h, const T* __restrict__ g1,
                                                      const float* __restrict__ mean, const float* __restrict__ rstd, T* __restrict__ dgb,
                                                      float* __restrict__ partial, int64_t P, int C, int64_t chunk, float neg, int H, int W)
@@ -418,7 +419,8 @@
                     s[j] += d.dxh; ss[j] += d.dxh * xh;
                     dgam[j] = d.dpre * xh; dbet[j] = d.dpre;
                 }
-                if (dgb) {
+                if constexpr (GONLY) EV<T>::store(dgb + base + (size_t)p * C, dgam);
+                else if (dgb) {
                     EV<T>::store(dgb + gbase + (size_t)p * Cr2, dgam);
                     EV<T>::store(dgb + gbase + (size_t)p * Cr2 + 32, dbet);
                 }
@@ -558,9 +560,29 @@
     } else
         mg_by_bool(h != nullptr, [&](auto hh) {
             hipLaunchKernelGGL((bwd_stage1_quad<T, hh.value>), grid, dim3(MG_NTHR), 0, st, (const T*)x, (const T*)dh, (const T*)h, (const T*)g1,
-                               mean, rstd, (T*)dgb, (float*)partial, P, C, sg.tpr, sg.rpb, sg.chunk, act, slope, up, H, W); });
+                               mean, rstd, (T*)dgb, (float*)partial, P, C, sg.tpr, sg.rpb, sg.chunk, act, slope, up, H, W, 0); });
     MG_CHECK_LAUNCH("reduce_stage1");
     dim3 grid2((2 * C + 31) / 32, G);
+    hipLaunchKernelGGL(reduce_stage2, grid2, dim3(256), 0, st, (const float*)partial, sums, sg.nchunks, 2 * C);
+    MG_CHECK_LAUNCH("reduce_stage2");
+    return MG_OK;
+}
+
+template <typename T>
+int run_reduce_dgamma(const void* x, const void* dh, const void* g1, const float* mean, const float* rstd,
+                      void* dgamma, int64_t P, int C, float* sums, void* partial, hipStream_t st, int up, int H, int W)
+{
+    const StatGeom sg = stat_geom(1, P, C);
+    dim3 grid(sg.nchunks, 1);
+    if (mg_opt(MG_OPT_NORM_BWD_VEC) && takes_vec<T>(C, MG_ACT_NONE))
+        mg_by_bool(up != 0, [&](auto upf) {
+            hipLaunchKernelGGL((bwd_stage1_vec<T, 2, false, upf.value, true>), grid, dim3(MG_NTHR), 0, st, (const T*)x, (const T*)dh, (const T*)nullptr,
+                               (const T*)g1, mean, rstd, (T*)dgamma, (float*)partial, P, C, sg.chunk, 1.f, H, W); });
+    else
+        hipLaunchKernelGGL((bwd_stage1_quad<T, false>), grid, dim3(MG_NTHR), 0, st, (const T*)x, (const T*)dh, (const T*)nullptr, (const T*)g1,
+                           mean, rstd, (T*)dgamma, (float*)partial, P, C, sg.tpr, sg.rpb, sg.chunk, MG_ACT_NONE, 0.f, up, H, W, 1);
+    MG_CHECK_LAUNCH("reduce_stage1 (d gamma)");
+    dim3 grid2((2 * C + 31) / 32, 1);
     hipLaunchKernelGGL(reduce_stage2, grid2, dim3(256), 0, st, (const float*)partial, sums, sg.nchunks, 2 * C);
     MG_CHECK_LAUNCH("reduce_stage2");
     return MG_OK;
@@ -649,6 +671,42 @@
                                      void* dgb, float* sums, void* partial, void* stream)
 {
     return norm_bwd_reduce("mg_norm_bwd_reduce_up", dh, h, x, g1, dtype, 1, (int64_t)N * H * W, C, mean, rstd, act, slope, dgb, sums, partial, stream, 1, N, H, W);
+}
+
+bool norm_reduce_dgamma_ok(int dtype, int C)
+{
+    return dtype == MG_BF16 && C > 0 && (C % 32) == 0 && C <= 4096;
+}
+
+static int norm_bwd_reduce_dgamma(const char* name, const void* dh, const void* h, const void* x, const void* g1,
+                                  int32_t dtype, int32_t G, int64_t P, int32_t C, const float* mean, const float* rstd, int32_t act,
+                                  void* dgamma, float* sums, void* partial, void* stream, int up, int32_t N, int32_t H, int32_t W)
+{
+    MG_CHECK_NORM_GEOM(name);
+    MG_CHECK_ARG(dh && x && mean && rstd && dgamma && sums && partial, "%s: null pointer", name);
+    MG_CHECK_ARG(h == nullptr && act == MG_ACT_NONE, "%s: the gradient must already be masked (act NONE, no h)", name);
+    MG_CHECK_ARG(G == 1, "%s: G must be 1", name);
+    if (up) MG_CHECK_ARG(N > 0 && H > 0 && W > 0 && (H % 2) == 0 && (W % 2) == 0 && P < (1L << 31), "%s: H, W must be even", name);
+    if (!norm_reduce_dgamma_ok(dtype, C)) return mg_fail(MG_ERR_UNSUPPORTED, "%s: bf16 with C=%d a multiple of 32 only", name, C);
+    return run_reduce_dgamma<uint16_t>(x, dh, g1, mean, rstd, dgamma, P, C, sums, partial, reinterpret_cast<hipStream_t>(stream), up, H, W);
+}
+
+extern "C" int mgs_norm_bwd_reduce(const void* dh, const void* h, const void* x, const void* g1,
+                                   int32_t dtype, int32_t G, int64_t P, int32_t C,
+                                   const float* mean, const float* rstd, int32_t act, float slope,
+                                   void* dgamma, float* sums, void* partial, void* stream)
+{
+    (void)slope;
+    return norm_bwd_reduce_dgamma("mgs_norm_bwd_reduce", dh, h, x, g1, dtype, G, P, C, mean, rstd, act, dgamma, sums, partial, stream, 0, 0, 0, 0);
+}
+
+extern "C" int mgs_norm_bwd_reduce_up(const void* dh, const void* h, const void* x, const void* g1,
+                                      int32_t dtype, int32_t N, int32_t H, int32_t W, int32_t C,
+                                      const float* mean, const float* rstd, int32_t act, float slope,
+                                      void* dgamma, float* sums, void* partial, void* stream)
+{
+    (void)slope;
+    return norm_bwd_reduce_dgamma("mgs_norm_bwd_reduce_up", dh, h, x, g1, dtype, 1, (int64_t)N * H * W, C, mean, rstd, act, dgamma, sums, partial, stream, 1, N, H, W);
 }
 
 template <typename T>
diff --git a/michigan_amd/csrc/mg_wgrad.hip b/michigan_amd/csrc/mg_wgrad.hip
--- a/michigan_amd/csrc/mg_wgrad.hip
+++ b/michigan_amd/csrc/mg_wgrad.hip
@@ -332,7 +332,17 @@
 
 namespace {
 
-int route_wgrad(const mg_wgrad_desc* d, hipStream_t st, float* dw, float* dbias, long det_stride, int* nsplit, bool dry)
+bool takes_wgrad3x3(const mg_wgrad_desc* d)
+{
+    if (!(mg_opt(MG_OPT_WGRAD3X3) && d->dtype == MG_BF16 && (d->flags & 1) && d->ntaps == 9 && d->isy == 1 && d->isx == 1 &&
+          d->Hin == d->Hj && d->Win == d->Wj && (d->Win == 16 || d->Win % 32 == 0) && (d->Hin * d->Win) % 32 == 0 &&
+          d->Cin >= 64 && d->Cg >= 64)) return false;
+    bool std3x3 = true;
+    for (int t = 0; t < 9; ++t) std3x3 = std3x3 && d->tap_dy[t] == t / 3 - 1 && d->tap_dx[t] == t % 3 - 1;
+    return std3x3;
+}
+
+int route_wgrad(const mg_wgrad_desc* d, hipStream_t st, float* dw, float* dbias, long det_stride, int* nsplit, bool dry, const void* dy2 = nullptr)
 {
     WgK k;
     k.x = d->x; k.dy = d->dy; k.dw = dw; k.dbias = dbias;
@@ -345,26 +355,21 @@
         bool std3x3 = true;
         for (int t = 0; t < 9; ++t) std3x3 = std3x3 && d->tap_dy[t] == t / 3 - 1 && d->tap_dx[t] == t % 3 - 1;
         Wg3K k3;
-        k3.x = d->x; k3.dy = d->dy; k3.dw = dw; k3.dbias = dbias;
+        k3.x = d->x; k3.dy = d->dy; k3.dy2 = nullptr; k3.dw = dw; k3.dbias = dbias;
         k3.N = d->N; k3.H = d->Hin; k3.W = d->Win; k3.Cin = d->Cin; k3.Cg = d->Cg;
         k3.nstg = 0; k3.sps = 0; k3.tiles_m = k3.tiles_n = 0; k3.splitk = 0; k3.det_stride = det_stride; k3.half_cu = 0; k3.stripe_w = 0;
         if (std3x3 && wgrad_thin_applies(k3)) return launch_wgrad_thin(k3, st, nsplit, dry);
     }
-    if (wgrad_thin_taps_applies(d)) return launch_wgrad_thin_taps(d, st, dw, dbias, det_stride, nsplit, dry);
-    if (mg_opt(MG_OPT_WGRAD3X3) && d->dtype == MG_BF16 && (d->flags & 1) && d->ntaps == 9 && d->isy == 1 && d->isx == 1 &&
-        d->Hin == d->Hj && d->Win == d->Wj && (d->Win == 16 || d->Win % 32 == 0) && (d->Hin * d->Win) % 32 == 0 &&
-        d->Cin >= 64 && d->Cg >= 64) {
-        bool std3x3 = true;
-        for (int t = 0; t < 9; ++t) std3x3 = std3x3 && d->tap_dy[t] == t / 3 - 1 && d->tap_dx[t] == t % 3 - 1;
-        if (std3x3) {
-            Wg3K k3;
-            k3.x = d->x; k3.dy = d->dy; k3.dw = dw; k3.dbias = dbias;
-            k3.N = d->N; k3.H = d->Hin; k3.W = d->Win; k3.Cin = d->Cin; k3.Cg = d->Cg;
-            k3.nstg = k.K / 32; k3.sps = 0; k3.tiles_m = k3.tiles_n = 0; k3.splitk = d->splitk; k3.det_stride = det_stride;
-            k3.half_cu = (d->flags & 2) ? 1 : 0; k3.stripe_w = 0;
-            return launch_wgrad3x3(k3, st, nsplit, dry);
-        }
-    }
+    if (dy2 == nullptr && wgrad_thin_taps_applies(d)) return launch_wgrad_thin_taps(d, st, dw, dbias, det_stride, nsplit, dry);
+    if (takes_wgrad3x3(d)) {
+        Wg3K k3;
+        k3.x = d->x; k3.dy = d->dy; k3.dy2 = dy2; k3.dw = dw; k3.dbias = dbias;
+        k3.N = d->N; k3.H = d->Hin; k3.W = d->Win; k3.Cin = d->Cin; k3.Cg = d->Cg;
+        k3.nstg = k.K / 32; k3.sps = 0; k3.tiles_m = k3.tiles_n = 0; k3.splitk = d->splitk; k3.det_stride = det_stride;
+        k3.half_cu = (d->flags & 2) ? 1 : 0; k3.stripe_w = 0;
+        return launch_wgrad3x3(k3, st, nsplit, dry);
+    }
+    if (dy2 != nullptr) return mg_fail(MG_ERR_UNSUPPORTED, "mgs_conv_wgrad2: not a launch of the 3x3 kernel-row weight gradient");
     if (d->dtype == MG_BF16)
         return (d->flags & 1) ? launch_wgrad<uint16_t, true>(k, st, nsplit, dry) : launch_wgrad<uint16_t, false>(k, st, nsplit, dry);
     return launch_wgrad<float, false>(k, st, nsplit, dry);
@@ -394,20 +399,43 @@
     return (int64_t)S * slab * (int64_t)sizeof(float);
 }
 
-extern "C" int mg_conv_wgrad(const mg_wgrad_desc* d, void* stream)
-{
-    const int rc = check_wgrad_desc(d, "mg_conv_wgrad");
-    if (rc != MG_OK) return rc;
+static int conv_wgrad(const mg_wgrad_desc* d, const void* dy2, void* stream)
+{
     hipStream_t st = reinterpret_cast<hipStream_t>(stream);
-    if (d->det_ws == nullptr) return route_wgrad(d, st, d->dw, d->dbias, 0, nullptr, false);
+    if (d->det_ws == nullptr) return route_wgrad(d, st, d->dw, d->dbias, 0, nullptr, false, dy2);
     int S = 0;
-    if (route_wgrad(d, st, d->dw, d->dbias, 0, &S, true) != MG_OK || S <= 0) return mg_fail(MG_ERR_ARG, "mg_conv_wgrad: cannot size the deterministic workspace");
+    if (route_wgrad(d, st, d->dw, d->dbias, 0, &S, true, dy2) != MG_OK || S <= 0) return mg_fail(MG_ERR_ARG, "mg_conv_wgrad: cannot size the deterministic workspace");
     const long ndw = (long)d->ntaps * d->Cg * d->Cin, nbias = d->dbias ? d->Cg : 0, slab = ndw + nbias;
     MG_CHECK_ARG(d->det_ws_bytes >= (int64_t)S * slab * (int64_t)sizeof(float), "mg_conv_wgrad: deterministic workspace too small (%ld splits)", (long)S);
     float* ws = reinterpret_cast<float*>(d->det_ws);
     int S2 = 0;
-    const int r2 = route_wgrad(d, st, ws, d->dbias ? ws + ndw : nullptr, slab, &S2, false);
+    const int r2 = route_wgrad(d, st, ws, d->dbias ? ws + ndw : nullptr, slab, &S2, false, dy2);
     if (r2 != MG_OK) return r2;
     if (S2 != S) return mg_fail(MG_ERR_LAUNCH, "mg_conv_wgrad: split count changed between sizing and launch (%d vs %d)", S, S2);
     return launch_wgrad_det_finish(ws, S, slab, d->dw, ndw, d->dbias, (int)nbias, st);
 }
+
+extern "C" int mg_conv_wgrad(const mg_wgrad_desc* d, void* stream)
+{
+    const int rc = check_wgrad_desc(d, "mg_conv_wgrad");
+    if (rc != MG_OK) return rc;
+    return conv_wgrad(d, nullptr, stream);
+}
+
+bool wgrad2_routed(const mg_wgrad_desc* d)
+{
+    if (d == nullptr || d->Cin == 8 || (d->Cg % 64) != 0) return false;
+    return !wgrad_thin_taps_applies(d) && takes_wgrad3x3(d);
+}
+
+extern "C" int mgs_conv_wgrad2(const mg_wgrad_desc* d, const void* dy_odd, void* stream)
+{
+    const int rc = check_wgrad_desc(d, "mgs_conv_wgrad2");
+    if (rc != MG_OK) return rc;
+    MG_CHECK_ARG(dy_odd != nullptr, "mgs_conv_wgrad2: null second source");
+    MG_CHECK_ARG(d->dtype == MG_BF16, "mgs_conv_wgrad2: bf16 only");
+    MG_CHECK_ARG((d->Cg % 64) == 0, "mgs_conv_wgrad2: Cg=%d must be a multiple of 64 (whole [32 | 32] blocks)", d->Cg);
+    MG_CHECK_ARG((long)d->N * d->Hj * d->Wj * d->Cg < (1L << 31), "mgs_conv_wgrad2: dY too large");
+    if (!takes_wgrad3x3(d)) return mg_fail(MG_ERR_UNSUPPORTED, "mgs_conv_wgrad2: not a launch of the 3x3 kernel-row weight gradient");
+    return conv_wgrad(d, dy_odd, stream);
+}
diff --git a/michigan_amd/csrc/mg_wgrad3x3.hip b/michigan_amd/csrc/mg_wgrad3x3.hip
--- a/michigan_amd/csrc/mg_wgrad3x3.hip
+++ b/michigan_amd/csrc/mg_wgrad3x3.hip
@@ -16,7 +16,7 @@
     return v;
 }
 
-template <int MT, int NT, bool W16, bool PROBE = false>
+template <int MT, int NT, bool W16, bool PROBE = false, bool SRC2 = false>
 __global__ __launch_bounds__(256, 2) void wgrad3x3_kernel(const Wg3K d)
 {
     constexpr int TM = 64 * MT, TN = 64 * NT;
@@ -64,13 +64,19 @@
     auto swz_a = [](int row) { return RBA == 256 ? (row & 3) : ((row >> 1) & 1); };
     auto swz_b = [](int row) { return RBB == 256 ? (row & 3) : ((row >> 1) & 1); };
 
+    const int a_pitch = SRC2 ? d.Cg : d.Cg * 2;
     int aoff[A_IPS];
+    long aoff2[SRC2 ? A_IPS : 1];
 #pragma unroll
     for (int j = 0; j < A_IPS; ++j) {
         const int g = j * 256 + tid, row = g / PPA, slot = g % PPA;
         int ch = m0 + ((slot ^ (swz_a(row) << 2)) << 3);
         if (ch >= d.Cg) ch = m0;
         aoff[j] = (row * d.Cg + ch) * 2;
+        if constexpr (SRC2) {
+            const long delta = reinterpret_cast<const unsigned char*>(d.dy2) - reinterpret_cast<const unsigned char*>(d.dy);
+            aoff2[j] = (long)(row * a_pitch + ((ch >> 6) * 32 + (ch & 31)) * 2) + (((ch >> 5) & 1) ? delta : 0L);
+        }
     }
     int boff[B_IPS], brc[B_IPS];
 #pragma unroll
@@ -89,7 +95,7 @@
     int simg = 0, sstripe = 0;
     const int SWp = W16 ? W : d.stripe_w, nsegs = SWp / 32, nstripes = W / SWp;
     if (W16) {
-        abase = dy0 + (size_t)sbeg * 32 * d.Cg * 2;
+        abase = dy0 + (size_t)sbeg * 32 * a_pitch;
         xbase = x0p + (size_t)sbeg * 32 * d.Cin * 2;
         const int rem = (sbeg * 32) % (H * W); sy = rem / W; sx = rem - sy * W;
     } else {
@@ -100,12 +106,12 @@
         sy = r / nsegs;
         sx = sstripe * SWp + (r - sy * nsegs) * 32;
         const size_t p = ((size_t)simg * H + sy) * W + sx;
-        abase = dy0 + p * d.Cg * 2;
+        abase = dy0 + p * a_pitch;
         xbase = x0p + p * d.Cin * 2;
     }
     sy = __builtin_amdgcn_readfirstlane(sy); sx = __builtin_amdgcn_readfirstlane(sx);
     simg = __builtin_amdgcn_readfirstlane(simg); sstripe = __builtin_amdgcn_readfirstlane(sstripe);
-    const int a_step = 32 * d.Cg * 2, x_step = 32 * d.Cin * 2;
+    const int a_step = 32 * a_pitch, x_step = 32 * d.Cin * 2;
 
     unsigned long long m_live[B_IPS], m_left[B_IPS], m_right[B_IPS], m_r1[B_IPS];
 #pragma unroll
@@ -125,8 +131,10 @@
         const unsigned sbase = lds0 + stage * STAGE;
         if (real) {
 #pragma unroll
-            for (int j = 0; j < A_IPS; ++j)
-                glds16_s(abase, (unsigned)aoff[j], __builtin_amdgcn_readfirstlane(sbase + j * 4096 + wave * 1024));
+            for (int j = 0; j < A_IPS; ++j) {
+                if constexpr (SRC2) glds16(abase + aoff2[j], __builtin_amdgcn_readfirstlane(sbase + j * 4096 + wave * 1024));
+                else glds16_s(abase, (unsigned)aoff[j], __builtin_amdgcn_readfirstlane(sbase + j * 4096 + wave * 1024));
+            }
         } else {
 #pragma unroll
             for (int j = 0; j < A_IPS; ++j)
@@ -163,7 +171,7 @@
                 sx = sstripe * SWp; ++sy;
                 if (sy >= H) { sy = 0; ++sstripe; if (sstripe >= nstripes) { sstripe = 0; ++simg; } sx = sstripe * SWp; }
                 const size_t p = ((size_t)simg * H + sy) * W + sx;
-                abase = dy0 + p * d.Cg * 2;
+                abase = dy0 + p * a_pitch;
                 xbase = x0p + p * d.Cin * 2;
             }
         }
@@ -285,7 +293,7 @@
 }
 
 
-template <int MT, int NT, bool W16>
+template <int MT, int NT, bool W16, bool SRC2>
 int launch3(Wg3K& k, hipStream_t st, int* nsplit, bool dry)
 {
     constexpr int TM = 64 * MT, TN = 64 * NT;
@@ -311,12 +319,12 @@
     if (nsplit) *nsplit = S;
     if (dry) return MG_OK;
     if (nblk <= 0 || nblk > 0x7fffffffL) return mg_fail(MG_ERR_ARG, "mg_conv_wgrad: bad grid %ld", nblk);
-    auto kern = wgrad3x3_kernel<MT, NT, W16>;
+    auto kern = wgrad3x3_kernel<MT, NT, W16, false, SRC2>;
     constexpr size_t LDS_HALF_CU = LDS > 84 * 1024 ? LDS : 84 * 1024;
     const size_t lds_req = k.half_cu ? LDS_HALF_CU : LDS;
     mg_raise_lds_cap(reinterpret_cast<const void*>(kern), (int)LDS_HALF_CU);
 #if MG_PROBES
-    if constexpr (MT == 2 && NT == 2 && !W16) {
+    if constexpr (MT == 2 && NT == 2 && !W16 && !SRC2) {
         if (mg_opt(MG_OPT_PROBE_WGRAD3X3)) {
             auto pk = wgrad3x3_kernel<MT, NT, W16, true>;
             mg_raise_lds_cap(reinterpret_cast<const void*>(pk), (int)LDS);
@@ -339,17 +347,23 @@
     return hipMemcpyToSymbol(HIP_SYMBOL(g_mg_wg3_probe_out), &p, sizeof(p)) == hipSuccess ? MG_OK : MG_ERR_ARG;
 }
 
-int launch_wgrad3x3(Wg3K& k, hipStream_t st, int* nsplit, bool dry)
+template <bool SRC2>
+static int launch_wgrad3x3_s(Wg3K& k, hipStream_t st, int* nsplit, bool dry)
 {
     const bool m2 = k.Cg > 64, n2 = k.Cin > 64;
     if (k.W == 16) {
-        if (m2 && n2) return launch3<2, 2, true>(k, st, nsplit, dry);
-        if (m2)       return launch3<2, 1, true>(k, st, nsplit, dry);
-        if (n2)       return launch3<1, 2, true>(k, st, nsplit, dry);
-        return launch3<1, 1, true>(k, st, nsplit, dry);
-    }
-    if (m2 && n2) return launch3<2, 2, false>(k, st, nsplit, dry);
-    if (m2)       return launch3<2, 1, false>(k, st, nsplit, dry);
-    if (n2)       return launch3<1, 2, false>(k, st, nsplit, dry);
-    return launch3<1, 1, false>(k, st, nsplit, dry);
-}
+        if (m2 && n2) return launch3<2, 2, true, SRC2>(k, st, nsplit, dry);
+        if (m2)       return launch3<2, 1, true, SRC2>(k, st, nsplit, dry);
+        if (n2)       return launch3<1, 2, true, SRC2>(k, st, nsplit, dry);
+        return launch3<1, 1, true, SRC2>(k, st, nsplit, dry);
+    }
+    if (m2 && n2) return launch3<2, 2, false, SRC2>(k, st, nsplit, dry);
+    if (m2)       return launch3<2, 1, false, SRC2>(k, st, nsplit, dry);
+    if (n2)       return launch3<1, 2, false, SRC2>(k, st, nsplit, dry);
+    return launch3<1, 1, false, SRC2>(k, st, nsplit, dry);
+}
+
+int launch_wgrad3x3(Wg3K& k, hipStream_t st, int* nsplit, bool dry)
+{
+    return k.dy2 ? launch_wgrad3x3_s<true>(k, st, nsplit, dry) : launch_wgrad3x3_s<false>(k, st, nsplit, dry);
+}
diff --git a/michigan_amd/csrc/mg_wgrad_common.h b/michigan_amd/csrc/mg_wgrad_common.h
--- a/michigan_amd/csrc/mg_wgrad_common.h
+++ b/michigan_amd/csrc/mg_wgrad_common.h
@@ -11,6 +11,7 @@
     long det_stride;
     int half_cu;
     int stripe_w;
+    const void* dy2;
 };
 
 __device__ __forceinline__ void wg_accum(float* base, long det_stride, int split, size_t idx, float v)
diff --git a/michigan_amd/ops.py b/michigan_amd/ops.py
--- a/michigan_amd/ops.py
+++ b/michigan_amd/ops.py
@@ -118,7 +118,7 @@
 
 def _launch_conv(inp, wt, out, bias, taps, *, Hj, Wj, isy, isx, osy=1, osx=1, ooy=0, oox=0,
                  cout, cout_gemm, act=ACT_NONE, slope=0.2, resid=None,
-                 spade_x=None, mean=None, rstd=None, gamma_out=None, algo_cin=None, relu_mask=None, x_up=False, mask_slope=0.0):
+                 spade_x=None, mean=None, rstd=None, gamma_out=None, algo_cin=None, relu_mask=None, x_up=False, mask_slope=0.0, in_odd=None):
     d = C.ConvDesc()
     d.in_, d.wt, d.out = inp.data_ptr(), wt.data_ptr(), out.data_ptr()
     d.bias = bias.data_ptr() if bias is not None else None
@@ -138,7 +138,13 @@
     d.x_up = 1 if (x_up and spade_x is not None) else 0
     d.mask_slope = float(mask_slope) if relu_mask is not None else 0.0
     _set_taps(d, taps)
-    assert wt.shape[0] == len(taps) and wt.shape[2] == inp.shape[3] and wt.dtype == inp.dtype
+    if in_odd is not None:
+        assert in_odd.shape == inp.shape and in_odd.dtype == inp.dtype and in_odd.is_contiguous() and algo_cin == 2 * inp.shape[3]
+        d.Cin = algo_cin
+    assert wt.shape[0] == len(taps) and wt.shape[2] == d.Cin and wt.dtype == inp.dtype
+    if in_odd is not None:
+        C.backend().mgs_conv_taps2(d, _p(in_odd), _stream(inp))
+        return
     C.backend().mg_conv_taps(d, _stream(inp))
 
 
@@ -390,8 +396,14 @@
 
 
 def conv_dgrad(dy: torch.Tensor, wt: torch.Tensor, kh: int, kw: int, stride: int, pad: int,
-               in_hw: Tuple[int, int], cin: int, relu_mask: Optional[torch.Tensor] = None, mask_slope: float = 0.0) -> torch.Tensor:
+               in_hw: Tuple[int, int], cin: int, relu_mask: Optional[torch.Tensor] = None, mask_slope: float = 0.0,
+               dy_odd: Optional[torch.Tensor] = None) -> torch.Tensor:
     n, ho, wo, cg8 = dy.shape
+    two = {}
+    if dy_odd is not None:
+        assert stride == 1
+        cg8 *= 2
+        two = dict(in_odd=dy_odd, algo_cin=cg8)
     t = kh * kw
     h, w = in_hw
     assert wt.shape[0] == t and wt.shape[2] == cg8
@@ -408,16 +420,19 @@
         if hj == 0 or wj == 0 or not taps:
             continue
         _launch_conv(dy, wt[lo:hi], dx, None, taps, Hj=hj, Wj=wj, isy=1, isx=1,
-                     osy=stride, osx=stride, ooy=py, oox=px, cout=cin, cout_gemm=cin, relu_mask=relu_mask, mask_slope=mask_slope)
+                     osy=stride, osx=stride, ooy=py, oox=px, cout=cin, cout_gemm=cin, relu_mask=relu_mask, mask_slope=mask_slope, **two)
     if relu_mask is not None:
         assert relu_mask.shape == dx.shape and relu_mask.dtype == dx.dtype
         _leave_mask_record(dx, relu_mask)
     return dx
 
 
-def conv_wgrad(x: torch.Tensor, dy: torch.Tensor, kh: int, kw: int, stride: int, pad: int, want_bias: bool = False, out=None, beside: bool = False):
+def conv_wgrad(x: torch.Tensor, dy: torch.Tensor, kh: int, kw: int, stride: int, pad: int, want_bias: bool = False, out=None, beside: bool = False,
+               dy_odd: Optional[torch.Tensor] = None):
     n, h, w, cin = x.shape
     _, hj, wj, cg8 = dy.shape
+    if dy_odd is not None:
+        return _wgrad_launch(x, dy, fwd_taps(kh, kw, pad), stride, want_bias, out, beside, dy_odd=dy_odd)
     if out is not None:
         return _wgrad_launch(x, dy, fwd_taps(kh, kw, pad), stride, want_bias, out, beside)
     if _wgrad_swapped(stride, cg8, cin):
@@ -485,11 +500,14 @@
         self.dirty = False
         self.held = []
 
-    def hold(self, event, x, dy):
+    def hold(self, event, x, dy, dy_odd=None):
         held = self.held
         while held and held[0][0].query():
             held.pop(0)
-        held.append((event, x, dy, x.numel() * x.element_size() + dy.numel() * dy.element_size()))
+        nbytes = x.numel() * x.element_size() + dy.numel() * dy.element_size()
+        if dy_odd is not None:
+            nbytes += dy_odd.numel() * dy_odd.element_size()
+        held.append((event, x, dy, nbytes, dy_odd))
         over = sum(h[3] for h in held) - WGRAD_HELD_BUDGET
         while over > 0 and len(held) > 1:
             old = held.pop(0)
@@ -515,20 +533,20 @@
             ent.join()
 
 
-def sink_wgrad(arena, slot, x, dy, kh, kw, stride, pad, need_b):
+def sink_wgrad(arena, slot, x, dy, kh, kw, stride, pad, need_b, dy_odd=None):
     if WGRAD_SIDE_STREAM and x.is_cuda:
         ent = _wgrad_side(x.device)
         side = ent.stream
         side.wait_stream(torch.cuda.current_stream(x.device))
         with torch.cuda.stream(side):
-            conv_wgrad(x, dy, kh, kw, stride, pad, want_bias=need_b, out=(slot[1], slot[2]), beside=WGRAD_HALF_CU)
+            conv_wgrad(x, dy, kh, kw, stride, pad, want_bias=need_b, out=(slot[1], slot[2]), beside=WGRAD_HALF_CU, dy_odd=dy_odd)
             arena.slot_written(slot[0])
             ev = torch.cuda.Event()
             ev.record(side)
         ent.dirty = True
-        ent.hold(ev, x, dy)
+        ent.hold(ev, x, dy, dy_odd)
         return
-    conv_wgrad(x, dy, kh, kw, stride, pad, want_bias=need_b, out=(slot[1], slot[2]))
+    conv_wgrad(x, dy, kh, kw, stride, pad, want_bias=need_b, out=(slot[1], slot[2]), dy_odd=dy_odd)
     arena.slot_written(slot[0])
 
 
@@ -543,9 +561,16 @@
     return stride == 1 and cg8 <= 8 and cin >= 32
 
 
-def _wgrad_launch(x, dy, taps, stride, want_bias, out=None, beside=False):
+def _wgrad_flags(x, beside=False) -> int:
+    return (1 if (WGRAD_USE_TR and x.dtype == torch.bfloat16) else 0) | (2 if beside else 0)
+
+
+def _wgrad_launch(x, dy, taps, stride, want_bias, out=None, beside=False, dy_odd=None):
     n, h, w, cin = x.shape
     _, hj, wj, cg8 = dy.shape
+    if dy_odd is not None:
+        assert dy_odd.shape == dy.shape and dy_odd.dtype == dy.dtype and dy_odd.is_contiguous() and dy.is_contiguous()
+        cg8 *= 2
     ndw = len(taps) * cg8 * cin
     if out is not None:
         dw, dbias = out
@@ -563,7 +588,7 @@
     d.Hj, d.Wj, d.Cg = hj, wj, cg8
     d.isy = d.isx = stride
     d.splitk = 0
-    d.flags = (1 if (WGRAD_USE_TR and x.dtype == torch.bfloat16) else 0) | (2 if beside else 0)
+    d.flags = _wgrad_flags(x, beside)
     _set_taps(d, taps)
     assert dy.dtype == x.dtype
     if WGRAD_DETERMINISTIC:
@@ -572,7 +597,10 @@
             raise RuntimeError("mg_wgrad_det_workspace failed")
         ws = torch.empty(max(nbytes, 16), dtype=torch.uint8, device=x.device)
         d.det_ws, d.det_ws_bytes = ws.data_ptr(), nbytes
-    C.backend().mg_conv_wgrad(d, _stream(x))
+    if dy_odd is not None:
+        C.backend().mgs_conv_wgrad2(d, _p(dy_odd), _stream(x))
+    else:
+        C.backend().mg_conv_wgrad(d, _stream(x))
     return (dw, dbias) if want_bias else dw
 
 
@@ -877,6 +905,11 @@
     return rows
 
 
+def _interleave_blocks(a: torch.Tensor, b: torch.Tensor) -> torch.Tensor:
+    c = a.shape[-1]
+    return torch.stack([a.reshape(*a.shape[:-1], c // 32, 32), b.reshape(*b.shape[:-1], c // 32, 32)], dim=-2).reshape(*a.shape[:-1], 2 * c)
+
+
 def _interleave32(a: torch.Tensor, b: torch.Tensor) -> torch.Tensor:
     c = a.numel()
     cr = _roundup(c, 32)
@@ -901,17 +934,48 @@
     return out, g1
 
 
-def _spade_branch_reduce(dh, h, g1, x, mean, rstd, act, slope, sums, up=False):
+SPADE_DBETA = os.environ.get("MG_SPADE_DBETA", "1") != "0"
+SPADE_DBETA_LOG = None
+
+
+class _GammaBeta:
+    __slots__ = ("dgamma", "dh")
+
+    def __init__(self, dgamma, dh):
+        self.dgamma, self.dh = dgamma, dh
+
+
+def spade_dbeta_eligible(backend_name, dtype, dh_is_dpre, dh_contiguous, consumers_routed) -> bool:
+    return bool(SPADE_DBETA and backend_name == "hip" and dtype == torch.bfloat16 and dh_is_dpre and dh_contiguous and consumers_routed())
+
+
+def _spade_branch_reduce(dh, h, g1, x, mean, rstd, act, slope, sums, up=False, consumer=None):
     n, hh, ww, c = dh.shape
     p = n * hh * ww
     rows = 2 * _roundup(c, 32)
     be = C.backend()
-    alloc = torch.zeros if rows != 2 * c else torch.empty
-    dgb = alloc((n, hh, ww, rows), dtype=x.dtype, device=x.device)
     ws = _stats_workspace(1, p, c, x.device)
     if _grad_premasked(dh, h, act):
         act = ACT_NONE
     hp = _p(h) if act != ACT_NONE else None
+    if consumer is not None:
+        actv, wg = consumer
+        routed = spade_dbeta_eligible(getattr(be, "name", None), x.dtype, act == ACT_NONE, dh.is_contiguous(), lambda: (
+            c % 32 == 0 and wg.shape[2] == 3 and wg.shape[3] == 3 and actv.dtype == x.dtype and
+            be.mgs_spade_dbeta_route(_dt(x), n, hh, ww, c, actv.shape[3], _wgrad_flags(actv)) == 1))
+        if SPADE_DBETA_LOG is not None:
+            SPADE_DBETA_LOG.append((n, hh, ww, c, routed))
+        if routed:
+            dgamma = torch.empty((n, hh, ww, c), dtype=x.dtype, device=x.device)
+            if up:
+                be.mgs_norm_bwd_reduce_up(_p(dh), None, _p(x), _p(g1), _dt(x), n, hh, ww, c, _p(mean), _p(rstd), ACT_NONE, slope,
+                                          _p(dgamma), _p(sums), _p(ws), _stream(x))
+            else:
+                be.mgs_norm_bwd_reduce(_p(dh), None, _p(x), _p(g1), _dt(x), 1, p, c, _p(mean), _p(rstd), ACT_NONE, slope,
+                                       _p(dgamma), _p(sums), _p(ws), _stream(x))
+            return _GammaBeta(dgamma, dh), act, hp
+    alloc = torch.zeros if rows != 2 * c else torch.empty
+    dgb = alloc((n, hh, ww, rows), dtype=x.dtype, device=x.device)
     if up:
         be.mg_norm_bwd_reduce_up(_p(dh), hp, _p(x), _p(g1), _dt(x), n, hh, ww, c, _p(mean), _p(rstd), act, slope,
                                  _p(dgb), _p(sums), _p(ws), _stream(x))
@@ -922,27 +986,32 @@
 
 
 def _spade_branch_grads(needs, sink, actv, dgb, wg, wb, actv_relu):
+    dh = None
+    if isinstance(dgb, _GammaBeta):
+        dgb, dh = dgb.dgamma, dgb.dh
     hh, ww, rows = dgb.shape[1:]
+    if dh is not None:
+        rows *= 2
     c, kh = wg.shape[0], wg.shape[2]
     pad = kh // 2
     dactv = dwg = dbg = dwb = dbb = None
     if needs[0]:
         wt = pack_weight(wg, wb, dgb.dtype, _roundup(actv.shape[3], 128), rows, 1)
         dactv = conv_dgrad(dgb, wt, kh, kh, 1, pad, (hh, ww), actv.shape[3],
-                           relu_mask=actv if (actv_relu and FUSE_RELU_MASK) else None)
+                           relu_mask=actv if (actv_relu and FUSE_RELU_MASK) else None, dy_odd=dh)
     need_w = needs[1] or needs[3]
     need_b = needs[2] or needs[4]
     slot = db = None
     if sink is not None and needs[1] and needs[3]:
         slot = sink[0].grad_slot(wg, wb, sink[2] if need_b else None, sink[3] if need_b else None, kh * kh, rows, actv.shape[3], None)
     if slot is not None:
-        sink_wgrad(sink[0], slot, actv, dgb, kh, kh, 1, pad, need_b)
+        sink_wgrad(sink[0], slot, actv, dgb, kh, kh, 1, pad, need_b, dy_odd=dh)
     elif need_w:
-        res = conv_wgrad(actv, dgb, kh, kh, 1, pad, want_bias=need_b)
+        res = conv_wgrad(actv, dgb, kh, kh, 1, pad, want_bias=need_b, dy_odd=dh)
         dwg, dwb = unpack_wgrad(res[0] if need_b else res, wg.shape, two=True)
         db = res[1] if need_b else None
     elif need_b:
-        db = channel_sums(dgb)[0, 0].float()
+        db = channel_sums(dgb if dh is None else _interleave_blocks(dgb, dh))[0, 0].float()
     if db is not None:
         db = db.reshape(rows // 64, 2, 32)
         dbg, dbb = db[:, 0].reshape(-1)[:c], db[:, 1].reshape(-1)[:c]
@@ -971,7 +1040,7 @@
         dh = dh.contiguous()
         n, hh, ww, c = x.shape
         sums = torch.empty((1, 2, c), dtype=torch.float32, device=x.device)
-        dgb, act, hp = _spade_branch_reduce(dh, h, g1, x, mean, rstd, act, slope, sums)
+        dgb, act, hp = _spade_branch_reduce(dh, h, g1, x, mean, rstd, act, slope, sums, consumer=(actv, w_gamma))
         dx = work = None
         if ctx.needs_input_grad[0] and SYNC_BN_GROUP is not None:
             work = _sync_bn_all_reduce(sums, "syncbn_bwd")
@@ -1010,8 +1079,8 @@
         need_x = ctx.needs_input_grad[0]
         sums = torch.empty((2, 2, c), dtype=torch.float32, device=x.device)
         branches = ((dh0.contiguous(), h0, g10, actv0, wg0, wb0, 1), (dh1.contiguous(), h1, g11, actv1, wg1, wb1, 6))
-        reduced = [_spade_branch_reduce(dh, h, g1, x, mean, rstd, acts[b], slope, sums[b], up)
-                   for b, (dh, h, g1, *_r) in enumerate(branches)]
+        reduced = [_spade_branch_reduce(dh, h, g1, x, mean, rstd, acts[b], slope, sums[b], up, consumer=(actv, wg))
+                   for b, (dh, h, g1, actv, wg, *_r) in enumerate(branches)]
         work = None
         if need_x and SYNC_BN_GROUP is not None:
             work = _sync_bn_all_reduce(sums, "syncbn_bwd")
```

Result: no change. 132.6 images/s (median of 6 runs) (+0.7%).
